# we1pingyu/CALD

Measured on AMD Instinct MI355X. Metric: unlabeled images scored/sec (CALD consistency sweep), higher is better.
Workload: dtype f32

## Files before the change

### cald_amd/_ffi.py

```python
import ctypes as C
import os

_HERE = os.path.dirname(os.path.abspath(__file__))
LIB_PATH = os.path.join(_HERE, "lib", "libcaldhip.so")
_lib = None

c_f = C.POINTER(C.c_float)
c_i = C.POINTER(C.c_int)
c_i64 = C.POINTER(C.c_int64)
c_d = C.POINTER(C.c_double)
c_u8 = C.POINTER(C.c_uint8)
c_i8 = C.POINTER(C.c_int8)


class ModelCfg(C.Structure):
    _fields_ = [("arch", C.c_int), ("depth", C.c_int), ("num_classes", C.c_int), ("min_size", C.c_int),
                ("max_size", C.c_int), ("box_score_thresh", C.c_float), ("box_nms_thresh", C.c_float),
                ("detections_per_img", C.c_int), ("rpn_pre_nms_top_n", C.c_int), ("rpn_post_nms_top_n", C.c_int),
                ("rpn_nms_thresh", C.c_float), ("precision", C.c_int)]


PRECISION = {"fp32": 0, "f16x3": 1}


# ... 51 lines not shown
PROBE_MAX_RECTS = 8


class ConvProbe(C.Structure):
    _fields_ = [("V", C.c_int), ("in_hw", (C.c_int * 2) * PROBE_MAX_VIEWS), ("up_hw", (C.c_int * 2) * PROBE_MAX_VIEWS),
                ("dyn_rows", C.c_int * PROBE_MAX_VIEWS), ("has_dyn", C.c_int), ("gather", C.c_int), ("nrect", C.c_int * PROBE_MAX_VIEWS),
                ("rect", ((C.c_int * 4) * PROBE_MAX_RECTS) * PROBE_MAX_VIEWS),
                ("Cin", C.c_int), ("Cout", C.c_int), ("KH", C.c_int), ("KW", C.c_int), ("stride", C.c_int), ("pad", C.c_int),
                ("relu", C.c_int), ("in_relu", C.c_int), ("out_ld", C.c_int), ("cin_true", C.c_int),
                ("weight", c_f), ("bias", c_f), ("bn_scale", c_f), ("bn_shift", c_f), ("in_", c_f), ("in16", C.POINTER(C.c_uint32)),
                ("residual", c_f), ("up", c_f), ("ex16", C.c_int), ("mask", c_f), ("row_map", c_i),
                ("out", c_f), ("out_n", C.c_int64), ("out16", C.POINTER(C.c_uint32)), ("out16_n", C.c_int64),
                ("energy4", c_f), ("energy4_n", C.c_int64),
                ("head_w", c_f), ("head_b", c_f), ("head_out", c_f), ("head_out_n", C.c_int64), ("head_ld", C.c_int),
                ("row_packing", C.c_int)]


PRUNE_PROBE_MAX_VIEWS = 8


class RpnPruneProbe(C.Structure):
    _fields_ = [("V", C.c_int), ("guard", C.c_int), ("hw", ((C.c_int * 2) * PRUNE_PROBE_MAX_VIEWS) * 2),
                ("pre_n", C.c_int), ("head_ld", C.c_int), ("c1", C.c_float * 3), ("c0", C.c_float * 3),
                ("energy", c_f * 2), ("exact", c_f * 2), ("head", c_f * 2), ("pnorm", c_f * 2),
                ("tau_key", C.POINTER(C.c_uint32)), ("row_map", (c_i * 2) * 2), ("nsel", c_i * 2),
                ("check", C.c_float * 2), ("stat", C.c_uint64 * 4)]


class WgradPlan(C.Structure):
    _fields_ = [("variant", C.c_int), ("reduce", C.c_int), ("MT", C.c_int), ("JT", C.c_int), ("S", C.c_longlong), ("chunk", C.c_longlong),
                ("csplit", C.c_longlong), ("rows_per_block", C.c_longlong), ("scratch_bytes", C.c_longlong),
                ("kernel", C.c_char * 48), ("reduce_kernel", C.c_char * 32)]


PICK_FN = C.CFUNCTYPE(C.c_int, C.c_void_p, C.c_int, C.c_int, c_i, c_i, c_i)
SSM_RETINA_TAKE = 500

SIGNATURES = {
    "cald_last_error": (C.c_char_p, []),
    "cald_version": (C.c_int, []),
    "cald_ctx_create": (C.c_int, [C.c_int, C.c_void_p, C.POINTER(C.c_void_p)]),
    "cald_ctx_destroy": (C.c_int, [C.c_void_p]),
    "cald_ctx_sync": (C.c_int, [C.c_void_p]),
    "cald_model_create": (C.c_int, [C.c_void_p, C.POINTER(ModelCfg), C.POINTER(C.c_void_p)]),
    "cald_model_load_tensor": (C.c_int, [C.c_void_p, C.c_char_p, c_f, c_i64, C.c_int]),
    "cald_model_finalize": (C.c_int, [C.c_void_p]),
    "cald_model_set_rpn_prune": (C.c_int, [C.c_void_p, C.c_int, c_i]),
    "cald_model_set_rpn_prune_capture": (C.c_int, [C.c_void_p, C.c_int]),
    "cald_model_rpn_prune_bound": (C.c_int, [C.c_void_p, c_f, c_f]),
    "cald_model_set_rpn_prune_bound": (C.c_int, [C.c_void_p, c_f, c_f]),
    "cald_profile_prune_fallbacks": (C.c_int, [C.c_void_p, C.POINTER(C.c_int64)]),
    "cald_model_destroy": (C.c_int, [C.c_void_p]),
    "cald_forward": (C.c_int, [C.c_void_p, C.c_int, C.POINTER(View), C.POINTER(Dets)]),
    "cald_sweep": (C.c_int, [C.c_void_p, C.c_int, C.POINTER(C.c_void_p), c_i, c_i, c_i64, C.POINTER(SweepCfg), c_d, c_d]),
    "cald_sweep_audit": (C.c_int, [C.c_void_p, C.c_int, C.POINTER(C.c_void_p), c_i, c_i, c_i64, C.POINTER(SweepCfg), c_d, c_d, c_f]),
    "cald_sweep_ltc": (C.c_int, [C.c_void_p, C.c_int, C.POINTER(C.c_void_p), c_i, c_i, C.c_int, c_d]),
    "cald_sweep_ssm": (C.c_int, [C.c_void_p, C.c_int, C.POINTER(C.c_void_p), c_i, c_i, C.c_int, C.c_int64, c_i, c_i, c_f, c_f, c_i8, c_i64]),
    "cald_ssm_pick_mt19937": (C.c_int, [C.c_void_p, C.c_int, C.c_int, c_i, c_i, c_i]),
    "cald_sweep_ssm_retina": (C.c_int, [C.c_void_p, C.c_int, C.POINTER(C.c_void_p), c_i, c_i, C.c_int, C.c_void_p, C.c_void_p, C.c_int64, c_i, c_i, c_f, c_f,
                                        c_i8, c_i64]),
    "cald_sweep_lsc": (C.c_int, [C.c_void_p, C.c_int, C.POINTER(C.c_void_p), c_i, c_i, c_i64, C.c_uint64, C.c_int, c_d]),
    "cald_lossnet_create": (C.c_int, [C.c_void_p, C.POINTER(C.c_void_p)]),
    "cald_lossnet_load_tensor": (C.c_int, [C.c_void_p, C.c_char_p, c_f, c_i64, C.c_int]),
    "cald_lossnet_finalize": (C.c_int, [C.c_void_p]),
    "cald_lossnet_destroy": (C.c_int, [C.c_void_p]),
    "cald_sweep_ll": (C.c_int, [C.c_void_p, C.c_void_p, C.c_int, C.POINTER(C.c_void_p), c_i, c_i, c_i, C.POINTER(LLCfg), c_d, c_f]),
    "cald_vaal_create": (C.c_int, [C.c_void_p, C.POINTER(C.c_void_p)]),
    "cald_vaal_load_tensor": (C.c_int, [C.c_void_p, C.c_char_p, c_f, c_i64, C.c_int]),
    "cald_vaal_finalize": (C.c_int, [C.c_void_p]),
    "cald_vaal_destroy": (C.c_int, [C.c_void_p]),
    "cald_sweep_vaal": (C.c_int, [C.c_void_p, C.c_void_p, C.c_int, C.POINTER(C.c_void_p), c_i, c_i, C.POINTER(VaalCfg), c_f, c_f]),
    "cald_op_vaal_resize": (C.c_int, [C.c_void_p, c_u8, C.c_int, C.c_int, c_f]),
    "cald_op_vaal_bn_relu": (C.c_int, [C.c_void_p, c_f, C.c_longlong, C.c_int, C.c_int, C.c_int, c_f, c_f, c_f]),
    "cald_op_vaal_fc_mu": (C.c_int, [C.c_void_p, C.c_int, c_f, c_f]),
    "cald_op_vaal_head": (C.c_int, [C.c_void_p, C.c_int, c_f, c_f]),
    "cald_train_gap": (C.c_int, [C.c_void_p, C.c_int, C.POINTER(C.c_void_p), c_i, C.c_void_p]),
    "cald_lossnet_train_fwd": (C.c_int, [C.c_void_p, C.c_int, C.c_int, C.POINTER(LossNetTensors), C.c_void_p, C.c_void_p, C.c_void_p]),
    "cald_lossnet_train_bwd": (C.c_int, [C.c_void_p, C.c_int, C.c_int, C.POINTER(LossNetTensors), C.c_void_p, C.c_void_p, C.c_void_p, C.c_void_p,
                                         C.POINTER(LossNetTensors), C.c_int, C.c_void_p]),
    "cald_loss_pred_loss": (C.c_int, [C.c_void_p, C.c_int, C.c_void_p, C.c_void_p, C.c_float, C.c_int, C.c_void_p, C.c_void_p, C.c_void_p, C.c_void_p]),
    "cald_op_gap": (C.c_int, [C.c_void_p, c_f, C.c_int, C.c_int, C.c_int, c_f]),
    "cald_op_lossnet": (C.c_int, [C.c_void_p, C.c_int, c_f, c_f]),
    "cald_op_consistency": (C.c_int, [C.c_void_p, C.c_int, c_f, c_f, c_f, C.c_int, c_f, c_f, c_f, C.c_int, C.c_float, c_f]),
    "cald_op_cls_corr": (C.c_int, [C.c_void_p, C.c_int, c_f, c_i64, C.c_int, c_f]),
    "cald_op_pil_resize": (C.c_int, [C.c_void_p, C.c_void_p, C.c_int, C.c_int, C.c_void_p, C.c_int, C.c_int]),
    "cald_op_cutout_rects": (C.c_int, [C.c_uint64, C.c_int, C.c_int, C.c_int, c_f, C.c_int, c_i, c_i]),
    "cald_op_cutout_geometry": (C.c_int, [C.c_int, C.c_int, C.c_int, C.c_int, C.c_int, c_i, C.c_int, c_i, c_i]),
    "cald_op_augment": (C.c_int, [C.c_void_p, C.c_int, C.c_double, C.c_uint64, C.c_void_p, C.c_int, C.c_int, C.c_int, c_f,
                                  C.c_void_p, c_f, c_i]),
    "cald_op_noise_stream": (C.c_int, [C.c_void_p, C.c_uint64, C.c_void_p, C.c_int, C.c_int, C.c_int, c_i, c_d, C.POINTER(C.c_void_p)]),
    "cald_op_frcnn_postprocess": (C.c_int, [C.c_void_p, C.c_int, C.c_int, c_f, c_f, c_f, C.c_int, C.c_int, C.c_int, C.c_int, C.c_float, C.c_float,
                                            C.c_int, c_f, c_f, c_i64, c_f, c_f, c_f, c_i]),
    "cald_op_frcnn_postprocess_min": (C.c_int, [C.c_void_p, C.c_int, C.c_int, c_f, c_f, c_f, C.c_int, C.c_int, C.c_int, C.c_int, C.c_float, C.c_float,
                                                C.c_int, C.c_float, c_f, c_f, c_i64, c_f, c_f, c_f, c_i]),
    "cald_op_ssm_postprocess": (C.c_int, [C.c_void_p, C.c_int, C.c_int, c_f, c_f, c_f, C.c_int, C.c_int, C.c_int, C.c_int, C.c_float, C.c_int,
                                          c_i, c_i, c_f, c_f, c_i8]),
    "cald_op_retina_postprocess": (C.c_int, [C.c_void_p, C.POINTER(c_f), C.POINTER(c_f), c_i, C.c_int, C.c_int, c_f] + [C.c_int] * 6
                                   + [C.c_float, C.c_float, C.c_int, c_f, c_f, c_i64, c_f, c_f, c_i]),
    "cald_op_retina_ssm_postprocess": (C.c_int, [C.c_void_p, C.POINTER(c_f), C.POINTER(c_f), c_i, C.c_int, C.c_int, c_f] + [C.c_int] * 6
                                       + [C.c_float, C.c_float, C.c_int, C.c_void_p, C.c_void_p, c_i, c_i, c_i, c_f, c_f, c_i8]),
    "cald_op_rpn_prune": (C.c_int, [C.c_void_p, C.POINTER(RpnPruneProbe)]),
    "cald_op_roi_align": (C.c_int, [C.c_void_p, C.POINTER(c_f), c_i, C.c_int, C.c_int, c_f, c_f]),
    "cald_op_conv2d": (C.c_int, [C.c_void_p, c_f, C.c_int, C.c_int, C.c_int, c_f, C.c_int, C.c_int, C.c_int, C.c_int,
                                 C.c_int, c_f, c_f, c_f, c_f, C.c_int, c_f]),
    "cald_op_conv_probe": (C.c_int, [C.c_void_p, C.c_int, C.POINTER(ConvProbe), C.c_int, C.c_int, C.c_int, C.c_char_p, C.c_int]),
    "cald_op_mfma_f16": (C.c_int, [C.c_void_p, C.POINTER(C.c_uint16), C.POINTER(C.c_uint16), C.POINTER(C.c_uint32), C.POINTER(C.c_uint32), C.c_int64]),
    "cald_op_conv2d_f16x3": (C.c_int, [C.c_void_p, c_f, C.c_int, C.c_int, C.c_int, c_f, C.c_int, C.c_int, C.c_int, C.c_int,
                                       C.c_int, c_f, c_f, c_f, c_f, C.c_int, c_f]),
    "cald_op_conv_bench": (C.c_int, [C.c_void_p] + [C.c_int] * 12 + [c_d, c_d]),
    "cald_op_row_pack_lookup": (C.c_int, [C.c_int, c_i, c_i, C.c_int, C.c_int, C.c_int64, c_i64, c_i, c_i64, c_i64]),
    "cald_op_transform_size": (C.c_int, [C.c_int, C.c_int, C.c_int, C.c_int, c_i, c_i, c_i, c_i]),
    "cald_debug_tensor": (C.c_int, [C.c_void_p, C.c_char_p, C.c_int, c_f, C.c_int64, c_i64]),
    "cald_jpeg_info": (C.c_int, [C.c_void_p, C.c_size_t, c_i, c_i, c_i]),
    "cald_jpeg_decode_batch": (C.c_int, [C.c_void_p, C.c_int, C.POINTER(C.c_void_p), C.POINTER(C.c_size_t), C.POINTER(C.c_void_p)]),
    "cald_jpeg_probe": (C.c_int, [C.c_void_p, C.c_size_t, c_i, c_i, c_i, c_i]),
    "cald_jpeg_decode_batch_any": (C.c_int, [C.c_void_p, C.c_int, C.POINTER(C.c_void_p), C.POINTER(C.c_size_t), C.POINTER(C.c_void_p)]),
    "cald_jpeg_decode_host": (C.c_int, [C.c_void_p, C.c_size_t, C.c_void_p]),
    "cald_profile_enable": (C.c_int, [C.c_void_p, C.c_int]),
    "cald_profile_read": (C.c_int, [C.c_void_p, c_d, c_d, c_i64, c_d]),
    "cald_profile_prune": (C.c_int, [C.c_void_p, c_d, c_d, c_d, c_d, c_d]),
    "cald_profile_roi_rows": (C.c_int, [C.c_void_p, c_d, c_i64]),
    "cald_profile_cutout": (C.c_int, [C.c_void_p, c_d, c_d, c_i64, c_i64]),
    "cald_model_set_cutout_reuse": (C.c_int, [C.c_void_p, C.c_int, c_i]),
    "cald_model_set_look_fuse": (C.c_int, [C.c_void_p, C.c_int, c_i]),
    "cald_model_set_row_packing": (C.c_int, [C.c_void_p, C.c_int, c_i]),
    "cald_model_set_box_min_size": (C.c_int, [C.c_void_p, C.c_float, c_f]),
    "cald_profile_dump": (C.c_int, [C.c_void_p, C.c_char_p]),
    "cald_train_packed_floats": (C.c_int, [C.c_int] * 6 + [c_i64]),
    "cald_train_pack_conv": (C.c_int, [C.c_void_p] * 5 + [C.c_int] * 6 + [C.c_void_p]),
    "cald_train_pack_plan_scratch_floats": (C.c_int, [C.c_int, C.POINTER(PackJob), c_i64]),
    "cald_train_pack_plan_create": (C.c_int, [C.c_void_p, C.c_int, C.POINTER(PackJob), C.c_void_p, C.c_int64, C.POINTER(C.c_void_p)]),
    "cald_train_pack_plan_run": (C.c_int, [C.c_void_p, C.c_void_p]),
    "cald_train_pack_plan_destroy": (C.c_int, [C.c_void_p]),
    "cald_train_conv": (C.c_int, [C.c_void_p, C.c_int, C.c_int, C.c_int, C.c_void_p, C.c_int, C.c_void_p] + [C.c_int] * 8
                        + [C.c_void_p, C.c_void_p, C.c_int, C.c_int, C.c_void_p, C.c_void_p, C.c_int]),
    "cald_train_conv_group": (C.c_int, [C.c_void_p, C.c_int, C.c_int, c_i, C.POINTER(C.c_void_p), C.c_int, C.POINTER(C.c_void_p)] + [C.c_int] * 8
                              + [C.POINTER(C.c_void_p), C.POINTER(C.c_void_p), C.c_int]),
    "cald_train_conv_wgrad": (C.c_int, [C.c_void_p, C.c_int, C.c_int, C.c_int, C.c_void_p, C.c_int, C.c_int, C.c_void_p, C.c_int,
                                        C.c_int, C.c_int, C.c_int, C.c_int, C.c_int, C.c_void_p, C.c_void_p, C.c_void_p, C.c_int]),
    "cald_train_linear_wgrad": (C.c_int, [C.c_void_p, C.c_int, C.c_void_p, C.c_int, C.c_void_p, C.c_int, C.c_int, C.c_int,
                                          C.c_void_p, C.c_void_p, C.c_int]),
    "cald_train_wgrad_plan": (C.c_int, [C.c_longlong] + [C.c_int] * 12 + [C.POINTER(WgradPlan)]),
    "cald_train_relu_bwd": (C.c_int, [C.c_void_p, C.c_longlong, C.c_int, C.c_void_p, C.c_void_p, C.c_void_p]),
    "cald_train_add": (C.c_int, [C.c_void_p, C.c_longlong, C.c_void_p, C.c_void_p, C.c_void_p]),
    "cald_train_dilate": (C.c_int, [C.c_void_p] + [C.c_int] * 7 + [C.c_void_p, C.c_void_p]),
    "cald_train_upsample_bwd": (C.c_int, [C.c_void_p] + [C.c_int] * 6 + [C.c_void_p, C.c_void_p]),
    "cald_train_rpn_proposals": (C.c_int, [C.c_void_p, C.c_int, C.c_int, C.c_int, c_i, C.POINTER(C.c_void_p), c_i, C.c_int, C.c_int, C.c_int,
                                           C.c_float, C.c_float, C.c_void_p, C.c_void_p]),
    "cald_train_roi_sample_host": (C.c_int, [C.c_int, c_i, c_i, c_i, C.c_void_p, C.c_void_p, C.c_void_p, C.c_int, C.c_double, C.c_int, C.c_int,
                                             C.c_void_p, C.c_void_p, C.c_void_p, C.c_void_p, C.c_void_p, C.c_void_p, c_i, c_i, c_i]),
    "cald_train_roi_gather": (C.c_int, [C.c_void_p, C.c_void_p, C.c_void_p, C.c_void_p, C.c_int, C.c_int, C.c_int] + [C.c_float] * 4 + [C.c_void_p, C.c_void_p]),
    "cald_train_anchors": (C.c_int, [C.c_void_p, C.c_int, C.c_int, C.c_int, c_i, C.c_void_p]),
    "cald_train_match": (C.c_int, [C.c_void_p, C.c_int, C.c_void_p, C.c_int, C.c_void_p, C.c_float, C.c_float, C.c_int, C.c_void_p, C.c_void_p]),
    "cald_train_box_encode": (C.c_int, [C.c_void_p, C.c_int, C.c_void_p, C.c_void_p, C.c_float, C.c_float, C.c_float, C.c_float, C.c_void_p]),
    "cald_train_roi_align": (C.c_int, [C.c_void_p, C.POINTER(C.c_void_p), c_i, C.c_int, C.c_int, C.c_void_p, C.c_void_p]),
    "cald_train_roi_align_bwd": (C.c_int, [C.c_void_p, C.c_int, C.POINTER(C.c_void_p), c_i, C.c_int, C.c_int, C.c_void_p, C.c_void_p]),
    "cald_train_softmax_ce": (C.c_int, [C.c_void_p, C.c_int, C.c_int, C.c_int, C.c_void_p, C.c_void_p, C.c_float, C.c_void_p, C.c_void_p]),
    "cald_train_smooth_l1": (C.c_int, [C.c_void_p, C.c_int, C.c_void_p, C.c_void_p, C.c_void_p, C.c_float, C.c_float, C.c_void_p, C.c_float,
                                       C.c_void_p, C.c_void_p]),
    "cald_train_focal_loss": (C.c_int, [C.c_void_p, C.c_int, c_i, C.c_int, C.c_int, C.c_int, C.c_void_p, C.c_void_p, C.c_void_p, C.c_void_p,
                                        C.c_void_p, C.c_float, C.c_float, C.c_void_p, C.c_void_p]),
    "cald_train_bce_logits": (C.c_int, [C.c_void_p, C.c_int, C.c_void_p, C.c_void_p, C.c_void_p, C.c_float, C.c_void_p, C.c_void_p]),
    "cald_train_softmax_ce_seg": (C.c_int, [C.c_void_p, C.c_int, c_i, C.c_int, C.c_int, C.c_void_p, C.c_void_p, C.c_void_p, C.c_void_p, C.c_void_p]),
    "cald_train_smooth_l1_seg": (C.c_int, [C.c_void_p, C.c_int, c_i, C.c_void_p, C.c_void_p, C.c_void_p, C.c_float, c_f, C.c_void_p, C.c_void_p,
                                           C.c_void_p]),
    "cald_train_bce_logits_seg": (C.c_int, [C.c_void_p, C.c_int, c_i, C.c_void_p, C.c_void_p, C.c_void_p, C.c_void_p, C.c_void_p, C.c_void_p]),
    "cald_train_focal_loss_seg": (C.c_int, [C.c_void_p, C.c_int, c_i, C.c_int, C.c_int, C.c_int, C.c_void_p, C.c_void_p, C.c_void_p, C.c_void_p,
                                            c_f, C.c_float, C.c_void_p, C.c_void_p, C.c_void_p, C.c_void_p]),
    "cald_train_seg_mean": (C.c_int, [C.c_void_p, C.c_int, C.c_void_p, C.c_void_p]),
    "cald_train_add_bcast": (C.c_int, [C.c_void_p, C.c_int, C.c_longlong, C.c_int, C.c_void_p, C.c_void_p, C.c_void_p, C.c_void_p, C.c_longlong]),
    "cald_train_preprocess": (C.c_int, [C.c_void_p, C.c_int, C.POINTER(C.c_void_p), C.POINTER(C.c_void_p), c_i, C.c_int, C.c_int, C.c_void_p]),
    "cald_train_maxpool": (C.c_int, [C.c_void_p, C.c_int, C.c_int, C.c_int, C.c_int, C.c_void_p, C.c_void_p]),
    "cald_train_subsample2": (C.c_int, [C.c_void_p, C.c_int, C.c_int, C.c_int, C.c_int, C.c_void_p, C.c_void_p]),
    "cald_train_sgd": (C.c_int, [C.c_void_p, C.c_longlong, C.c_void_p, C.c_void_p, C.c_void_p, C.c_float, C.c_float, C.c_float, C.c_int]),
    "cald_train_seg_cache_size": (C.c_int, []),
    "cald_comm_unique_id": (C.c_int, [C.c_void_p]),
# ... 37 lines not shown
```

### cald_amd/csrc/conv_p4.hip

```cpp
#include "h16.h"

typedef float f32x16 __attribute__((ext_vector_type(16)));
typedef int i32x4 __attribute__((ext_vector_type(4)));
typedef float f32x4 __attribute__((ext_vector_type(4)));

template <int EPI, bool MASK, int TM, int TN, bool GATHER = false>
__device__ __forceinline__ void p4_epilogue(const ConvArgs& a, const f32x16 (&acc)[TM][TN], float* smem, const int v, const LevelSeg& so,
                                            const int m0, const int Mv, const int n0, const bool straddle = false) {
    constexpr int BM = 128, WN = 2;
    const int tid = threadIdx.x, lane = tid & 63, wave = tid >> 6;
    const int wm = wave / WN, wn = wave % WN;
    const int kh_lane = lane >> 5, l31 = lane & 31;
    const int Ho = so.H, Wo = so.W;
    const int out_ld = a.out_ld;
    float* __restrict__ out_v = a.out + so.pix_off * (long long)out_ld;
    const float* __restrict__ ex_v = nullptr;
    int upH = 1, upW = 1;
    float uph_s = 0.f, upw_s = 0.f;
    long long up_off = 0;
    if (EPI == 1) ex_v = a.residual + so.pix_off * (long long)out_ld;
    if (EPI == 2) {
        const LevelSeg su = a.seg_up[v];
        up_off = su.pix_off;
        ex_v = a.up + su.pix_off * (long long)out_ld;
        upH = su.H; upW = su.W;
        uph_s = (float)upH / (float)Ho; upw_s = (float)upW / (float)Wo;
    }
    const bool relu = a.relu != 0, has_bias = a.bias != nullptr, has_bn = a.scale != nullptr;
    constexpr bool has_mask = MASK;
    const float* __restrict__ mask_v = has_mask ? a.mask + so.pix_off * (long long)out_ld : out_v;
    const int row_b = out_ld * 4;
    const unsigned long long vb64 = (unsigned long long)(GATHER ? Ho * Wo : Mv) * (unsigned)row_b;
    const unsigned valid_b = vb64 < 0x7FFE0000ull ? (unsigned)vb64 : 0x7FFE0000u;
    const __amdgpu_buffer_rsrc_t rsO = __builtin_amdgcn_make_buffer_rsrc((void*)out_v, 0, valid_b, 0x00020000);
    const __amdgpu_buffer_rsrc_t rsX = __builtin_amdgcn_make_buffer_rsrc((void*)(EPI != 0 ? ex_v : out_v), 0, EPI == 1 ? valid_b : 0x7FFE0000, 0x00020000);
    const __amdgpu_buffer_rsrc_t rsM = __builtin_amdgcn_make_buffer_rsrc((void*)mask_v, 0, valid_b, 0x00020000);
    static_assert(!(GATHER && EPI == 2), "gathered rows take no top-down term");
    const int Mlast = Mv - 1;
    int* const s_src = reinterpret_cast<int*>(smem);
    if (EPI == 2 || GATHER) {
        if (tid < BM) {
            int m = m0 + tid;
            if (GATHER) {
                s_src[tid] = m < Mv ? gather_pixel(a.gather[v], m, Wo) * row_b : 0x7FFF0000;
            } else if (EPI == 2 && straddle) {
                int src = 0;
                if (m < Mv) {
                    const long long r = so.pix_off + m;
                    int vr = v;
                    while (vr + 1 < a.V && a.seg_out[vr + 1].pix_off <= r) vr++;
                    const LevelSeg sor = a.seg_out[vr], sur = a.seg_up[vr];
                    const int ml = (int)(r - sor.pix_off), oy = ml / sor.W, ox = ml - oy * sor.W;
                    const float hs = (float)sur.H / (float)sor.H, ws = (float)sur.W / (float)sor.W;
                    int sy = (int)floorf((float)oy * hs); sy = sy > sur.H - 1 ? sur.H - 1 : sy;
                    int sx = (int)floorf((float)ox * ws); sx = sx > sur.W - 1 ? sur.W - 1 : sx;
                    src = ((int)(sur.pix_off - up_off) + sy * sur.W + sx) * out_ld * 4;
                }
                s_src[tid] = src;
            } else {
                m = m < Mlast ? m : Mlast;
                const int oy = m / Wo, ox = m - oy * Wo;
                int sy = (int)floorf((float)oy * uph_s); sy = sy > upH - 1 ? upH - 1 : sy;
                int sx = (int)floorf((float)ox * upw_s); sx = sx > upW - 1 ? upW - 1 : sx;
                s_src[tid] = (sy * upW + sx) * out_ld * 4;
            }
        }
        __syncthreads();
    }
    auto gather_offs = [&](const int i, const int n, const bool nok, int (&go)[16]) {
        const int rl = wm * TM * 32 + i * 32 + 4 * kh_lane;
#pragma unroll
        for (int q = 0; q < 4; q++) {
            const i32x4 so4 = *reinterpret_cast<const i32x4*>(s_src + rl + 8 * q);
#pragma unroll
            for (int jj = 0; jj < 4; jj++) go[4 * q + jj] = nok ? so4[jj] + n * 4 : 0x7FFF0000;
        }
    };
    constexpr bool EXTRA = EPI == 0 && !MASK && !GATHER;
    const bool want16 = EXTRA && a.out16 != nullptr, wantE = EXTRA && TN == 2 && a.energy4 != nullptr;
    unsigned char* const out16_v = want16 ? reinterpret_cast<unsigned char*>(a.out16) + so.pix_off * (long long)out_ld * 4 : nullptr;
    const __amdgpu_buffer_rsrc_t rsS = __builtin_amdgcn_make_buffer_rsrc((void*)(want16 ? (void*)out16_v : (void*)out_v), 0, valid_b, 0x00020000);
    const bool odd = (lane & 1) != 0;
    float sq[TM][16];
    if (EXTRA) {
#pragma unroll
        for (int i = 0; i < TM; i++)
#pragma unroll
            for (int r = 0; r < 16; r++) sq[i][r] = 0.0f;
    }
    float bs_[TN], sc_[TN], sh_[TN];
#pragma unroll
    for (int j = 0; j < TN; j++) {
        const int n = n0 + wn * TN * 32 + j * 32 + l31;
        const int nc = n < a.Cout ? n : 0;
        bs_[j] = has_bias ? a.bias[nc] : 0.0f;
        sc_[j] = has_bn ? a.scale[nc] : 1.0f;
        sh_[j] = has_bn ? a.shift[nc] : 0.0f;
    }
    constexpr int NTILE = TM * TN, PRE = GATHER ? 1 : NTILE;
    float extra_[EPI != 0 ? NTILE : 1][16];
    auto load_extra = [&](const int t, float (&extra)[16]) {
        const int j = t / TM, i = t - j * TM;
        const int n = n0 + wn * TN * 32 + j * 32 + l31;
        const bool nok = n < a.Cout;
        const int nc = nok ? n : 0;
        const int mbase = m0 + wm * TM * 32 + i * 32 + 4 * kh_lane;
        if (EPI == 1 && GATHER) {
            int go[16];
            gather_offs(i, n, nok, go);
#pragma unroll
            for (int r = 0; r < 16; r++) extra[r] = __builtin_bit_cast(float, __builtin_amdgcn_raw_buffer_load_b32(rsX, go[r], 0, 0));
        } else if (EPI == 1) {
            const int vo = nok ? (mbase * out_ld + n) * 4 : 0x7FFF0000;
#pragma unroll
            for (int r = 0; r < 16; r++)
                extra[r] = __builtin_bit_cast(float, __builtin_amdgcn_raw_buffer_load_b32(rsX, vo, ((r & 3) + 8 * (r >> 2)) * row_b, 0));
        } else if (EPI == 2) {
            const int rl = wm * TM * 32 + i * 32 + 4 * kh_lane;
#pragma unroll
            for (int q = 0; q < 4; q++) {
                const i32x4 so4 = *reinterpret_cast<const i32x4*>(s_src + rl + 8 * q);
#pragma unroll
                for (int jj = 0; jj < 4; jj++)
                    extra[4 * q + jj] = __builtin_bit_cast(float, __builtin_amdgcn_raw_buffer_load_b32(rsX, so4[jj] + nc * 4, 0, 0));
            }
        }
    };
    if (EPI != 0) {
#pragma unroll
        for (int t = 0; t < PRE; t++) load_extra(t, extra_[EPI != 0 ? t : 0]);
    }
#pragma unroll
    for (int j = 0; j < TN; j++) {
        const int n = n0 + wn * TN * 32 + j * 32 + l31;
        const bool nok = n < a.Cout;
        const int nc = nok ? n : 0;
        const float bs = bs_[j], sc = sc_[j], sh = sh_[j];
#pragma unroll
        for (int i = 0; i < TM; i++) {
            const int mbase = m0 + wm * TM * 32 + i * 32 + 4 * kh_lane;
            const float (&extra)[16] = extra_[EPI != 0 ? j * TM + i : 0];
            float val[16];
#pragma unroll
            for (int r = 0; r < 16; r++) val[r] = acc[i][j][r];
            if (has_bias) {
#pragma unroll
                for (int r = 0; r < 16; r++) val[r] = val[r] + bs;
            }
            if (has_bn) {
#pragma unroll
                for (int r = 0; r < 16; r++) { val[r] = val[r] * sc; val[r] = val[r] + sh; }
            }
            if (EPI != 0) {
#pragma unroll
                for (int r = 0; r < 16; r++) val[r] = val[r] + extra[r];
            }
            if (relu) {
#pragma unroll
                for (int r = 0; r < 16; r++) val[r] = val[r] > 0.0f ? val[r] : 0.0f;
            }
            if (EPI != 0 && j * TM + i + PRE < NTILE) load_extra(j * TM + i + PRE, extra_[EPI != 0 ? j * TM + i + PRE : 0]);
            const int vo = nok ? (mbase * out_ld + n) * 4 : 0x7FFF0000;
            if (has_mask) {
                float mk[16];
#pragma unroll
                for (int r = 0; r < 16; r++)
                    mk[r] = __builtin_bit_cast(float, __builtin_amdgcn_raw_buffer_load_b32(rsM, vo, ((r & 3) + 8 * (r >> 2)) * row_b, 0));
#pragma unroll
                for (int r = 0; r < 16; r++) val[r] = mk[r] > 0.0f ? val[r] : 0.0f;
            }
            if (GATHER) {
                int go[16];
                gather_offs(i, n, nok, go);
#pragma unroll
                for (int r = 0; r < 16; r++) __builtin_amdgcn_raw_buffer_store_b32(__builtin_bit_cast(unsigned, val[r]), rsO, go[r], 0, 0);
            } else {
#pragma unroll
                for (int r = 0; r < 16; r++)
                    __builtin_amdgcn_raw_buffer_store_b32(__builtin_bit_cast(unsigned, val[r]), rsO, vo, ((r & 3) + 8 * (r >> 2)) * row_b, 0);
            }
            if (EXTRA) {
                if (wantE) {
#pragma unroll
                    for (int r = 0; r < 16; r++) sq[i][r] = sq[i][r] + (nok ? val[r] * val[r] : 0.0f);
                }
                if (want16) {
                    const int poff = h16_pair_off(nc);
#pragma unroll
                    for (int r = 0; r < 16; r++) {
                        const unsigned w = h16_split(val[r]);
                        const unsigned pw = h16_pair_word(w, h16_partner(w), odd);
                        __builtin_amdgcn_raw_buffer_store_b32(pw, rsS, nok ? mbase * row_b + poff : 0x7FFF0000, ((r & 3) + 8 * (r >> 2)) * row_b, 0);
                    }
                }
            }
        }
    }
    if (EXTRA) {
        if (wantE) {
            __syncthreads();
            float* const red = smem + wave * (64 * 33);
#pragma unroll
            for (int i = 0; i < TM; i++)
#pragma unroll
                for (int r = 0; r < 16; r++) red[(i * 32 + 4 * kh_lane + (r & 3) + 8 * (r >> 2)) * 33 + l31] = sq[i][r];
            asm volatile("s_waitcnt lgkmcnt(0)" ::: "memory");
            float e = 0.0f;
#pragma unroll
            for (int q = 0; q < 32; q++) e = e + red[lane * 33 + q];
            const int m = m0 + wm * TM * 32 + lane;
            if (m < Mv) a.energy4[(so.pix_off + m) * 4 + (n0 / (64 * TN)) * 2 + wn] = e;
        }
    }
}

template <int EPIX, bool C4, int TN, int TAPS>
__device__ __forceinline__ void conv_p4_body(const ConvArgs& a, const int blk, const ConvArgs* a3 = nullptr) {
    constexpr int EPI = EPIX & 3;
    constexpr bool MASK = (EPIX & 4) != 0;
    constexpr bool FUSE = (EPIX & 8) != 0;
    constexpr bool GATHER = (EPIX & 16) != 0;
    static_assert(!(GATHER && (FUSE || MASK || C4)), "gathered rows: plain EPI 0 / 1 kernels only");
    constexpr int BM = 128, BN = 64 * TN, BK = 16, TM = 2, WN = 2;
    constexpr int TILE_A = 2 * BM * 8, TILE_F = TILE_A + 2 * BN * 8;
    constexpr int FUSE_T = 4 * TILE_A;
    __shared__ __attribute__((aligned(16))) float smem[FUSE ? FUSE_T + 4096 : 3 * TILE_F];

    const int tid = threadIdx.x, lane = tid & 63, wave = tid >> 6;
    const int wm = wave / WN, wn = wave % WN;
    const int NT = a.CoutPad / BN;
    unsigned long long* const trace = (a.trace && blockIdx.x < (1u << 17)) ? a.trace + (size_t)blockIdx.x * 8 : nullptr;
    if (trace && tid == 0) {
        trace[0] = __builtin_amdgcn_s_memtime();
        trace[5] = (unsigned)__builtin_amdgcn_s_getreg((31 << 11) | 4);
        trace[6] = (unsigned)__builtin_amdgcn_s_getreg((31 << 11) | 20);
        trace[7] = blockIdx.x;
    }
    int mt, nt;
    if (a.KH * a.KW > 1) {
        const int MT = a.total_mtiles, CH = (MT + 7) >> 3;
        const int xcd = blk & 7, idx = blk >> 3;
        mt = xcd * CH + idx / NT; nt = idx % NT;
        if (idx / NT >= CH || mt >= MT) return;
    } else {
        const int b = blk, MT = a.total_mtiles, MT8 = MT & ~7;
        if (b < MT8 * NT) { const int xcd = b & 7, idx = b >> 3; mt = (idx / NT) * 8 + xcd; nt = idx % NT; }
        else { const int r = b - MT8 * NT; mt = MT8 + r / NT; nt = r % NT; }
    }
    const int n0 = nt * BN;
    constexpr bool CAN_PACK = !C4 && !MASK && !FUSE && !GATHER;
    const bool packed = CAN_PACK && a.packed_rows != 0;
    const int v = packed ? seg_find_row(a.seg_out, a.V, (long long)mt * BM) : seg_find_view(a.seg_out, a.V, mt);
    const LevelSeg so = a.seg_out[v];
    const LevelSeg si = a.seg_in[v];
    const int Ho = so.H, Wo = so.W, Hi = si.H, Wi = si.W;
    int Mv = Ho * Wo;
    if (a.dyn_rows) { const int d = a.dyn_rows[v]; Mv = d < Mv ? d : Mv; }
    if (GATHER) Mv = a.gather[v].cum[a.gather[v].nr];
    int m0 = (mt - so.tile_start) * BM;
    bool straddle = false;
    if (CAN_PACK && packed) {
        const int row0 = mt * BM, left = a.packed_rows - row0;
        m0 = row0 - (int)so.pix_off;
        const int end = m0 + (left < BM ? left : BM);
        straddle = end > Mv;
        Mv = end;
    }
    if (m0 >= Mv) return;
    const float* __restrict__ in_v = a.in + si.pix_off * (long long)a.Cin;
    const int Cin = a.Cin, KW = a.KW, KH = a.KH, CoutPad = a.CoutPad;
    const bool in_relu = a.in_relu != 0;

    const int g = tid & 3, arow = tid >> 2;
    unsigned rowmask[2];
// ... 328 lines not shown
            __syncthreads();
            if (n0c + 64 < CoutPad3) fetch_w(n0c + 64);
            const int n3 = n0c + wn * 32 + l31;
            int vo3[2];
            float ex[2][16];
#pragma unroll
            for (int i = 0; i < 2; i++) vo3[i] = ((m0 + wm * 64 + i * 32 + 4 * kh_lane) * ld3 + n3) * 4;
#pragma unroll
            for (int i = 0; i < 2; i++)
#pragma unroll
                for (int r = 0; r < 16; r++)
                    ex[i][r] = __builtin_bit_cast(float, __builtin_amdgcn_raw_buffer_load_b32(rsX3, vo3[i], ((r & 3) + 8 * (r >> 2)) * ld3 * 4, 0));
            __builtin_amdgcn_sched_barrier(0);
            f32x16 acc2[2][1];
#pragma unroll
            for (int i = 0; i < 2; i++)
#pragma unroll
                for (int r = 0; r < 16; r++) acc2[i][0][r] = 0.0f;
#pragma unroll
            for (int kt = 0; kt < 4; kt++) {
                f32x4 ga0[2], ga1[2];
#pragma unroll
                for (int t = 0; t < 2; t++) {
                    ga0[t] = *reinterpret_cast<const f32x4*>(Tl + kt * TILE_A + foa2[t]);
                    ga1[t] = *reinterpret_cast<const f32x4*>(Tl + kt * TILE_A + foa2[t] + BM * 8);
                }
                const f32x4 gb0 = *reinterpret_cast<const f32x4*>(Wl + kt * 1024 + fob2);
                const f32x4 gb1 = *reinterpret_cast<const f32x4*>(Wl + kt * 1024 + fob2 + 64 * 8);
#pragma unroll
                for (int q = 0; q < 4; q++)
#pragma unroll
                    for (int i = 0; i < 2; i++) acc2[i][0] = __builtin_amdgcn_mfma_f32_32x32x2f32(ga0[i][q], gb0[q], acc2[i][0], 0, 0, 0);
#pragma unroll
                for (int q = 0; q < 4; q++)
#pragma unroll
                    for (int i = 0; i < 2; i++) acc2[i][0] = __builtin_amdgcn_mfma_f32_32x32x2f32(ga1[i][q], gb1[q], acc2[i][0], 0, 0, 0);
            }
            {
                const float sc3 = b.scale[n3], sh3 = b.shift[n3];
#pragma unroll
                for (int i = 0; i < 2; i++) {
#pragma unroll
                    for (int r = 0; r < 16; r++) {
                        float val = acc2[i][0][r] * sc3;
                        val = val + sh3;
                        val = val + ex[i][r];
                        if (relu3) val = val > 0.0f ? val : 0.0f;
                        __builtin_amdgcn_raw_buffer_store_b32(__builtin_bit_cast(unsigned, val), rsO3, vo3[i], ((r & 3) + 8 * (r >> 2)) * ld3 * 4, 0);
                    }
                }
            }
        }
    } else {
        p4_epilogue<EPI, MASK, TM, TN, GATHER>(a, acc, smem, v, so, m0, Mv, n0, CAN_PACK && straddle);
    }
    if (trace && tid == 0) {
        trace[3] = __builtin_amdgcn_s_memtime();
        asm volatile("s_waitcnt vmcnt(0)" ::: "memory");
        trace[4] = __builtin_amdgcn_s_memtime();
    }
}

template <int EPI, bool C4, int TN, int TAPS>
__global__ __launch_bounds__(256, 3) void conv_p4_kernel(const ConvArgs a) { conv_p4_body<EPI, C4, TN, TAPS>(a, blockIdx.x); }
template <int EPI, bool C4, int TN, int TAPS>
__global__ __launch_bounds__(256, 3) void conv_p4_group_kernel(const ConvGroup g) {
    int i = 0;
    while (i + 1 < g.n && g.blk0[i + 1] <= (int)blockIdx.x) i++;
    conv_p4_body<EPI, C4, TN, TAPS>(g.p[i], (int)blockIdx.x - g.blk0[i]);
}
__global__ __launch_bounds__(256, 3) void conv_p4_fused_kernel(const ConvGroup g) { conv_p4_body<8, false, 1, 9>(g.p[0], blockIdx.x, &g.p[1]); }

static inline int p4_taps(const ConvArgs& a) {
    if (a.Cin % 16 != 0) return 0;
    if (a.KH == 3 && a.KW == 3) return 9;
    if (a.KH == 1 && a.KW == 1) return 1;
    return 0;
}

static inline int p4_grid_mtiles(const ConvArgs& a) { return a.KH * a.KW > 1 ? 8 * ((a.total_mtiles + 7) / 8) : a.total_mtiles; }

static inline bool p4_refuses(const ConvArgs& a) {
    if (!a.w4 || !a.out || a.in16 || a.ex16 || a.CoutPad % 64 != 0 || (a.residual && a.up)) return true;
    const bool extra = a.out16 || a.energy4;
    if (extra && (a.residual || a.up || a.mask || a.gather)) return true;
    if (a.energy4 && a.CoutPad != 256) return true;
    if (a.row_map && (a.residual || a.up || a.mask || a.gather)) return true;
    return false;
}
static inline bool p4_tile_ok(const ConvArgs& a, const bool wide, const ConvForce f) {
    if (f.tile == TILE_NARROW && wide) return false;
    if (f.tile == TILE_WIDE && !wide) return false;
    return !(a.energy4 && !wide);
}

static inline ConvArgs p4_tiled(ConvArgs a) {
    if (a.packed_rows > 0 && a.Cin != 4 && !a.dyn_rows && !a.row_map && !a.gather && !a.mask) a.total_mtiles = (a.packed_rows + 127) / 128;
    else a.packed_rows = 0;
    return a;
}

#define P4_NAME(K, EPIV, C4V, TNV, TAPSV) K "<" #EPIV "," #C4V "," #TNV "," #TAPSV ">"
template <int EPI, bool C4, int TN, int TAPS>
static const char* p4_go(const dim3 grid, hipStream_t stream, const ConvArgs& a, const char* name) {
    hipLaunchKernelGGL((conv_p4_kernel<EPI, C4, TN, TAPS>), grid, dim3(256), 0, stream, a);
    return name;
}
template <int EPI, int TN, int TAPS>
static const char* p4_group_go(const dim3 grid, hipStream_t stream, const ConvGroup& g, const char* name) {
    hipLaunchKernelGGL((conv_p4_group_kernel<EPI, false, TN, TAPS>), grid, dim3(256), 0, stream, g);
    return name;
}

const char* launch_conv_p4_group(const ConvArgs* p, int n, hipStream_t stream, ConvForce f) {
    if (n < 1 || n > CALD_MAX_GROUP) return nullptr;
    const bool wide = f.tile == TILE_NARROW ? false : p[0].CoutPad % 128 == 0;
    ConvGroup g; g.n = n; int blk = 0;
    for (int i = 0; i < n; i++) {
        const ConvArgs a = p4_tiled(p[i]);
        if (p4_refuses(a) || !p4_tile_ok(a, wide, f) || (a.CoutPad % 128 == 0) != (p[0].CoutPad % 128 == 0)) return nullptr;
        if (a.Cin % 16 != 0 || a.KH * a.KW > 32 || a.residual || a.up || a.gather) return nullptr;
        if ((a.mask != nullptr) != (p[0].mask != nullptr)) return nullptr;
        if (a.mask && (a.out16 || a.energy4)) return nullptr;
        g.blk0[i] = blk; blk += p4_grid_mtiles(a) * (a.CoutPad / (wide ? 128 : 64)); g.p[i] = a;
    }
    g.blk0[n] = blk;
    const int taps = p4_taps(p[0]);
    for (int i = 1; i < n; i++) if (p4_taps(p[i]) != taps) return nullptr;
    const dim3 grid((unsigned)blk);
#define P4_GROUP(EV, TNV, TAPSV) p4_group_go<EV, TNV, TAPSV>(grid, stream, g, P4_NAME("conv_p4_group_kernel", EV, false, TNV, TAPSV))
#define P4_GROUP_T(EV) (wide ? (taps == 9 ? P4_GROUP(EV, 2, 9) : taps == 1 ? P4_GROUP(EV, 2, 1) : P4_GROUP(EV, 2, 0)) \
                             : (taps == 9 ? P4_GROUP(EV, 1, 9) : taps == 1 ? P4_GROUP(EV, 1, 1) : P4_GROUP(EV, 1, 0)))
    const char* name = p[0].mask ? P4_GROUP_T(4) : P4_GROUP_T(0);
#undef P4_GROUP_T
#undef P4_GROUP
    return name;
}

const char* launch_conv_p4_fused(const ConvArgs& c2, const ConvArgs& c3, hipStream_t stream) {
    if (!c2.w4 || !c3.w4 || c2.w16 || c3.w16) return nullptr;
    if (c2.KH != 3 || c2.KW != 3 || c2.stride != 1 || c2.pad != 1 || c2.Cin % 16 || c2.Cout != 64 || c2.CoutPad != 64 || c2.out_ld != 64) return nullptr;
    if (c2.residual || c2.up || c2.mask || c2.dyn_rows || c2.in_relu || c2.gather || c3.gather || p4_taps(c2) != 9) return nullptr;
    if (c3.KH != 1 || c3.KW != 1 || c3.stride != 1 || c3.pad != 0 || c3.Cin != 64 || c3.Kpad != 64 || c3.CoutPad % 64 || c3.Cout != c3.CoutPad) return nullptr;
    if (!c3.residual || !c3.scale || c3.bias || c3.out_ld != c3.Cout || c3.up || c3.mask || c3.dyn_rows || c3.in_relu || c3.in != c2.out || c3.total_mtiles != c2.total_mtiles || c3.V != c2.V) return nullptr;
    if (c2.row_map || c3.row_map || c2.in16 || c3.in16 || c2.out16 || c3.out16 || c2.energy4 || c3.energy4 || c2.ex16 || c3.ex16 || !c3.out) return nullptr;
    ConvGroup g; g.n = 2; g.blk0[0] = 0; g.p[0] = c2; g.p[1] = c3;
    const unsigned grid = (unsigned)p4_grid_mtiles(c2);
    hipLaunchKernelGGL(conv_p4_fused_kernel, dim3(grid), dim3(256), 0, stream, g);
    return "conv_p4_fused_kernel";
}

const char* launch_conv_p4(const ConvArgs& a_in, hipStream_t stream, ConvForce f) {
    const ConvArgs a = p4_tiled(a_in);
    if (p4_refuses(a)) return nullptr;
    bool wide = a.CoutPad % 128 == 0;
    if (wide) {
        const long long b2 = (long long)a.total_mtiles * (a.CoutPad / 128), b1 = 2 * b2;
        const double e2 = (double)b2 / (double)(((b2 + 767) / 768) * 768), e1 = 0.88 * (double)b1 / (double)(((b1 + 767) / 768) * 768);
        if (e1 > e2 && !a.dyn_rows && !a.energy4) wide = false;
    }
    if (f.tile == TILE_NARROW) wide = false;
    else if (f.tile == TILE_WIDE) wide = a.CoutPad % 128 == 0;
    if (!p4_tile_ok(a, wide, f)) return nullptr;
    const dim3 grid((unsigned)(p4_grid_mtiles(a) * (a.CoutPad / (wide ? 128 : 64))));
#define P4_ONE(EPIV, C4V, TNV, TAPSV) p4_go<EPIV, C4V, TNV, TAPSV>(grid, stream, a, P4_NAME("conv_p4_kernel", EPIV, C4V, TNV, TAPSV))
    if (a.gather) {
        const int taps = p4_taps(a);
        if (a.Cin == 4 || a.up || a.mask || a.in_relu || a.dyn_rows || a.row_map || (taps != 1 && taps != 9)) return nullptr;
        if (a.total_mtiles == 0) return "none (no gathered rows)";
#define P4_G(EPIV, TNV) (taps == 9 ? P4_ONE(EPIV, false, TNV, 9) : P4_ONE(EPIV, false, TNV, 1))
        return wide ? (a.residual ? P4_G(17, 2) : P4_G(16, 2)) : (a.residual ? P4_G(17, 1) : P4_G(16, 1));
#undef P4_G
    }
    if (a.Cin == 4) {
        if (a.residual || a.up || a.in_relu || a.mask) return nullptr;
        if (a.KH == 7 && a.KW == 7 && a.Kpad == 208)
            return wide ? P4_ONE(0, true, 2, 13) : P4_ONE(0, true, 1, 13);
        return wide ? P4_ONE(0, true, 2, 0) : P4_ONE(0, true, 1, 0);
    }
    if (a.Cin % 16 != 0 || a.KH * a.KW > 32) return nullptr;
    const int taps = p4_taps(a);
#define P4_TAPS(EPIV, TNV) (taps == 9 ? P4_ONE(EPIV, false, TNV, 9) : taps == 1 ? P4_ONE(EPIV, false, TNV, 1) : P4_ONE(EPIV, false, TNV, 0))
    const char* name;
    if (a.mask) {
        if (a.up) return nullptr;
        name = wide ? (a.residual ? P4_TAPS(5, 2) : P4_TAPS(4, 2)) : (a.residual ? P4_TAPS(5, 1) : P4_TAPS(4, 1));
    } else if (wide) {
        name = a.residual ? P4_TAPS(1, 2) : a.up ? P4_TAPS(2, 2) : P4_TAPS(0, 2);
    } else {
        name = a.residual ? P4_TAPS(1, 1) : a.up ? P4_TAPS(2, 1) : P4_TAPS(0, 1);
    }
#undef P4_TAPS
#undef P4_ONE
    return name;
}
#undef P4_NAME
```

### cald_amd/csrc/ctx.hip

```cpp
#include "host.h"

static thread_local char g_err[512] = "";
int cald_host::fail(int code, const char* fmt, ...) {
    va_list ap; va_start(ap, fmt); vsnprintf(g_err, sizeof(g_err), fmt, ap); va_end(ap);
    return code;
}

int cald_internal_fail(int code, const char* fmt, ...) {
    va_list ap; va_start(ap, fmt); vsnprintf(g_err, sizeof(g_err), fmt, ap); va_end(ap);
    return code;
}
void cald_internal_train_release(cald_ctx* c);

extern "C" const char* cald_last_error(void) { return g_err; }
extern "C" int cald_version(void) { return 100; }

hipStream_t cald_internal_stream(cald_ctx* c) { return c->stream; }
int cald_internal_device(cald_ctx* c) { return c->device; }
const float* cald_internal_zeros(cald_ctx* c) { return c->d_zeros; }
int cald_internal_scratch(cald_ctx* c, size_t bytes, void** out) {
    if (bytes > c->train_scratch_cap) {
        HIPCHK(hipStreamSynchronize(c->stream));
        if (c->train_scratch) HIPCHK(hipFree(c->train_scratch));
        c->train_scratch = nullptr; c->train_scratch_cap = 0;
// ... 97 lines not shown
    }
    if (gemm_ms) *gemm_ms = ms;
    unsigned long long rows = 0;
    HIPCHK(hipMemcpy(&rows, c->d_roi_rows, 8, hipMemcpyDeviceToHost));
    double fl = c->prof_flops - look_fl;
    if (c->prof_roi_rows_cap > 0.0) fl -= c->prof_roi_flops_cap * (1.0 - (double)rows / c->prof_roi_rows_cap);
    unsigned long long st[4] = {0, 0, 0, 0};
    HIPCHK(hipMemcpy(st, c->d_prune_stat, 32, hipMemcpyDeviceToHost));
    for (int l = 0; l < 2; l++) if (st[2 * l + 1]) fl -= c->prof_prune_flops_cap[l] * (1.0 - (double)st[2 * l] / (2.0 * (double)st[2 * l + 1]));
    if (gemm_flops) *gemm_flops = fl;
    if (launches) *launches = (int64_t)c->prof_launches.size() - look_n + c->prof_extra_launches;
    if (total_ms) *total_ms = c->tot_ms;
    return 0;
}

extern "C" int cald_profile_prune(cald_ctx* c, double* look_ms, double* look_flops, double* selected_frac2, double* worst_bound_ratio, double* pruned_flops) {
    if (!c) return fail(CALD_ERR_INVALID, "ctx is null");
    HIPCHK(hipStreamSynchronize(c->stream));
    double ms = 0.0, fl = 0.0;
    for (const ProfLaunch& L : c->prof_launches)
        if (L.tag) { float t = 0.f; HIPCHK(hipEventElapsedTime(&t, L.e0, L.e1)); ms += t; fl += L.flops; }
    unsigned long long st[4] = {0, 0, 0, 0};
    HIPCHK(hipMemcpy(st, c->d_prune_stat, 32, hipMemcpyDeviceToHost));
    if (look_ms) *look_ms = ms;
    if (look_flops) *look_flops = fl;
    if (selected_frac2) for (int l = 0; l < 2; l++) selected_frac2[l] = st[2 * l + 1] ? (double)st[2 * l] / (double)st[2 * l + 1] : 0.0;
    if (worst_bound_ratio) *worst_bound_ratio = (double)c->prune_worst;
    if (pruned_flops) {
        double fl2 = 0.0;
        for (int l = 0; l < 2; l++) if (st[2 * l + 1]) fl2 += c->prof_prune_flops_cap[l] / 2.0 * (1.0 - (double)st[2 * l] / (double)st[2 * l + 1]);
        *pruned_flops = fl2;
    }
    return 0;
}

extern "C" int cald_profile_roi_rows(cald_ctx* c, double* mean_rows_per_view, int64_t* views) {
    if (!c) return fail(CALD_ERR_INVALID, "ctx is null");
    HIPCHK(hipStreamSynchronize(c->stream));
    unsigned long long rows = 0;
    HIPCHK(hipMemcpy(&rows, c->d_roi_rows, 8, hipMemcpyDeviceToHost));
    if (views) *views = c->prof_roi_views;
    if (mean_rows_per_view) *mean_rows_per_view = c->prof_roi_views ? (double)rows / (double)c->prof_roi_views : 0.0;
    return 0;
}

extern "C" int cald_profile_cutout(cald_ctx* c, double* rows3, double* dense_rows3, int64_t* batches, int64_t* fallbacks) {
    if (!c) return fail(CALD_ERR_INVALID, "ctx is null");
    for (int i = 0; i < 3; i++) { if (rows3) rows3[i] = c->cut_rows[i]; if (dense_rows3) dense_rows3[i] = c->cut_dense[i]; }
    if (batches) *batches = c->cut_batches;
    if (fallbacks) *fallbacks = c->cut_fallbacks;
    return 0;
}

extern "C" int cald_profile_dump(cald_ctx* c, const char* path) {
    if (!c || !path) return fail(CALD_ERR_INVALID, "null argument");
    HIPCHK(hipStreamSynchronize(c->stream));
    FILE* f = fopen(path, "w");
    if (!f) return fail(CALD_ERR_INVALID, "cannot open %s", path);
    fprintf(f, "launch,desc,gflop,ms,tflops\n");
    std::vector<unsigned long long> lg((size_t)CALD_PRUNE_LOG * 4, 0ull);
    if (!c->prof_gather.empty()) HIPCHK(hipMemcpy(lg.data(), c->d_prune_log, lg.size() * 8, hipMemcpyDeviceToHost));
    for (size_t i = 0; i < c->prof_launches.size(); i++) {
        const ProfLaunch& L = c->prof_launches[i];
        float t = 0.f; hipEventElapsedTime(&t, L.e0, L.e1);
        double fl = L.flops;
        const char* extra = L.tag ? ",f16x3-lookahead" : "";
        auto g = c->prof_gather.find(i);
        if (g != c->prof_gather.end()) {
            for (int l = 0; l < 2; l++) {
                const unsigned long long sel = lg[(size_t)g->second.log * 4 + 2 * l], tot = lg[(size_t)g->second.log * 4 + 2 * l + 1];
                if (tot) fl -= g->second.cap[l] * (1.0 - (double)sel / (double)tot);
            }
            extra = ",gathered-rows";
        }
        fprintf(f, "%zu,\"%s%s\",%.3f,%.4f,%.2f\n", i, L.desc.c_str(), extra, fl / 1e9, t, fl / (t * 1e-3) / 1e12);
    }
    fclose(f);
    return 0;
}
extern "C" int cald_profile_prune_fallbacks(cald_ctx* c, int64_t* n) {
    if (!c || !n) return fail(CALD_ERR_INVALID, "null argument");
    *n = (int64_t)c->prune_fallbacks;
    return 0;
}

int cald_host::prof_begin(cald_ctx* c, ProfLaunch& t) {
    if (!c->prof) return 0;
    HIPCHK(hipEventCreate(&t.e0)); HIPCHK(hipEventCreate(&t.e1));
    HIPCHK(hipEventRecord(t.e0, c->stream));
    return 0;
}
int cald_host::prof_end(cald_ctx* c, ProfLaunch& t, double flops, int tag, const char* fmt, ...) {
    if (!c->prof) return 0;
    HIPCHK(hipEventRecord(t.e1, c->stream));
    char d[160];
    va_list ap; va_start(ap, fmt); vsnprintf(d, sizeof(d), fmt, ap); va_end(ap);
    t.flops = flops; t.tag = tag; t.desc = d;
    c->prof_launches.push_back(t); c->prof_flops += flops;
    return 0;
}

int cald_host::conv_refused(const ConvArgs& a) {
    return fail(CALD_ERR_UNSUPPORTED, "no conv kernel implements this launch (Cin=%d Cout=%d k=%dx%d residual=%d up=%d mask=%d gather=%d energy4=%d out16=%d)",
                a.Cin, a.Cout, a.KH, a.KW, a.residual != nullptr, a.up != nullptr, a.mask != nullptr, a.gather != nullptr, a.energy4 != nullptr,
                a.out16 != nullptr);
}
// ... 9 lines not shown
```

### cald_amd/csrc/forward.hip

```cpp
#include "host.h"

#define ROI_DENSE_VIEWS 32
void cald_host::build_plan(BatchPlan& P, int V, const ViewDesc* views, const int (*hp)[2], bool retina) {
    memset(&P, 0, sizeof(P));
    for (int l = 0; l < CALD_MAX_LEVELS; l++) {
        long long off = 0; int tile = 0;
        for (int v = 0; v <= V; v++) {
            LevelSeg& s = P.seg[l][v];
            s.pix_off = off; s.tile_start = tile;
            if (v == V) break;
            int H, W;
            if (l == 7 && retina) { int h6 = (hp[v][0] / 32 - 1) / 2 + 1, w6 = (hp[v][1] / 32 - 1) / 2 + 1; H = (h6 - 1) / 2 + 1; W = (w6 - 1) / 2 + 1; }
            else if (l == 7) { H = 1; W = CALD_ROI_CAP; }
            else if (l == 8) {
                const int first = v * ROI_DENSE_VIEWS, cnt = first < V ? (V - first < ROI_DENSE_VIEWS ? V - first : ROI_DENSE_VIEWS) : 0;
                H = cnt ? 1 : 0; W = cnt * CALD_ROI_CAP;
            }
            else if (l == 6) { H = (hp[v][0] / 32 - 1) / 2 + 1; W = (hp[v][1] / 32 - 1) / 2 + 1; }
            else { H = hp[v][0] >> l; W = hp[v][1] >> l; }
            s.H = H; s.W = W;
            off += (long long)H * W;
            tile += (H * W + 127) / 128;
        }
    }
// ... 248 lines not shown
static int conv_pair_on(cald_model* m, const ConvLayer& L2, const ConvLayer& L3, const float* in, float* mid, float* out, int lin, int lout,
                        int V, const float* residual) {
    cald_ctx* c = m->ctx;
    if (m->cfg.precision == CALD_PRECISION_FP32 && L2.stride == 1 && lin == lout) {
        ConvArgs a2, a3;
            const double f2 = fill_conv_args(m, a2, L2, in, mid, lin, lout, V, true);
        const double f3 = fill_conv_args(m, a3, L3, mid, out, lout, lout, V, true, residual);
        if (f2 < 0.0 || f3 < 0.0) return (int)(f2 < 0.0 ? f2 : f3);
        ProfLaunch t; int rc;
        if ((rc = prof_begin(c, t))) return rc;
        if (launch_conv_p4_fused(a2, a3, c->stream) != nullptr)
            return prof_end(c, t, f2 + f3, 0, "mt=%d,Cin=%d,Cout=%d,k=3x3+1x1,s=1,fused->%d", a2.total_mtiles, a2.Cin, a2.Cout, a3.Cout);
        if (c->prof) { hipEventDestroy(t.e0); hipEventDestroy(t.e1); }
    }
    int rc = conv_on(m, L2, in, mid, lin, lout, V, true);
    if (rc) return rc;
    return conv_on(m, L3, mid, out, lout, lout, V, true, residual);
}
static int conv_group_on(cald_model* m, const ConvSpec* sp, int n, int V) {
    ConvArgs a[CALD_MAX_GROUP];
    double flops = 0.0; int tiles = 0;
    for (int i = 0; i < n; i++) {
        const double f = fill_conv_args(m, a[i], *sp[i].L, sp[i].in, sp[i].out, sp[i].level, sp[i].level, V, sp[i].relu, nullptr, nullptr, 0, sp[i].dyn);
        if (f < 0.0) return (int)f;
        a[i].row_map = sp[i].row_map;
        if (sp[i].in16) a[i].in16 = sp[i].in16;
        if (sp[i].out16) a[i].out16 = sp[i].out16;
        a[i].energy4 = sp[i].energy4;
        offer_packing(m, a[i], sp[i].level, sp[i].level, 0, V);
        flops += f; tiles += a[i].total_mtiles;
    }
    cald_ctx* c = m->ctx;
    const char* names[CALD_MAX_GROUP];
    ProfLaunch t; int rc;
    if ((rc = prof_begin(c, t))) return rc;
    const int launches = launch_conv_group(a, n, c->stream, names);
    if (c->prof) c->prof_extra_launches += launches - 1;
    if ((rc = prof_end(c, t, flops, c->prof_tag_now, "mt=%d,Cin=%d,Cout=%d,k=%dx%d,s=%d,group=%d", tiles, a[0].Cin, a[0].Cout, a[0].KH, a[0].KW, a[0].stride, n))) return rc;
    for (int i = 0; i < n; i++) if (!names[i]) return conv_refused(a[i]);
    return 0;
}

static int gconv_on(cald_model* m, const ConvLayer& L, const float* in, float* out, int lin, int lout, int V, bool relu, const float* residual,
                    const FwdReuse& ru, int b, int kind) {
    if (!ru.tiles[b][kind]) return 0;
    ConvArgs a;
    const double f = fill_conv_args(m, a, L, in, out, lin, lout, V, relu, residual);
    if (f < 0.0) return (int)f;
    const char* base = ru.d_gp + (size_t)(2 * b + kind) * cut_plan_set_bytes(V);
    a.seg_out = reinterpret_cast<const LevelSeg*>(base);
    a.gather = reinterpret_cast<const GatherSet*>(base + (size_t)(V + 1) * sizeof(LevelSeg));
    a.total_mtiles = ru.tiles[b][kind];
    return run_conv(m->ctx, a, 2.0 * ru.rows[b][kind] * (double)L.Cout * (double)(L.KH * L.KW * L.CinTrue));
}

__global__ void accumulate_rows_kernel(const int* __restrict__ counts, int V, unsigned long long* acc) {
    unsigned long long s = 0;
    for (int v = threadIdx.x; v < V; v += 64) s += (unsigned long long)counts[v];
    for (int o = 32; o > 0; o >>= 1) s += __shfl_down(s, o);
    if (threadIdx.x == 0) atomicAdd(acc, s);
}

static const float RPN_MIN_SIZE = 1e-3f;
struct ForwardRun {
    cald_model* m; int V; ViewDesc* views; const DetBuffers& det; float* audit_out; bool prune_ok; const FwdReuse* ru; FwdFeatures* feat; FwdSsm* ssm; FwdRetinaSsm* rssm;
    cald_ctx* c = nullptr; hipStream_t st = nullptr; const BatchPlan* dp = nullptr;
    bool retina = false, prune = false;
    int hp[CALD_MAX_VIEWS][2], max_pix0 = 0, max_pix2 = 0, max_pix6 = 0;
    BodyBufs Fb; PyramidBufs Fp; RetinaBufs Fr; RpnBufs Fn; PruneBufs Fq; BoxBufs Fx; AuditBufs Fa;
    void layout(Bump& B) {
        const BatchPlan& P = m->plan; long long px[8];
        for (int l = 0; l < 8; l++) px[l] = level_pix(P, l, V);
        m->split.clear();
        static const bool split_on = !(getenv("CALD_H3_S16") && atoi(getenv("CALD_H3_S16")) == 0);
        SplitReg S{m, B, m->cfg.precision == CALD_PRECISION_F16X3 && split_on};
        Fb.layout(B, S, px);
        Fp.layout(B, S, px, retina);
        if (feat) return;
        if (retina) {
            int maxa = 0;
            for (int v = 0; v < V; v++) { int t = 0; for (int l = 3; l < 8; l++) t += P.seg[l][v].H * P.seg[l][v].W * 9; if (t > maxa) maxa = t; }
            Fr.layout(B, S, px, V, m->cls_out.Cout, m->cfg.num_classes, m->cfg.detections_per_img, maxa, rssm ? &rssm->out : nullptr);
            return;
        }
        Fn.layout(B, px, V, m->cfg.rpn_pre_nms_top_n);
        if (m->prune) Fq.layout(B, px, V, m->prune_capture);
        Fx.layout(B, S, V, m->pred.Cout, m->cfg.num_classes, m->key_cap);
        Fa.layout(B, V, m->det_cap());
        if (ssm) ssm->out.layout(B, V, m->cfg.num_classes, m->cfg.detections_per_img);
    }
    int prepare() {
        c = m->ctx;
        if (!m->finalized) return fail(CALD_ERR_STATE, "model not finalized (call cald_model_finalize)");
        if (V < 1 || V > CALD_MAX_VIEWS) return fail(CALD_ERR_INVALID, "n_views must be 1..%d", CALD_MAX_VIEWS);
        if (feat && (audit_out || prune_ok || ru)) return fail(CALD_ERR_INVALID, "a features-only forward takes no audit, pruning or cut_out reuse");
        if (ssm && (feat || audit_out || ru || m->cfg.arch != CALD_ARCH_FRCNN)) return fail(CALD_ERR_INVALID, "the SSM forward is a plain Faster R-CNN forward");
        if (rssm && (feat || audit_out || ru || ssm || !rssm->pick || m->cfg.arch != CALD_ARCH_RETINANET || m->cfg.num_classes < 2))
            return fail(CALD_ERR_INVALID, "the RetinaNet SSM forward is a plain RetinaNet forward with a pick callback and at least two classes");
        if (!feat && !ssm && !rssm && det.cap < m->det_cap()) return fail(CALD_ERR_INVALID, "detection capacity %d < required %d", det.cap, m->det_cap());
        HIPCHK(hipSetDevice(c->device));
        for (int v = 0; v < V; v++) {
            ViewDesc& d = views[v];
            if (!d.src || d.H <= 0 || d.W <= 0 || d.nrect < 0 || d.nrect > CALD_MAX_CUT) return fail(CALD_ERR_INVALID, "view %d is malformed", v);
            int Hp, Wp;
            transform_size(d.H, d.W, m->cfg.min_size, m->cfg.max_size, &d.Hr, &d.Wr, &Hp, &Wp);
            d.Ho = d.H; d.Wo = d.W;
// ... 20 lines not shown
        { Bump dry(nullptr, true); layout(dry); int rc = arena_reserve(c, dry.off); if (rc) return rc; }
        { Bump real(c->arena, false); layout(real); }
        const int si = c->stage_i; c->stage_i = (si + 1) % cald_ctx::NSTAGE;
        HIPCHK(hipEventSynchronize(c->stage_ev[si]));
        memcpy(c->h_stage[si], &m->plan, sizeof(BatchPlan));
        memcpy(c->h_stage[si] + sizeof(BatchPlan), views, sizeof(ViewDesc) * V);
        HIPCHK(hipMemcpyAsync(c->d_plan, c->h_stage[si], sizeof(BatchPlan), hipMemcpyHostToDevice, c->stream));
        HIPCHK(hipMemcpyAsync(c->d_views, c->h_stage[si] + sizeof(BatchPlan), sizeof(ViewDesc) * V, hipMemcpyHostToDevice, c->stream));
        HIPCHK(hipEventRecord(c->stage_ev[si], c->stream));
        dp = c->d_plan; st = c->stream;
        m->dbg.clear();
        return 0;
    }
    int dense_block(const Bottleneck& B, const float* cur, float* dst, int lvl, int lout) {
        int rc; const float* idn = cur;
        if (B.has_down) { if ((rc = conv_on(m, B.down, cur, Fb.D, lvl, lout, V, false))) return rc; idn = Fb.D; }
        if ((rc = conv_on(m, B.c1, cur, Fb.T1, lvl, lvl, V, true))) return rc;
        return conv_pair_on(m, B.c2, B.c3, Fb.T1, Fb.T2, dst, lvl, lout, V, idn);
    }
    int gathered_block(const Bottleneck& B, int b, const float* cur, float* dst, int lvl, int lout) {
        int rc; const float* idn = cur;
        if (B.has_down) { if ((rc = gconv_on(m, B.down, cur, Fb.D, lvl, lout, V, false, nullptr, *ru, b, 0))) return rc; idn = Fb.D; }
        if ((rc = gconv_on(m, B.c1, cur, Fb.T1, lvl, lvl, V, true, nullptr, *ru, b, 1))) return rc;
        if ((rc = gconv_on(m, B.c2, Fb.T1, Fb.T2, lvl, lout, V, true, nullptr, *ru, b, 0))) return rc;
        return gconv_on(m, B.c3, Fb.T2, dst, lout, lout, V, true, idn, *ru, b, 0);
    }
    int body() {
        int rc;
        launch_preprocess(c->d_views, dp->seg[0], Fb.in0, V, max_pix0, st);
        m->dbg["input"] = {Fb.in0, 0, 4, 0};
        if ((rc = conv_on(m, m->conv1, Fb.in0, Fb.c1, 0, 1, V, true))) return rc;
        m->dbg["conv1"] = {Fb.c1, 1, 64, 0};
        launch_maxpool(Fb.c1, Fb.p1, dp->seg[1], dp->seg[2], 64, V, max_pix2, st, m->split.count(Fb.p1) != 0);
        m->dbg["pool1"] = {Fb.p1, 2, 64, 0};
        const float* cur = Fb.p1; int lvl = 2, layer = 0, xi = 0;
        for (size_t b = 0; b < m->blocks.size(); b++) {
            const Bottleneck& B = m->blocks[b];
            const int lout = lvl + (B.c2.stride == 2 ? 1 : 0);
            const bool kept = ru && (int)b < ru->nblk;
            float* dst = kept ? ru->out[b] : (B.layer_end ? Fb.Cf[layer] : Fb.X[xi]);
            if ((rc = kept && ru->mode == 2 && ru->gather[layer] ? gathered_block(B, (int)b, cur, dst, lvl, lout) : dense_block(B, cur, dst, lvl, lout))) return rc;
            if (B.layer_end) Fb.Cf[layer] = dst;
            cur = dst; lvl = lout;
            if (B.layer_end) layer++; else xi ^= 1;
        }
        const char* cn[4] = {"C2", "C3", "C4", "C5"};
        for (int i = 0; i < 4; i++) m->dbg[cn[i]] = {Fb.Cf[i], 2 + i, CCH[i], 0};
        return 0;
    }
    void name_pyramid(int first, int n) { for (int i = 0; i < n; i++) m->dbg["P" + std::to_string(first + i)] = {Fp.Pf[i], first + i, 256, 0}; }
    int fpn() {
        const int first = retina ? 3 : 2, nl = retina ? 3 : 4, c0 = 4 - nl;
        int rc; ConvSpec sp[4];
        if ((rc = conv_on(m, m->fpn_inner[nl - 1], Fb.Cf[3], Fp.inner[nl - 1], 5, 5, V, false))) return rc;
        for (int i = nl - 2; i >= 0; i--)
            if ((rc = conv_on(m, m->fpn_inner[i], Fb.Cf[c0 + i], Fp.inner[i], first + i, first + i, V, false, nullptr, Fp.inner[i + 1], first + 1 + i))) return rc;
        for (int i = 0; i < nl; i++) sp[i] = {&m->fpn_layer[i], Fp.inner[i], Fp.Pf[i], first + i, false};
        if (prune)
            for (int i = 0; i < 2; i++) { sp[i].out16 = Fq.p16[i]; sp[i].energy4 = Fq.energy[i]; }
        if ((rc = conv_group_on(m, sp, nl, V))) return rc;
        if (!retina) return 0;
        if ((rc = conv_on(m, m->p6, Fp.Pf[2], Fp.Pf[3], 5, 6, V, false))) return rc;
        if (feat && !feat->p7) return 0;
        return conv_on(m, m->p7, Fp.Pf[3], Fp.Pf[4], 6, 7, V, false, nullptr, nullptr, 0, nullptr, true);
    }
    void hand_out(int first, int n) {
        name_pyramid(first, n);
        for (int i = 0; i < n; i++) {
            auto sp = m->split.find(Fp.Pf[i]);
            feat->P[i] = Fp.Pf[i]; feat->split_only[i] = sp != m->split.end() && sp->second.fp32_dead; feat->plan_level[i] = first + i;
        }
    }
    int retina_head_and_tail() {
        int rc;
        for (int t = 0; t < 4; t++) {
            ConvSpec sp[10];
            for (int hsel = 0; hsel < 2; hsel++)
                for (int i = 0; i < 5; i++)
                    sp[hsel * 5 + i] = {&(hsel == 0 ? m->cls_tower : m->reg_tower)[t], t == 0 ? Fp.Pf[i] : Fr.ret_t[hsel][(t - 1) & 1][i],
                                        Fr.ret_t[hsel][t & 1][i], 3 + i, true};
            if ((rc = conv_group_on(m, sp, 10, V))) return rc;
        }
        for (int hsel = 0; hsel < 2; hsel++) {
            ConvSpec sp[5];
            for (int i = 0; i < 5; i++) sp[i] = {hsel == 0 ? &m->cls_out : &m->reg_out, Fr.ret_t[hsel][1][i], hsel == 0 ? Fr.cls_h[i] : Fr.reg_h[i], 3 + i, false};
            if ((rc = conv_group_on(m, sp, 5, V))) return rc;
        }
        for (int i = 0; i < 5; i++) {
            m->dbg["cls" + std::to_string(i)] = {Fr.cls_h[i], 3 + i, m->cls_out.Cout, 0};
            m->dbg["reg" + std::to_string(i)] = {Fr.reg_h[i], 3 + i, 36, 0};
        }
        if (rssm) return retina_ssm_tail();
        launch_retina_postprocess(retina_args(Fr.tail, Fr.cls_h, Fr.reg_h, dp, c->d_views, m->d_anchors, 9, m->cfg.num_classes, V, m->cfg.box_score_thresh,
                                              m->cfg.box_nms_thresh, m->cfg.detections_per_img, det), Fr.tail.max_anchors, st);
        return 0;
    }
    int retina_ssm_tail() {
        const RetinaSsmArgs sa = retina_ssm_args(rssm->out, Fr.cls_h, Fr.reg_h, dp, c->d_views, m->d_anchors, 9, m->cfg.num_classes, V, m->cfg.box_score_thresh,
                                                 m->cfg.box_nms_thresh, m->cfg.detections_per_img);
        launch_retina_ssm_phase_a(sa, st);
        HIPCHK(hipGetLastError());
        if (int rc = retina_ssm_pick_stop(c, rssm->out, V, m->cfg.num_classes, rssm->pick, rssm->user, rssm->image0, nullptr)) return rc;
        launch_retina_ssm_phase_b(sa, st);
        return 0;
    }
    void p6_subsample() {
        auto tw = m->split.find(Fp.Pf[3]);
        const bool p6_split = m->split.count(Fp.Pf[4]) != 0 && tw != m->split.end();
        launch_subsample2(p6_split ? reinterpret_cast<const float*>(tw->second.s16) : Fp.Pf[3], Fp.Pf[4], dp->seg[5], dp->seg[6], 256, V, max_pix6, st);
        name_pyramid(2, 5);
    }
    void name_rpn(int first) { for (int i = first; i < 5; i++) m->dbg["rpn" + std::to_string(i)] = {Fn.rpn_h[i], 2 + i, 15, 0}; }
    int rpn_dense() {
// ... 208 lines not shown
```

### cald_amd/csrc/host.h

```cpp
#pragma once
#include "../../include/cald_hip.h"
#include "common.h"
#include "kernels.h"
#include "host_logic.h"

#include <climits>
#include <cmath>
#include <cstdarg>
#include <cstdio>
#include <cstring>
#include <algorithm>
#include <map>
#include <string>
#include <vector>

namespace cald_host {
int fail(int code, const char* fmt, ...);
#define HIPCHK(x) do { hipError_t e_ = (x); if (e_ != hipSuccess) return fail(CALD_ERR_HIP, "%s failed: %s (%s:%d)", #x, hipGetErrorString(e_), __FILE__, __LINE__); } while (0)

struct PilCoef { int ksize; int* d_bounds; int* d_kk; };
struct PilKey { int in, out, fid; bool operator<(const PilKey& o) const { return in != o.in ? in < o.in : (out != o.out ? out < o.out : fid < o.fid); } };
struct ProfLaunch {
    hipEvent_t e0 = nullptr, e1 = nullptr;
    double flops = 0.0;
    int tag = 0;
    std::string desc;
};
}
using namespace cald_host;

#define CALD_PRUNE_LOG 4096
struct cald_ctx {
    int device = 0;
    hipStream_t stream = nullptr;
    bool own_stream = false;
    char* arena = nullptr; size_t arena_cap = 0, arena_off = 0;
    BatchPlan* d_plan = nullptr;
    ViewDesc* d_views = nullptr;
    float* d_zeros = nullptr;
    static const int NSTAGE = 8;
    char* h_stage[NSTAGE] = {nullptr}; hipEvent_t stage_ev[NSTAGE] = {nullptr}; int stage_i = 0;
    bool prof = false;
    std::vector<ProfLaunch> prof_launches;
    double prof_flops = 0.0; int64_t prof_extra_launches = 0;
    int prof_tag_now = 0;
    double prof_prune_flops_cap[2] = {0.0, 0.0};
    hipEvent_t tot0 = nullptr, tot1 = nullptr; bool tot_open = false; double tot_ms = 0.0;
    float prune_worst = 0.0f;
    long long prune_fallbacks = 0;
    float* d_prune_check = nullptr;
    unsigned long long* d_prune_stat = nullptr;
    unsigned long long* d_prune_log = nullptr; int prune_log_n = 0;
    struct GatherNote { int log; double cap[2]; };
    std::map<size_t, GatherNote> prof_gather;
    unsigned long long* d_roi_rows = nullptr; double prof_roi_rows_cap = 0.0, prof_roi_flops_cap = 0.0; long long prof_roi_views = 0;
    std::map<PilKey, PilCoef> pil;
    char* train_scratch = nullptr; size_t train_scratch_cap = 0;
    double cut_rows[3] = {0.0, 0.0, 0.0}, cut_dense[3] = {0.0, 0.0, 0.0};
    long long cut_batches = 0, cut_fallbacks = 0;
};

namespace cald_host {
struct ScopedDev {
    std::vector<void*> ptrs;
    hipStream_t st;
    explicit ScopedDev(hipStream_t s) : st(s) {}
    ~ScopedDev() { if (!ptrs.empty()) { hipStreamSynchronize(st); for (void* p : ptrs) hipFree(p); } }
    void release() { ptrs.clear(); }
    template <typename T> int alloc(T** out, size_t bytes) {
        HIPCHK(hipMalloc((void**)out, bytes ? bytes : 1));
        ptrs.push_back((void*)*out);
        return 0;
    }
    template <typename T> int upload(T** out, const void* h, size_t bytes) {
        *out = nullptr;
        if (!h) return 0;
        if (int rc = alloc(out, bytes)) return rc;
        HIPCHK(hipMemcpy((void*)*out, h, bytes, hipMemcpyHostToDevice));
        return 0;
    }
};
struct Bump {
    char* base; size_t off = 0; bool dry;
    explicit Bump(char* b, bool d) : base(b), dry(d) {}
    template <typename T> T* get(size_t count) {
        size_t bytes = (count * sizeof(T) + 255) & ~(size_t)255;
        T* p = dry ? nullptr : reinterpret_cast<T*>(base + off);
        off += bytes;
        return p;
    }
};

struct HostTensor { std::vector<float> data; std::vector<int64_t> shape; };
struct ConvLayer {
    float *w = nullptr, *w4 = nullptr, *bias = nullptr, *scale = nullptr, *shift = nullptr;
    float* wstem = nullptr;
    uint16_t* w16 = nullptr; float w16_unscale = 1.0f;
    int Cin = 0, Cout = 0, CoutPad = 0, K = 0, Kpad = 0, KH = 1, KW = 1, stride = 1, pad = 0;
    int CinTrue = 0;
};
struct Bottleneck { ConvLayer c1, c2, c3, down; bool has_down = false; bool layer_end = false; };
struct DebugEntry { const float* ptr; int level; int C; int kind; };
}

struct cald_model {
    cald_ctx* ctx = nullptr;
    cald_model_cfg cfg;
    std::map<std::string, HostTensor> sd;
    bool finalized = false;
    ConvLayer conv1; std::vector<Bottleneck> blocks;
    ConvLayer fpn_inner[4], fpn_layer[4], rpn_conv, rpn_head, fc6, fc7, pred;
    ConvLayer rpn_conv16; bool prune = false; float prune_c1[3] = {0, 0, 0}, prune_c0[3] = {0, 0, 0};
    bool prune_allowed = false;
    int look_fuse = 1; float* look_head_w = nullptr; float look_head_b[3] = {0, 0, 0};
    int row_packing = -1;
    bool prune_bound_voided = false;
    bool prune_capture = false;
    ConvLayer p6, p7, cls_tower[4], reg_tower[4], cls_out, reg_out;
    int det_cap() const { return cfg.arch == CALD_ARCH_RETINANET ? cfg.num_classes * cfg.detections_per_img : cfg.detections_per_img; }
    float* d_anchors = nullptr;
    std::vector<void*> owned;
    std::map<std::string, DebugEntry> dbg;
    BatchPlan plan; int last_V = 0;
    struct SplitFmt { unsigned* s16; bool fp32_dead; };
    std::map<const float*, SplitFmt> split;
    std::vector<ViewDesc> last_views;
    DetBuffers sweep_det; int sweep_det_views = 0;
    DetBuffers sweep_det2; int sweep_det2_views = 0;
    struct SweepScratch {
        size_t dev_bytes = 0, pin_bytes = 0, aug_cap = 0;
        char* dev = nullptr; char* pin = nullptr; uint8_t* d_aug = nullptr;
        hipEvent_t ev_ref[2] = {nullptr, nullptr}, ev_score[2] = {nullptr, nullptr};
    } ss;
    float box_min_size = 0.0f;
    int key_cap = 32768;
    struct CutReuse {
        int mode = -1;
        char* slot[2] = {nullptr, nullptr}; size_t cap[2] = {0, 0};
        char* h_gp[2] = {nullptr, nullptr}; char* d_gp = nullptr;
    } cr;
};

namespace cald_host {
struct ConvPack {
    std::vector<float> w, w4, wstem;
    std::vector<uint16_t> w16; float w16_unscale = 1.0f;
    int Cout = 0, CoutPad = 0, K = 0, Kpad = 0;
};
struct ConvSpec { const ConvLayer* L; const float* in; float* out; int level; bool relu; const int* dyn = nullptr; const int* row_map = nullptr; const unsigned* in16 = nullptr;
                  unsigned* out16 = nullptr; float* energy4 = nullptr; };

#define CUT_MAX_BLOCKS 32
struct FwdReuse {
    int mode = 0;
    int nblk = 0;
    float* out[CUT_MAX_BLOCKS] = {};
    bool gather[3] = {false, false, false};
    const char* d_gp = nullptr;
    int tiles[CUT_MAX_BLOCKS][2] = {};
    double rows[CUT_MAX_BLOCKS][2] = {};
};
struct FwdFeatures {
    const int (*pad_to)[2] = nullptr;
    bool p7 = false;
    const float* P[5] = {}; bool split_only[5] = {}; int plan_level[5] = {};
};
struct ProposalBufs { float* proposals = nullptr; int* prop_count = nullptr; void layout(Bump& B, int V); };
struct RoiBufs { float* roi = nullptr; int* order = nullptr; void layout(Bump& B, int V, int C); };
struct PostBufs {
    float *prob = nullptr, *pmax = nullptr, *cbox = nullptr; unsigned long long* keys = nullptr; int* key_count = nullptr; int key_cap = 0;
    unsigned char* skip = nullptr;
    void layout(Bump& B, int V, int C, int key_cap);
};
struct SsmBufs {
    float *prob = nullptr, *kept_box = nullptr, *boxes = nullptr, *scores = nullptr; unsigned* vmax = nullptr; signed char* labels = nullptr;
    int *kept_prop = nullptr, *cls_count = nullptr, *row_off = nullptr, *al = nullptr, *count = nullptr, *total = nullptr;
    void layout(Bump& B, int V, int C, int cap);
};
struct FwdSsm { SsmBufs out; };
#define SSM_NMS_THR 0.3f
#define SSM_CONF_THR 0.5f
struct RetinaTailBufs {
    int *cand_count = nullptr, *kept_anchor = nullptr, *kept_count = nullptr, cand_cap = 0, max_anchors = 0; unsigned long long* cand_key = nullptr;
    float *cand_box = nullptr, *kept_box = nullptr; unsigned char* cand_skip = nullptr;
    void layout(Bump& B, int V, int K, int per_class, int max_anchors);
};
struct RetinaSsmBufs {
    int *cand_count = nullptr, *blk_off = nullptr, *list = nullptr, *al = nullptr, *picks = nullptr, *n_picks = nullptr, *kept_anchor = nullptr, *kept_count = nullptr,
        *row_off = nullptr, *count = nullptr, *total = nullptr, cand_cap = 0, nblk = 0;
    unsigned* vmax = nullptr; float *kept_box = nullptr, *boxes = nullptr, *scores = nullptr; signed char* labels = nullptr;
    void layout(Bump& B, int V, int K, int per_class, int max_anchors);
};
struct FwdRetinaSsm { cald_ssm_pick_fn pick = nullptr; void* user = nullptr; int image0 = 0; RetinaSsmBufs out; };
RetinaSsmArgs retina_ssm_args(const RetinaSsmBufs& S, const float* const* cls, const float* const* reg, const BatchPlan* plan, const ViewDesc* views,
                              const float* base_anchors, int A, int K, int V, float score_thr, float nms_thr, int per_class);
int retina_ssm_pick_stop(cald_ctx* c, const RetinaSsmBufs& S, int V, int K, cald_ssm_pick_fn pick, void* user, int image0, int* h_counts);
RoiArgs roi_args(const RoiBufs& S, const float* const* feat, const BatchPlan* plan, int C, int V, const ProposalBufs& P, bool out16);
PostArgs post_args(const PostBufs& S, const float* pred, int pred_ld, int C, int V, const ProposalBufs& P, const ViewDesc* views,
                   float score_thr, float nms_thr, const DetBuffers& det);
SsmArgs ssm_args(const SsmBufs& S, const float* pred, int pred_ld, int C, int V, const ProposalBufs& P, const ViewDesc* views, float score_thr, int cap);
RetinaArgs retina_args(const RetinaTailBufs& S, const float* const* cls, const float* const* reg, const BatchPlan* plan, const ViewDesc* views,
                       const float* base_anchors, int A, int K, int V, float score_thr, float nms_thr, int per_class, const DetBuffers& det);
inline size_t cut_plan_set_bytes(int V) { return (size_t)(V + 1) * sizeof(LevelSeg) + (size_t)V * sizeof(GatherSet); }
inline long long level_pix(const BatchPlan& P, int l, int V) { return P.seg[l][V].pix_off; }

int arena_reserve(cald_ctx* c, size_t bytes);
int prof_begin(cald_ctx* c, ProfLaunch& t);
int prof_end(cald_ctx* c, ProfLaunch& t, double flops, int tag, const char* fmt, ...);
int conv_refused(const ConvArgs& a);
int run_conv(cald_ctx* c, const ConvArgs& a, double flops);
int pil_resize(cald_ctx* c, const uint8_t* src, int H, int W, uint8_t* dst, int oh, int ow, uint8_t* tmp, int fid = 0);
std::vector<float> pack_w4(const std::vector<float>& w, int Kpad, int CoutPad);
void pack_conv(const std::vector<const float*>& ts, const std::vector<int>& couts, int cin, int cinp, int kh, int kw, int stride, int pad,
// ... 11 lines not shown
```

### cald_amd/csrc/host_logic.h

```cpp
#pragma once
#include <cmath>
#include <cstdint>
#include <cstdio>
#include <cstdlib>
#include <cstring>
#include <vector>

static inline void transform_size(int H, int W, int min_size, int max_size, int* Hr, int* Wr, int* Hp, int* Wp) {
    double mn = (double)(H < W ? H : W), mx = (double)(H > W ? H : W);
    double scale = (double)min_size / mn;
    if (mx * scale > (double)max_size) scale = (double)max_size / mx;
    *Hr = (int)std::floor((double)H * scale);
    *Wr = (int)std::floor((double)W * scale);
    *Hp = ((*Hr + 31) / 32) * 32;
    *Wp = ((*Wr + 31) / 32) * 32;
}

struct PyRandom {
    uint32_t mt[624]; int idx;
    void init_genrand(uint32_t s) {
        mt[0] = s;
        for (int i = 1; i < 624; i++) mt[i] = 1812433253u * (mt[i - 1] ^ (mt[i - 1] >> 30)) + (uint32_t)i;
        idx = 624;
    }
// ... 217 lines not shown
    if (h > n - 1) h = n - 1;
    *lo = l; *hi = h;
    return l <= h;
}
static inline CutSet cut_map(const CutSet& in, int k, int s, int p, int Ho, int Wo) {
    CutSet o; o.n = 0;
    for (int i = 0; i < in.n; i++) {
        CutRect r;
        if (cut_span(in.r[i].x0, in.r[i].x1, k, s, p, Wo, &r.x0, &r.x1) && cut_span(in.r[i].y0, in.r[i].y1, k, s, p, Ho, &r.y0, &r.y1)) o.r[o.n++] = r;
    }
    return o;
}
static inline CutSet cut_window(const CutSet& out, int s, int Hi, int Wi) {
    CutSet o; o.n = 0;
    for (int i = 0; i < out.n; i++) {
        CutRect r = {out.r[i].x0 * s - 1, out.r[i].y0 * s - 1, out.r[i].x1 * s + 1, out.r[i].y1 * s + 1};
        if (r.x0 < 0) r.x0 = 0; if (r.y0 < 0) r.y0 = 0;
        if (r.x1 > Wi - 1) r.x1 = Wi - 1; if (r.y1 > Hi - 1) r.y1 = Hi - 1;
        if (r.x0 <= r.x1 && r.y0 <= r.y1) o.r[o.n++] = r;
    }
    return o;
}
static inline bool cut_resize_span(int a, int b, int n_src, int nr, int* lo, int* hi) {
    const double sc = (double)n_src / (double)nr;
    int l = nr, h = -1;
    for (int y = 0; y < nr; y++) {
        double f = sc * ((double)y + 0.5) - 0.5; if (f < 0.0) f = 0.0;
        const int t0 = (int)f;
        if (t0 + 2 >= a && t0 - 1 <= b) { if (y < l) l = y; h = y; }
    }
    *lo = l; *hi = h;
    return l <= h;
}
static inline void cut_geometry(int H, int W, int Hr, int Wr, int Hp, int Wp, int nrect, const int* rects, int nblk, const int* stride,
                                CutSet* pool1, CutSet* out, CutSet* t1) {
    CutSet s; s.n = 0;
    for (int i = 0; i < nrect && i < CUT_SET_MAX; i++) {
        const int* q = rects + 4 * i;
        if (q[2] <= q[0] || q[3] <= q[1]) continue;
        CutRect r;
        if (cut_resize_span(q[0], q[2] - 1, W, Wr, &r.x0, &r.x1) && cut_resize_span(q[1], q[3] - 1, H, Hr, &r.y0, &r.y1)) s.r[s.n++] = r;
    }
    s = cut_map(s, 7, 2, 3, Hp >> 1, Wp >> 1);
    s = cut_map(s, 3, 2, 1, Hp >> 2, Wp >> 2);
    *pool1 = s;
    int l = 2;
    for (int b = 0; b < nblk; b++) {
        const int lo = l + (stride[b] == 2 ? 1 : 0);
        out[b] = cut_map(s, 3, stride[b], 1, Hp >> lo, Wp >> lo);
        t1[b] = cut_window(out[b], stride[b], Hp >> l, Wp >> l);
        s = out[b]; l = lo;
    }
}
static inline int cut_disjoint(const CutSet& s, CutRect* o, int cap) {
    int ys[2 * CUT_SET_MAX], ny = 0;
    for (int i = 0; i < s.n; i++) { ys[ny++] = s.r[i].y0; ys[ny++] = s.r[i].y1 + 1; }
    for (int i = 1; i < ny; i++) for (int j = i; j > 0 && ys[j] < ys[j - 1]; j--) { const int t = ys[j]; ys[j] = ys[j - 1]; ys[j - 1] = t; }
    int n = 0;
    for (int k = 0; k + 1 < ny; k++) {
        const int ya = ys[k], yb = ys[k + 1] - 1;
        if (ya > yb) continue;
        int x0[CUT_SET_MAX], x1[CUT_SET_MAX], nx = 0;
        for (int i = 0; i < s.n; i++)
            if (s.r[i].y0 <= ya && s.r[i].y1 >= yb) { x0[nx] = s.r[i].x0; x1[nx] = s.r[i].x1; nx++; }
        for (int i = 1; i < nx; i++) for (int j = i; j > 0 && x0[j] < x0[j - 1]; j--) {
            int t = x0[j]; x0[j] = x0[j - 1]; x0[j - 1] = t; t = x1[j]; x1[j] = x1[j - 1]; x1[j - 1] = t;
        }
        for (int i = 0; i < nx;) {
            const int a = x0[i];
            int b = x1[i++];
            while (i < nx && x0[i] <= b + 1) { if (x1[i] > b) b = x1[i]; i++; }
            bool ext = false;
            for (int q = 0; q < n && !ext; q++)
                if (o[q].x0 == a && o[q].x1 == b && o[q].y1 == ya - 1) { o[q].y1 = yb; ext = true; }
            if (ext) continue;
            if (n == cap) return -1;
            o[n++] = {a, ya, b, yb};
        }
    }
    return n;
}
```

### cald_amd/csrc/model.hip

```cpp
#include "host.h"

extern "C" int cald_model_create(cald_ctx* ctx, const cald_model_cfg* cfg, cald_model** out) {
    if (!ctx || !cfg || !out) return fail(CALD_ERR_INVALID, "null argument");
    if (cfg->arch != CALD_ARCH_FRCNN && cfg->arch != CALD_ARCH_RETINANET) return fail(CALD_ERR_INVALID, "unknown arch %d", cfg->arch);
    if (cfg->depth != 50 && cfg->depth != 101) return fail(CALD_ERR_INVALID, "depth must be 50 or 101");
    if (cfg->num_classes < 2 || cfg->num_classes > 256) return fail(CALD_ERR_INVALID, "num_classes out of range");
    if (cfg->rpn_pre_nms_top_n > 1024 || cfg->rpn_post_nms_top_n > CALD_ROI_CAP || cfg->rpn_pre_nms_top_n < 1 || cfg->rpn_post_nms_top_n < 1)
        return fail(CALD_ERR_INVALID, "rpn top-n out of range (pre <= 1024, post <= %d)", CALD_ROI_CAP);
    if (cfg->detections_per_img < 1 || cfg->detections_per_img > 1024) return fail(CALD_ERR_INVALID, "detections_per_img out of range");
    if (cfg->precision != CALD_PRECISION_FP32 && cfg->precision != CALD_PRECISION_F16X3) return fail(CALD_ERR_INVALID, "unknown precision %d", cfg->precision);
    cald_model* m = new cald_model();
    m->ctx = ctx; m->cfg = *cfg;
    {
        const float thr = cfg->box_score_thresh;
        long long per = cfg->num_classes - 1;
        if (thr > 0.0f && std::isfinite(thr)) { const long long lim = (long long)std::ceil(1.0 / (double)thr) - 1; if (lim < per) per = lim < 1 ? 1 : lim; }
        long long need = (long long)CALD_ROI_CAP * per;
        int kc = 1024; while (kc < need) kc <<= 1;
        m->key_cap = kc;
    }
    memset(&m->sweep_det, 0, sizeof(m->sweep_det)); memset(&m->sweep_det2, 0, sizeof(m->sweep_det2));
    *out = m;
    return 0;
}
// ... 244 lines not shown
        for (int i = 0; i < 3; i++) {
            char k[128];
            snprintf(k, sizeof(k), "backbone.fpn.inner_blocks.%d", i);
            if ((rc = make_conv(m, m->fpn_inner[i], {std::string(k) + ".weight"}, {std::string(k) + ".bias"}, "", 1, 0))) return rc;
            snprintf(k, sizeof(k), "backbone.fpn.layer_blocks.%d", i);
            if ((rc = make_conv(m, m->fpn_layer[i], {std::string(k) + ".weight"}, {std::string(k) + ".bias"}, "", 1, 1))) return rc;
        }
        if ((rc = make_conv(m, m->p6, {"backbone.fpn.extra_blocks.p6.weight"}, {"backbone.fpn.extra_blocks.p6.bias"}, "", 2, 1))) return rc;
        if ((rc = make_conv(m, m->p7, {"backbone.fpn.extra_blocks.p7.weight"}, {"backbone.fpn.extra_blocks.p7.bias"}, "", 2, 1))) return rc;
        for (int i = 0; i < 4; i++) {
            char k[128];
            snprintf(k, sizeof(k), "head.classification_head.conv.%d", 2 * i);
            if ((rc = make_conv(m, m->cls_tower[i], {std::string(k) + ".weight"}, {std::string(k) + ".bias"}, "", 1, 1))) return rc;
            snprintf(k, sizeof(k), "head.regression_head.conv.%d", 2 * i);
            if ((rc = make_conv(m, m->reg_tower[i], {std::string(k) + ".weight"}, {std::string(k) + ".bias"}, "", 1, 1))) return rc;
        }
        if ((rc = make_conv(m, m->cls_out, {"head.classification_head.cls_logits.weight"}, {"head.classification_head.cls_logits.bias"}, "", 1, 1))) return rc;
        if ((rc = make_conv(m, m->reg_out, {"head.regression_head.bbox_reg.weight"}, {"head.regression_head.bbox_reg.bias"}, "", 1, 1))) return rc;
        if (m->cls_out.Cout != 9 * m->cfg.num_classes || m->reg_out.Cout != 36)
            return fail(CALD_ERR_INVALID, "RetinaNet heads must have 9*num_classes / 36 outputs (got %d / %d)", m->cls_out.Cout, m->reg_out.Cout);
        std::vector<float> base(5 * 9 * 4);
        const float ratios[3] = {0.5f, 1.0f, 2.0f};
        for (int l = 0; l < 5; l++) {
            const int x = 32 << l;
            const float sizes[3] = {(float)x, (float)(int)((double)x * pow(2.0, 1.0 / 3)), (float)(int)((double)x * pow(2.0, 2.0 / 3))};
            for (int r = 0; r < 3; r++) {
                float hr = sqrtf(ratios[r]), wr = 1.0f / hr;
                for (int sidx = 0; sidx < 3; sidx++) {
                    float ws = wr * sizes[sidx], hs = hr * sizes[sidx];
                    float* b = &base[((l * 9) + r * 3 + sidx) * 4];
                    b[0] = rintf(-ws / 2.0f); b[1] = rintf(-hs / 2.0f); b[2] = rintf(ws / 2.0f); b[3] = rintf(hs / 2.0f);
                }
            }
        }
        if ((rc = upload(m, base, &m->d_anchors))) return rc;
    }
    m->sd.clear();
    m->finalized = true;
    return 0;
}
extern "C" int cald_model_set_rpn_prune(cald_model* m, int on, int* was) {
    if (!m) return fail(CALD_ERR_INVALID, "model is null");
    if (!m->finalized) return fail(CALD_ERR_STATE, "model not finalized");
    if (was) *was = m->prune ? 1 : 0;
    m->prune = on != 0 && m->prune_allowed;
    return 0;
}
extern "C" int cald_model_set_cutout_reuse(cald_model* m, int mode, int* was) {
    if (!m || mode < -1 || mode > 2) return fail(CALD_ERR_INVALID, "bad argument");
    if (was) *was = m->cr.mode;
    m->cr.mode = mode;
    return 0;
}
extern "C" int cald_model_set_row_packing(cald_model* m, int mode, int* was) {
    if (!m || mode < -1 || mode > 1) return fail(CALD_ERR_INVALID, "bad argument");
    if (was) *was = m->row_packing;
    m->row_packing = mode;
    return 0;
}
extern "C" int cald_model_set_look_fuse(cald_model* m, int mode, int* was) {
    if (!m || mode < 0 || mode > 2) return fail(CALD_ERR_INVALID, "bad argument");
    if (was) *was = m->look_fuse;
    m->look_fuse = mode;
    return 0;
}
extern "C" int cald_model_set_box_min_size(cald_model* m, float min_size, float* was) {
    if (!m || !(min_size >= 0.0f)) return fail(CALD_ERR_INVALID, "bad argument");
    if (m->cfg.arch != CALD_ARCH_FRCNN) return fail(CALD_ERR_INVALID, "box_min_size belongs to the Faster R-CNN tail (RetinaNet's always removes small boxes)");
    if (was) *was = m->box_min_size;
    m->box_min_size = min_size;
    return 0;
}
extern "C" int cald_model_set_rpn_prune_capture(cald_model* m, int on) {
    if (!m) return fail(CALD_ERR_INVALID, "model is null");
    if (on && !(m->prune && m->prune_allowed)) return fail(CALD_ERR_STATE, "certified RPN pruning is not active on this model");
    m->prune_capture = on != 0;
    return 0;
}
extern "C" int cald_model_rpn_prune_bound(cald_model* m, float* c1, float* c0) {
    if (!m || !c1 || !c0) return fail(CALD_ERR_INVALID, "null argument");
    if (!m->rpn_conv16.w16) return fail(CALD_ERR_STATE, "the model has no look-ahead layer (not an exact Faster R-CNN model)");
    for (int a = 0; a < 3; a++) { c1[a] = m->prune_c1[a]; c0[a] = m->prune_c0[a]; }
    return 0;
}
extern "C" int cald_model_set_rpn_prune_bound(cald_model* m, const float* c1, const float* c0) {
    if (!m || !c1 || !c0) return fail(CALD_ERR_INVALID, "null argument");
    if (!m->rpn_conv16.w16) return fail(CALD_ERR_STATE, "the model has no look-ahead layer (not an exact Faster R-CNN model)");
    for (int a = 0; a < 3; a++) { m->prune_c1[a] = c1[a]; m->prune_c0[a] = c0[a]; }
    m->prune_bound_voided = true;
    return 0;
}
extern "C" int cald_model_destroy(cald_model* m) {
    if (!m) return 0;
    hipSetDevice(m->ctx->device);
    hipStreamSynchronize(m->ctx->stream);
    for (void* p : m->owned) hipFree(p);
    if (m->sweep_det_views) free_det(m->sweep_det);
    if (m->sweep_det2_views) free_det(m->sweep_det2);
    if (m->ss.dev) hipFree(m->ss.dev);
    if (m->ss.pin) hipHostFree(m->ss.pin);
    if (m->ss.d_aug) hipFree(m->ss.d_aug);
    for (int i = 0; i < 2; i++) { if (m->cr.slot[i]) hipFree(m->cr.slot[i]); if (m->cr.h_gp[i]) hipHostFree(m->cr.h_gp[i]); }
    if (m->cr.d_gp) hipFree(m->cr.d_gp);
    for (int i = 0; i < 2; i++) { if (m->ss.ev_ref[i]) hipEventDestroy(m->ss.ev_ref[i]); if (m->ss.ev_score[i]) hipEventDestroy(m->ss.ev_score[i]); }
    delete m;
    return 0;
// ... 2 lines not shown
```

### cald_amd/csrc/ops.hip

```cpp
#include "host.h"

extern "C" int cald_op_transform_size(int H, int W, int min_size, int max_size, int* Hr, int* Wr, int* Hp, int* Wp) {
    if (H <= 0 || W <= 0 || min_size <= 0 || max_size <= 0) return fail(CALD_ERR_INVALID, "bad sizes");
    transform_size(H, W, min_size, max_size, Hr, Wr, Hp, Wp);
    return 0;
}

extern "C" int cald_op_cutout_rects(uint64_t seed, int H, int W, int N, const float* boxes, int cut_num, int* rects_out, int* n_out) {
    if (cut_num < 0 || cut_num > CALD_MAX_CUT) return fail(CALD_ERR_INVALID, "cut_num must be 0..%d", CALD_MAX_CUT);
    *n_out = cutout_rects(seed, H, W, N, boxes, cut_num, rects_out);
    return 0;
}

extern "C" int cald_op_cutout_geometry(int H, int W, int min_size, int max_size, int nrect, const int* rects, int nblk, const int* strides, int* out) {
    if (H < 1 || W < 1 || nrect < 0 || nrect > CALD_MAX_CUT || (nrect && !rects) || nblk < 0 || nblk > 64 || (nblk && !strides) || !out)
        return fail(CALD_ERR_INVALID, "bad argument");
    int Hr, Wr, Hp, Wp;
    transform_size(H, W, min_size, max_size, &Hr, &Wr, &Hp, &Wp);
    std::vector<CutSet> o(nblk + 1), t(nblk + 1);
    cut_geometry(H, W, Hr, Wr, Hp, Wp, nrect, rects, nblk, strides, &o[0], o.data() + 1, t.data() + 1);
    t[0].n = 0;
    for (int e = 0; e <= nblk; e++)
        for (int k = 0; k < 2; k++) {
            const CutSet& sset = k ? t[e] : o[e];
            int* q = out + (size_t)(2 * e + k) * (1 + 4 * CUT_SET_MAX);
            memset(q, 0, sizeof(int) * (1 + 4 * CUT_SET_MAX));
            q[0] = sset.n;
            for (int i = 0; i < sset.n; i++) { q[1 + 4 * i] = sset.r[i].x0; q[2 + 4 * i] = sset.r[i].y0; q[3 + 4 * i] = sset.r[i].x1; q[4 + 4 * i] = sset.r[i].y1; }
        }
    return 0;
}
static int get_pil(cald_ctx* c, int inSize, int outSize, int fid, PilCoef* out) {
    PilKey key{inSize, outSize, fid};
    auto it = c->pil.find(key);
    if (it == c->pil.end()) {
        std::vector<int> b, k;
        PilCoef pc; pc.ksize = pil_coeffs(inSize, outSize, fid, b, k);
        ScopedDev sd(c->stream); int rc;
        if ((rc = sd.upload(&pc.d_bounds, b.data(), b.size() * sizeof(int))) || (rc = sd.upload(&pc.d_kk, k.data(), k.size() * sizeof(int)))) return rc;
        sd.release();
        it = c->pil.insert(std::make_pair(key, pc)).first;
    }
    *out = it->second;
    return 0;
}
int cald_host::pil_resize(cald_ctx* c, const uint8_t* src, int H, int W, uint8_t* dst, int oh, int ow, uint8_t* tmp, int fid) {
    const uint8_t* cur = src;
    if (ow != W) {
        PilCoef pc; int rc = get_pil(c, W, ow, fid, &pc); if (rc) return rc;
        uint8_t* hdst = (oh != H) ? tmp : dst;
        launch_pil_horizontal(src, H, W, hdst, ow, pc.d_bounds, pc.d_kk, pc.ksize, c->stream);
        cur = hdst;
    }
    if (oh != H) {
        PilCoef pc; int rc = get_pil(c, H, oh, fid, &pc); if (rc) return rc;
        launch_pil_vertical(cur, H, ow, dst, oh, pc.d_bounds, pc.d_kk, pc.ksize, c->stream);
    } else if (ow == W) {
        HIPCHK(hipMemcpyAsync(dst, src, (size_t)H * W * 3, hipMemcpyDeviceToDevice, c->stream));
    }
    return 0;
}
extern "C" int cald_op_pil_resize(cald_ctx* c, const uint8_t* src_dev, int H, int W, uint8_t* dst_dev, int oh, int ow) {
    if (!c || !src_dev || !dst_dev || H <= 0 || W <= 0 || oh <= 0 || ow <= 0) return fail(CALD_ERR_INVALID, "bad arguments");
    ScopedDev sd(c->stream);
    uint8_t* tmp; int rc;
    if ((rc = sd.alloc(&tmp, (size_t)H * ow * 3))) return rc;
    return pil_resize(c, src_dev, H, W, dst_dev, oh, ow, tmp);
}

extern "C" int cald_op_noise_stream(cald_ctx* c, uint64_t seed, const uint8_t* src_dev, int H, int W, int nseg, const int* kinds,
                                    const double* params, void* const* dsts) {
    if (!c || !src_dev || H <= 0 || W <= 0 || !kinds || !params || !dsts) return fail(CALD_ERR_INVALID, "cald_op_noise_stream: bad arguments");
    if (nseg < 1 || nseg > CALD_MAX_NOISE_SEG) return fail(CALD_ERR_INVALID, "cald_op_noise_stream: 1..%d segments", CALD_MAX_NOISE_SEG);
    NoiseJob nj; memset(&nj, 0, sizeof(nj));
    nj.seed = seed; nj.src = src_dev; nj.H = H; nj.W = W; nj.nseg = nseg;
    for (int g = 0; g < nseg; g++) {
        NoiseSeg& sg = nj.seg[g];
        if (!dsts[g]) return fail(CALD_ERR_INVALID, "cald_op_noise_stream: segment %d has no destination", g);
        sg.dst = dsts[g];
        if (kinds[g] == CALD_AUG_GAUSS) {
            if (randn_unsupported(H, W))
                return fail(CALD_ERR_UNSUPPORTED, "GaussianNoise on a %dx%d image: torch.randn of fewer than 16 elements takes torch's scalar path, which is not implemented", H, W);
// ... 658 lines not shown
```

### cald_amd/csrc/sweep.hip

```cpp
#include "host.h"

void cald_host::free_det(DetBuffers& d) {
    hipFree(d.boxes); hipFree(d.scores); hipFree(d.labels); hipFree(d.props); hipFree(d.prob_max); hipFree(d.scores_cls); hipFree(d.count);
    memset(&d, 0, sizeof(d));
}
int cald_host::alloc_det(DetBuffers& d, int V, int cap, int C) {
    memset(&d, 0, sizeof(d));
    d.cap = cap; d.C = C;
    hipError_t e = hipMalloc((void**)&d.boxes, (size_t)V * cap * 16);
    if (e == hipSuccess) e = hipMalloc((void**)&d.scores, (size_t)V * cap * 4);
    if (e == hipSuccess) e = hipMalloc((void**)&d.labels, (size_t)V * cap * 8);
    if (e == hipSuccess) e = hipMalloc((void**)&d.props, (size_t)V * cap * 16);
    if (e == hipSuccess) e = hipMalloc((void**)&d.prob_max, (size_t)V * cap * 4);
    if (e == hipSuccess) e = hipMalloc((void**)&d.scores_cls, (size_t)V * cap * C * 4);
    if (e == hipSuccess) e = hipMalloc((void**)&d.count, (size_t)V * 4);
    if (e != hipSuccess) {
        free_det(d);
        return fail(CALD_ERR_HIP, "hipMalloc of detection buffers (%d views x %d rows x %d classes) failed: %s", V, cap, C, hipGetErrorString(e));
    }
    return 0;
}
static int ensure_det(cald_model* m, DetBuffers& set, int& views, int VT) {
    if (views >= VT) return 0;
    if (views) {
        HIPCHK(hipStreamSynchronize(m->ctx->stream));
        free_det(set);
        views = 0;
    }
    int rc = alloc_det(set, VT, m->det_cap(), m->cfg.num_classes);
    if (rc) return rc;
    views = VT;
    return 0;
}
static DetBuffers det_at(const DetBuffers& D, size_t o) {
    DetBuffers d2 = D;
    const int cap = D.cap, C = D.C;
    d2.boxes += o * cap * 4; d2.scores += o * cap; d2.labels += o * cap; d2.props += o * cap * 4;
    d2.prob_max += o * cap; d2.scores_cls += o * cap * C; d2.count += o;
    return d2;
}
static ViewDesc plain_view(const uint8_t* src, int H, int W) {
    ViewDesc d; memset(&d, 0, sizeof(d));
    d.src = src; d.H = H; d.W = W;
    return d;
}
static std::vector<ViewDesc> ref_views(const uint8_t* const* images_dev, const int* H, const int* W, int i0, int nb) {
    std::vector<ViewDesc> views(nb);
    for (int i = 0; i < nb; i++) views[i] = plain_view(images_dev[i0 + i], H[i0 + i], W[i0 + i]);
    return views;
}

static int sweep_fwd_views() {
    static const int env = getenv("CALD_FWD_VIEWS") ? atoi(getenv("CALD_FWD_VIEWS")) : 96;
    return env < 1 ? 1 : (env > CALD_MAX_VIEWS ? CALD_MAX_VIEWS : env);
}
static int fwd_count(int n) { return (n + sweep_fwd_views() - 1) / sweep_fwd_views(); }
static void fwd_span(int n, int f, int* a0, int* nv) {
    const int n_fw = fwd_count(n);
    *a0 = (int)(((long long)n * f) / n_fw); *nv = (int)(((long long)n * (f + 1)) / n_fw) - *a0;
}
static bool cut_reuse_env() {
    static const bool on = !(getenv("CALD_CUTOUT_REUSE") && atoi(getenv("CALD_CUTOUT_REUSE")) == 0);
    return on;
}
#define CUT_GATHER_MAX_COST 0.7

namespace {
struct PairLayout {
    int P_MAX, B, VT;
    struct Ptrs { int *ref_view, *aug_view, *aug_kind, *pair_img, *ref_sel, *ref_n, *view_img, *view_isref; };
    size_t n_ints() const { return (size_t)P_MAX * 4 + (size_t)B * 51 + (size_t)VT * 2; }
    Ptrs at(int* base) const {
        Ptrs p;
        p.ref_view = base; p.aug_view = p.ref_view + P_MAX; p.aug_kind = p.aug_view + P_MAX; p.pair_img = p.aug_kind + P_MAX;
        p.ref_sel = p.pair_img + P_MAX; p.ref_n = p.ref_sel + (size_t)B * 50; p.view_img = p.ref_n + B; p.view_isref = p.view_img + VT;
        return p;
    }
    ScoreArgs score_args(int* d_base, const DetBuffers& D, const float* d_par, int P, float bp, float* cons) const {
        const Ptrs p = at(d_base);
        ScoreArgs sa; sa.det = D;
        sa.ref_view = p.ref_view; sa.aug_view = p.aug_view; sa.aug_kind = p.aug_kind; sa.pair_img = p.pair_img;
        sa.ref_sel = p.ref_sel; sa.ref_n = p.ref_n; sa.aug_param = d_par; sa.P = P; sa.bp = bp; sa.cons = cons;
        return sa;
    }
};

struct SweepBatch {
    int i0 = 0, nb = 0, P = 0, VV = 0; bool live = false;
    int* h_count; float* h_boxes; int* h_ints; float* h_par; NoiseJob* h_jobs; float* h_cons; float* h_clsc; float* h_vm; float* h_pm;
    std::vector<int> ref_n, pair_img, view_img, pair_aug, view_aug;
    std::vector<char> view_inert;
    std::vector<float> cut_margin;
    bool kept = false;
    std::vector<int> ref_sel, pair_kind, view_isref;
    std::vector<float> pair_par;
    std::vector<ViewDesc> aviews;
};

struct SweepRun {
    cald_model* m; int n_images; const uint8_t* const* images_dev; const int* H; const int* W; const int64_t* pool_pos;
    const cald_sweep_cfg* cfg; double* consistency_out; double* cls_corr_out; float* margins_out; bool force_dense;
    cald_ctx* c = nullptr;
    bool audit = false, prune_ok = false, retina = false, reuse = false;
    int C = 0, cap = 0, A = 0, B = 0, VT = 0, NB = 0, P_MAX = 0, cut_a = -1;
    PairLayout lay{0, 0, 0}; size_t n_ints = 0;
    DetBuffers* DS[2] = {nullptr, nullptr};
    int* d_ints = nullptr; float *d_par = nullptr, *d_cons = nullptr, *d_clsc = nullptr; NoiseJob* d_jobs = nullptr; unsigned long long* d_lsum = nullptr;
    float *d_vm[2] = {nullptr, nullptr}, *d_pm = nullptr;
    SweepBatch bt[2];
    int nblk = 0, blk_lin[CUT_MAX_BLOCKS], blk_lout[CUT_MAX_BLOCKS], blk_stage[CUT_MAX_BLOCKS], blk_stride[CUT_MAX_BLOCKS];
    std::vector<BatchPlan> rplan;

    static size_t al(size_t b) { return (b + 255) & ~(size_t)255; }

    int setup() {
        if (!m || !images_dev || !H || !W || !pool_pos || !cfg || !consistency_out || !cls_corr_out) return fail(CALD_ERR_INVALID, "null argument");
        audit = margins_out != nullptr;
        prune_ok = !audit && !force_dense;
        if (!m->finalized) return fail(CALD_ERR_STATE, "model not finalized");
        c = m->ctx;
        HIPCHK(hipSetDevice(c->device));
        C = m->cfg.num_classes; cap = m->det_cap();
        A = cfg->n_augs;
        if (A < 0 || A > CALD_MAX_AUGS) return fail(CALD_ERR_INVALID, "n_augs %d outside [0, %d]", A, CALD_MAX_AUGS);
        int n_noise = 0; bool any_gauss = false;
        for (int a = 0; a < A; a++) {
            const int k = cfg->augs[a].kind;
            if (k < CALD_AUG_FLIP || k > CALD_AUG_ROTATE) return fail(CALD_ERR_INVALID, "augmentation %d: unknown kind %d", a, k);
            if (k == CALD_AUG_CUTOUT && (cfg->augs[a].param < 1.0 || cfg->augs[a].param > (double)CALD_MAX_CUT))
                return fail(CALD_ERR_INVALID, "cutout: cut_num must be in [1, %d]", CALD_MAX_CUT);
            if (k == CALD_AUG_RESIZE && !(cfg->augs[a].param > 0.0)) return fail(CALD_ERR_INVALID, "resize: ratio must be positive");
            n_noise += (k == CALD_AUG_GAUSS || k == CALD_AUG_SALT_PEPPER);
            any_gauss |= k == CALD_AUG_GAUSS;
        }
        if (n_noise > CALD_MAX_NOISE_SEG) return fail(CALD_ERR_INVALID, "at most %d GaussianNoise / SaltPepperNoise views per image", CALD_MAX_NOISE_SEG);
        if (any_gauss)
            for (int i = 0; i < n_images; i++)
                if (randn_unsupported(H[i], W[i]))
                    return fail(CALD_ERR_UNSUPPORTED, "GaussianNoise on image %d (%dx%d): torch.randn of fewer than 16 elements takes torch's scalar path, which is not implemented", i, H[i], W[i]);
        B = cfg->batch_images > 0 ? cfg->batch_images : 64;
        if (B > CALD_MAX_VIEWS) B = CALD_MAX_VIEWS;
        VT = B * (1 + A);
        NB = (n_images + B - 1) / B;
        const bool two_sets = NB > 1;
        { int rc0 = ensure_det(m, m->sweep_det, m->sweep_det_views, VT); if (rc0) return rc0; }
        if (two_sets) { int rc0 = ensure_det(m, m->sweep_det2, m->sweep_det2_views, VT); if (rc0) return rc0; }
        DS[0] = &m->sweep_det; DS[1] = two_sets ? &m->sweep_det2 : &m->sweep_det;
        P_MAX = B * (A > 0 ? A : 1);
        lay = PairLayout{P_MAX, B, VT}; n_ints = lay.n_ints();
        cald_model::SweepScratch& S = m->ss;
        const size_t dev_need = al(n_ints * 4) + al((size_t)P_MAX * 12 * 4) + al((size_t)P_MAX * 4) + al((size_t)VT * (C - 1) * 4) + al(sizeof(NoiseJob) * B) +
                                al(sizeof(unsigned long long) * P_MAX) + 2 * al((size_t)VT * CALD_VM * 4) + al((size_t)P_MAX * 2 * 4);
        const size_t pin_set = al((size_t)VT * 4) + al((size_t)B * cap * 16) + al(n_ints * 4) + al((size_t)P_MAX * 12 * 4) + al(sizeof(NoiseJob) * B) +
                               al((size_t)P_MAX * 4) + al((size_t)VT * (C - 1) * 4) + al((size_t)VT * CALD_VM * 4) + al((size_t)P_MAX * 2 * 4);
        if (dev_need > S.dev_bytes || 2 * pin_set > S.pin_bytes) {
            HIPCHK(hipStreamSynchronize(c->stream));
            if (S.dev) { hipFree(S.dev); S.dev = nullptr; S.dev_bytes = 0; }
            if (S.pin) { hipHostFree(S.pin); S.pin = nullptr; S.pin_bytes = 0; }
            HIPCHK(hipMalloc((void**)&S.dev, dev_need)); S.dev_bytes = dev_need;
            HIPCHK(hipHostMalloc((void**)&S.pin, 2 * pin_set)); S.pin_bytes = 2 * pin_set;
        }
        for (int i = 0; i < 2; i++) {
            if (!S.ev_ref[i]) HIPCHK(hipEventCreateWithFlags(&S.ev_ref[i], hipEventDisableTiming));
            if (!S.ev_score[i]) HIPCHK(hipEventCreateWithFlags(&S.ev_score[i], hipEventDisableTiming));
        }
        { Bump b(S.dev, false); d_ints = b.get<int>(n_ints); d_par = b.get<float>((size_t)P_MAX * 12); d_cons = b.get<float>(P_MAX);
          d_clsc = b.get<float>((size_t)VT * (C - 1)); d_jobs = b.get<NoiseJob>(B); d_lsum = b.get<unsigned long long>(P_MAX);
          d_vm[0] = b.get<float>((size_t)VT * CALD_VM); d_vm[1] = b.get<float>((size_t)VT * CALD_VM); d_pm = b.get<float>((size_t)P_MAX * 2); }
        for (int q = 0; q < 2; q++) {
            Bump b(S.pin + (size_t)q * pin_set, false);
            bt[q].h_count = b.get<int>(VT); bt[q].h_boxes = b.get<float>((size_t)B * cap * 4); bt[q].h_ints = b.get<int>(n_ints);
            bt[q].h_par = b.get<float>((size_t)P_MAX * 12); bt[q].h_jobs = b.get<NoiseJob>(B); bt[q].h_cons = b.get<float>(P_MAX);
            bt[q].h_clsc = b.get<float>((size_t)VT * (C - 1));
            bt[q].h_vm = b.get<float>((size_t)VT * CALD_VM); bt[q].h_pm = b.get<float>((size_t)P_MAX * 2);
        }
        if (m->prune && prune_ok) HIPCHK(hipMemsetAsync(c->d_prune_check, 0, 8, c->stream));
        retina = m->cfg.arch == CALD_ARCH_RETINANET;
        for (int a = 0; a < A && cut_a < 0; a++) if (cfg->augs[a].kind == CALD_AUG_CUTOUT) cut_a = a;
        for (int b = 0, layer = 0, l = 2; b < (int)m->blocks.size() && layer < 3 && nblk < CUT_MAX_BLOCKS; b++) {
            const Bottleneck& Bk = m->blocks[b];
            blk_stride[nblk] = Bk.c2.stride; blk_lin[nblk] = l; l += Bk.c2.stride == 2 ? 1 : 0; blk_lout[nblk] = l; blk_stage[nblk] = layer;
            nblk++;
            if (Bk.layer_end) layer++;
        }
        reuse = (m->cr.mode < 0 ? cut_reuse_env() : m->cr.mode != 0) && cut_a >= 0 && !audit && m->cfg.precision == CALD_PRECISION_FP32 && nblk < CUT_MAX_BLOCKS;
        rplan.resize(reuse ? 1 : 0);
        return 0;
    }

    void plan_of(int nv, const ViewDesc* vs, BatchPlan& P) const {
        int hp[CALD_MAX_VIEWS][2];
        for (int v = 0; v < nv; v++) { int Hr, Wr; transform_size(vs[v].H, vs[v].W, m->cfg.min_size, m->cfg.max_size, &Hr, &Wr, &hp[v][0], &hp[v][1]); }
        build_plan(P, nv, vs, hp, retina);
    }
    size_t retain_layout(const BatchPlan& P, int nv, char* base, float** out) const {
        size_t off = 0;
        for (int b = 0; b < nblk; b++) {
            if (out) out[b] = reinterpret_cast<float*>(base + off);
            off += al((size_t)level_pix(P, blk_lout[b], nv) * (size_t)m->blocks[b].c3.Cout * 4);
        }
        return off;
    }

    int enqueue_ref(int k) {
        SweepBatch& b = bt[k & 1];
        b.i0 = k * B; b.nb = (n_images - b.i0 < B) ? n_images - b.i0 : B; b.live = true; b.P = 0; b.VV = b.nb;
        std::vector<ViewDesc> views = ref_views(images_dev, H, W, b.i0, b.nb);
        const DetBuffers& D = *DS[k & 1];
        FwdReuse ru; b.kept = false;
        if (reuse) {
            plan_of(b.nb, views.data(), rplan[0]);
            const size_t need = retain_layout(rplan[0], b.nb, nullptr, nullptr);
            cald_model::CutReuse& R = m->cr;
            const int q = k & 1;
            if (need > R.cap[q]) {
                HIPCHK(hipStreamSynchronize(c->stream));
                if (R.slot[q]) hipFree(R.slot[q]);
                R.slot[q] = nullptr; R.cap[q] = 0;
                if (hipMalloc((void**)&R.slot[q], need + (need >> 3)) != hipSuccess) { (void)hipGetLastError(); R.slot[q] = nullptr; }
                else R.cap[q] = need + (need >> 3);
            }
            if (R.slot[q]) { ru.mode = 1; ru.nblk = nblk; retain_layout(rplan[0], b.nb, R.slot[q], ru.out); b.kept = true; }
            else c->cut_fallbacks++;
        }
        int r = forward_model(m, b.nb, views.data(), D, audit ? d_vm[k & 1] : nullptr, prune_ok, b.kept ? &ru : nullptr);
        if (r) return r;
        if (hipMemcpyAsync(b.h_count, D.count, (size_t)b.nb * 4, hipMemcpyDeviceToHost, c->stream) != hipSuccess ||
            hipMemcpyAsync(b.h_boxes, D.boxes, (size_t)b.nb * cap * 16, hipMemcpyDeviceToHost, c->stream) != hipSuccess ||
            hipEventRecord(m->ss.ev_ref[k & 1], c->stream) != hipSuccess) return fail(CALD_ERR_HIP, "D2H of reference detections failed");
        return 0;
    }

    int build_aug_views(int k) {
        SweepBatch& b = bt[k & 1];
        cald_model::SweepScratch& S = m->ss;
        const int nb = b.nb, i0 = b.i0;
        if (hipEventSynchronize(S.ev_ref[k & 1]) != hipSuccess) return fail(CALD_ERR_HIP, "reference forward failed: %s", hipGetErrorString(hipGetLastError()));
        const int* h_count = b.h_count; const float* h_boxes = b.h_boxes;
        b.ref_sel.assign((size_t)B * 50, 0); b.pair_aug.clear(); b.pair_kind.clear(); b.view_isref.assign(VT, 0);
        b.ref_n.assign(B, 0); b.pair_img.clear(); b.view_img.assign(VT, 0); b.cut_margin.assign(B, INFINITY);
        b.view_aug.assign(VT, 0); b.view_inert.assign(VT, 0);
        b.pair_par.clear(); b.aviews.clear();
        int njobs = 0;
        size_t need = 0;
        for (int i = 0; i < nb; i++) {
            if (h_count[i] == 0) continue;
            const int Hi = H[i0 + i], Wi = W[i0 + i];
            for (int a = 0; a < A; a++) {
                const int kd = cfg->augs[a].kind; const double prm = cfg->augs[a].param;
                if (kd == CALD_AUG_SALT_PEPPER) need += al((size_t)Hi * Wi * 3);
                else if (kd == CALD_AUG_GAUSS) need += al((size_t)Hi * Wi * 3 * sizeof(float));
                else if (kd == CALD_AUG_COLOR_ADJUST) need += 2 * al((size_t)Hi * Wi * 3);
                else if (kd == CALD_AUG_RESIZE) {
                    const int ow = (int)((double)Wi * prm), oh = (int)((double)Hi * prm);
                    if (ow < 1 || oh < 1) return fail(CALD_ERR_INVALID, "resize ratio %g empties a %dx%d image", prm, Hi, Wi);
                    need += al((size_t)oh * ow * 3) + al((size_t)Hi * ow * 3);
                } else if (kd == CALD_AUG_ROTATE) {
                    int fx[6], nh, nw; pil_rotate_setup(Hi, Wi, prm, fx, &nh, &nw);
                    need += al((size_t)nh * nw * 3) + al((size_t)nh * Wi * 3) + al((size_t)Hi * Wi * 3);
                }
            }
        }
        if (need > S.aug_cap) {
            HIPCHK(hipStreamSynchronize(c->stream));
            if (S.d_aug) hipFree(S.d_aug);
            S.d_aug = nullptr; S.aug_cap = 0;
            if (hipMalloc((void**)&S.d_aug, need + (need >> 2)) != hipSuccess) return fail(CALD_ERR_HIP, "hipMalloc of the augmentation arena failed");
            S.aug_cap = need + (need >> 2);
        }
        size_t aug_off = 0;
        auto take = [&](size_t bytes) { uint8_t* p = S.d_aug + aug_off; aug_off += al(bytes); return p; };
        int r = 0;
        for (int i = 0; i < nb; i++) {
            b.view_img[i] = i; b.view_isref[i] = 1;
            const int n = h_count[i];
            b.ref_n[i] = subsample_indices(n, &b.ref_sel[(size_t)i * 50]);
            if (n == 0) continue;
            const int Hi = H[i0 + i], Wi = W[i0 + i];
            const uint64_t seed = (uint64_t)cfg->base_seed * 1000003ull + (uint64_t)pool_pos[i0 + i];
            float sub[50 * 4];
            for (int q = 0; q < b.ref_n[i]; q++) memcpy(sub + 4 * q, &h_boxes[((size_t)i * cap + b.ref_sel[(size_t)i * 50 + q]) * 4], 16);
            int cur_a = 0;
// ... 8 lines not shown
            NoiseJob nj; memset(&nj, 0, sizeof(nj)); nj.seed = seed; nj.src = images_dev[i0 + i]; nj.H = Hi; nj.W = Wi;
            for (int a = 0; a < A && !r; a++) {
                const int kd = cfg->augs[a].kind; const double prm = cfg->augs[a].param;
                float par[12] = {0};
                cur_a = a;
                if (kd == CALD_AUG_FLIP) { ViewDesc v = base; v.flip = 1; par[0] = (float)Wi; add_view(v, 1, par); }
                else if (kd == CALD_AUG_GAUSS) {
                    NoiseSeg& sg = nj.seg[nj.nseg++]; sg.kind = 0; sg.p0 = (float)prm; sg.p1 = 0.0f;
                    sg.dst = take((size_t)Hi * Wi * 3 * sizeof(float));
                    ViewDesc v = base; v.noise = reinterpret_cast<const float*>(sg.dst); add_view(v, 0, nullptr);
                } else if (kd == CALD_AUG_SALT_PEPPER) {
                    NoiseSeg& sg = nj.seg[nj.nseg++]; sg.kind = 1; sg.p0 = (float)(prm / 2.0); sg.p1 = (float)(1.0 - prm / 2.0);
                    sg.dst = take((size_t)Hi * Wi * 3);
                    ViewDesc v = base; v.src = reinterpret_cast<const uint8_t*>(sg.dst); add_view(v, 0, nullptr);
                } else if (kd == CALD_AUG_COLOR_ADJUST) {
                    uint8_t* tmp = take((size_t)Hi * Wi * 3); uint8_t* dst = take((size_t)Hi * Wi * 3);
                    launch_color_adjust(images_dev[i0 + i], Hi, Wi, (float)prm, tmp, d_lsum + b.pair_img.size(), dst, c->stream);
                    ViewDesc v = base; v.src = dst; add_view(v, 0, nullptr);
                } else if (kd == CALD_AUG_COLOR_SWAP) {
                    ViewDesc v = base; v.swap = pyrng.randbelow(6); add_view(v, 0, nullptr);
                } else if (kd == CALD_AUG_CUTOUT) {
                    ViewDesc v = base;
                    float cm = INFINITY;
                    v.nrect = cutout_rects(pyrng, Hi, Wi, b.ref_n[i], sub, (int)prm, v.rects, &cm);
                    if (cm < b.cut_margin[i]) b.cut_margin[i] = cm;
                    add_view(v, 0, nullptr);
                } else if (kd == CALD_AUG_RESIZE) {
                    const int ow = (int)((double)Wi * prm), oh = (int)((double)Hi * prm);
                    uint8_t* dst = take((size_t)oh * ow * 3); uint8_t* tmp = take((size_t)Hi * ow * 3);
                    if ((r = pil_resize(c, images_dev[i0 + i], Hi, Wi, dst, oh, ow, tmp, 0))) break;
                    par[0] = (float)prm; add_view(plain_view(dst, oh, ow), 2, par);
                } else if (kd == CALD_AUG_ROTATE) {
                    int fx[6], nh, nw; pil_rotate_setup(Hi, Wi, prm, fx, &nh, &nw);
                    uint8_t* rot = take((size_t)nh * nw * 3); uint8_t* tmp = take((size_t)nh * Wi * 3); uint8_t* dst = take((size_t)Hi * Wi * 3);
                    launch_affine_nearest(images_dev[i0 + i], Hi, Wi, rot, nh, nw, fx, c->stream);
                    if ((r = pil_resize(c, rot, nh, nw, dst, Hi, Wi, tmp, 1))) break;
                    ViewDesc v = base; v.src = dst;
                    rotate_box_params(Hi, Wi, prm, nw, nh, par);
                    add_view(v, 3, par);
                }
            }
            if (r) return r;
            if (nj.nseg) b.h_jobs[njobs++] = nj;
        }
        if (njobs) {
            if (hipMemcpyAsync(d_jobs, b.h_jobs, sizeof(NoiseJob) * njobs, hipMemcpyHostToDevice, c->stream) != hipSuccess) return fail(CALD_ERR_HIP, "H2D of noise jobs failed");
            launch_noise_stream(d_jobs, njobs, c->stream);
        }
        return 0;
    }

    int cut_plan(int k, int V, const ViewDesc* vs, FwdReuse& ru) {
        cald_model::CutReuse& R = m->cr;
        const size_t per = cut_plan_set_bytes(V), total = per * 2 * (size_t)nblk;
        if (!R.d_gp) {
            const size_t cap = cut_plan_set_bytes(CALD_MAX_VIEWS) * 2 * CUT_MAX_BLOCKS;
            HIPCHK(hipMalloc((void**)&R.d_gp, cap));
            HIPCHK(hipHostMalloc((void**)&R.h_gp[0], cap)); HIPCHK(hipHostMalloc((void**)&R.h_gp[1], cap));
        }
        plan_of(V, vs, rplan[0]);
        const BatchPlan& P = rplan[0];
        char* const h = R.h_gp[k & 1];
        std::vector<CutSet> g_out((size_t)V * nblk), g_t1((size_t)V * nblk);
        for (int v = 0; v < V; v++) {
            int Hr, Wr, Hp, Wp; CutSet pool1;
            transform_size(vs[v].H, vs[v].W, m->cfg.min_size, m->cfg.max_size, &Hr, &Wr, &Hp, &Wp);
            cut_geometry(vs[v].H, vs[v].W, Hr, Wr, Hp, Wp, vs[v].nrect, vs[v].rects, nblk, blk_stride, &pool1, &g_out[(size_t)v * nblk], &g_t1[(size_t)v * nblk]);
        }
        auto kf = [](const ConvLayer& L) { return (double)L.Cout * (double)(L.KH * L.KW * L.CinTrue); };
        double cost_g[3] = {0, 0, 0}, cost_d[3] = {0, 0, 0}, rows_g[3] = {0, 0, 0}, rows_d[3] = {0, 0, 0};
        for (int b = 0; b < nblk; b++)
            for (int kind = 0; kind < 2; kind++) {
                const int lvl = kind ? blk_lin[b] : blk_lout[b];
                LevelSeg* sg = reinterpret_cast<LevelSeg*>(h + (size_t)(2 * b + kind) * per);
                GatherSet* gs = reinterpret_cast<GatherSet*>(reinterpret_cast<char*>(sg) + (size_t)(V + 1) * sizeof(LevelSeg));
                int tiles = 0; double rows = 0.0;
                for (int v = 0; v < V; v++) {
                    LevelSeg L = P.seg[lvl][v]; L.tile_start = tiles; sg[v] = L;
                    CutRect rr[CALD_GATHER_RECTS];
                    int n = cut_disjoint(kind ? g_t1[(size_t)v * nblk + b] : g_out[(size_t)v * nblk + b], rr, CALD_GATHER_RECTS);
                    if (n < 0) { n = 1; rr[0] = {0, 0, L.W - 1, L.H - 1}; }
                    GatherSet& G = gs[v]; memset(&G, 0, sizeof(G));
                    G.nr = n;
                    for (int q = 0; q < n; q++) {
                        G.x0[q] = rr[q].x0; G.y0[q] = rr[q].y0; G.w[q] = rr[q].x1 - rr[q].x0 + 1;
                        G.cum[q + 1] = G.cum[q] + G.w[q] * (rr[q].y1 - rr[q].y0 + 1);
                    }
                    tiles += (G.cum[n] + 127) / 128; rows += (double)G.cum[n];
                }
                sg[V] = P.seg[lvl][V]; sg[V].tile_start = tiles;
                ru.tiles[b][kind] = tiles; ru.rows[b][kind] = rows;
                const Bottleneck& Bk = m->blocks[b];
                const double w = kind ? kf(Bk.c1) : kf(Bk.c2) + kf(Bk.c3) + (Bk.has_down ? kf(Bk.down) : 0.0);
                const double nconv = kind ? 1.0 : (Bk.has_down ? 3.0 : 2.0), dense = (double)level_pix(P, lvl, V);
                const int st = blk_stage[b];
                cost_g[st] += 128.0 * tiles * w; cost_d[st] += dense * w;
                rows_g[st] += rows * nconv; rows_d[st] += dense * nconv;
            }
        for (int st = 0; st < 3; st++) {
            ru.gather[st] = m->cr.mode != 2 && cost_g[st] <= CUT_GATHER_MAX_COST * cost_d[st];
            c->cut_rows[st] += ru.gather[st] ? rows_g[st] : rows_d[st]; c->cut_dense[st] += rows_d[st];
        }
        if (hipMemcpyAsync(R.d_gp, h, total, hipMemcpyHostToDevice, c->stream) != hipSuccess) return fail(CALD_ERR_HIP, "H2D of the cut_out gather plan failed");
        ru.mode = 2; ru.nblk = nblk; ru.d_gp = R.d_gp;
        retain_layout(P, V, m->cr.slot[k & 1], ru.out);
        c->cut_batches++;
        return 0;
    }

    int enqueue_aug_forwards(int k) {
        SweepBatch& b = bt[k & 1];
        const DetBuffers& D = *DS[k & 1];
        const int nb = b.nb, na = (int)b.aviews.size();
        int r, n_rest = na, rest_slot = nb;
        ViewDesc* rest_views = b.aviews.data();
        std::vector<ViewDesc> rest;
        int n_cut = 0;
        for (int j = 0; j < na; j++) n_cut += b.view_aug[nb + j] == cut_a;
        b.VV = nb + na;
        if (b.kept && n_cut > 0 && 2 * nb + (na - n_cut) <= VT) {
            std::vector<ViewDesc> cutv(nb);
            std::vector<int> slot(na), nimg(VT, 0), naug(VT, 0);
            std::vector<char> has(nb, 0), ninert(VT, 0);
            for (int i = 0; i < nb; i++) nimg[i] = i;
            int nr2 = 0;
            for (int j = 0; j < na; j++) {
                const int img = b.view_img[nb + j];
                if (b.view_aug[nb + j] == cut_a) { slot[j] = nb + img; cutv[img] = b.aviews[j]; has[img] = 1; }
                else { slot[j] = 2 * nb + nr2++; rest.push_back(b.aviews[j]); }
                nimg[slot[j]] = img; naug[slot[j]] = b.view_aug[nb + j];
            }
            for (int i = 0; i < nb; i++)
                if (!has[i]) {
                    cutv[i] = plain_view(images_dev[b.i0 + i], H[b.i0 + i], W[b.i0 + i]);
                    nimg[nb + i] = i; naug[nb + i] = cut_a; ninert[nb + i] = 1;
                }
            for (size_t p = 0; p < b.pair_aug.size(); p++) b.pair_aug[p] = slot[b.pair_aug[p] - nb];
            b.view_img = nimg; b.view_aug = naug; b.view_inert = ninert;
            FwdReuse ru;
            if ((r = cut_plan(k, nb, cutv.data(), ru))) return r;
            if ((r = forward_model(m, nb, cutv.data(), det_at(D, (size_t)nb), nullptr, prune_ok, &ru))) return r;
            b.VV = 2 * nb + nr2; n_rest = nr2; rest_slot = 2 * nb; rest_views = rest.data();
        } else if (b.kept) {
            c->cut_fallbacks++;
        }
        for (int f = 0; f < fwd_count(n_rest); f++) {
            int a0, nv; fwd_span(n_rest, f, &a0, &nv);
            const size_t o = (size_t)(rest_slot + a0);
            if ((r = forward_model(m, nv, rest_views + a0, det_at(D, o), audit ? d_vm[k & 1] + o * CALD_VM : nullptr, prune_ok))) return r;
        }
        return 0;
    }

    int enqueue_scoring(int k) {
        SweepBatch& b = bt[k & 1];
        const DetBuffers& D = *DS[k & 1];
        const int P = (int)b.pair_img.size(), VV = b.VV;
        b.P = P;
// ... 30 lines not shown
        for (int i = 0; i < nb; i++)
            std::stable_sort(img_views[i].begin(), img_views[i].end(), [&](int x, int y) { return b.view_aug[x] < b.view_aug[y]; });
        for (int i = 0; i < nb; i++) {
            double* cc = cls_corr_out + (size_t)(b.i0 + i) * (C - 1);
            const int nvw = 1 + (int)img_views[i].size();
            for (int k2 = 0; k2 < C - 1; k2++) {
                double sm = (double)b.h_clsc[(size_t)i * (C - 1) + k2];
                for (int v : img_views[i]) sm += (double)b.h_clsc[(size_t)v * (C - 1) + k2];
                cc[k2] = sm / (double)nvw;
            }
            if (b.h_count[i] == 0 || img_pairs[i].empty()) { consistency_out[b.i0 + i] = 0.0; continue; }
            std::vector<double> cs;
            for (int p : img_pairs[i]) cs.push_back((double)b.h_cons[p]);
            consistency_out[b.i0 + i] = np_sum(cs.data(), (int)cs.size()) / (double)cs.size();
        }
        if (audit) {
            for (int i = 0; i < nb; i++) {
                float* mg = margins_out + (size_t)(b.i0 + i) * CALD_N_MARGINS;
                for (int q = 0; q < CALD_N_MARGINS; q++) mg[q] = INFINITY;
                auto take_view = [&](int v) { for (int q = 0; q <= VM_POST_CAP; q++) { const float t = b.h_vm[(size_t)v * CALD_VM + q]; if (t < mg[q]) mg[q] = t; } };
                take_view(i);
                for (int v : img_views[i]) take_view(v);
                mg[CALD_MARGIN_REF_SUBSAMPLE] = b.h_vm[(size_t)i * CALD_VM + VM_POST_SUBORDER];
                for (int p : img_pairs[i]) {
                    if (b.h_pm[2 * p] < mg[CALD_MARGIN_ARGMAX]) mg[CALD_MARGIN_ARGMAX] = b.h_pm[2 * p];
                    if (b.h_pm[2 * p + 1] != 0.0f) {
                        const float t = b.h_vm[(size_t)b.pair_aug[p] * CALD_VM + VM_POST_TOP2];
                        if (t < mg[CALD_MARGIN_ZERO_ROW]) mg[CALD_MARGIN_ZERO_ROW] = t;
                    }
                }
                mg[CALD_MARGIN_CUTOUT] = b.cut_margin[i];
            }
        }
        b.live = false;
        return 0;
    }

    int run() {
        int rc = setup();
        if (rc) return rc;
        if (NB > 0) rc = enqueue_ref(0);
        for (int k = 0; k < NB && !rc; k++) {
            if (k + 1 < NB) {
                if ((rc = finish(k - 1))) break;
                if ((rc = enqueue_ref(k + 1))) break;
            }
            if ((rc = build_aug_views(k)) || (rc = enqueue_aug_forwards(k)) || (rc = enqueue_scoring(k))) break;
        }
        for (int k = (NB >= 2 ? NB - 2 : 0); k < NB && !rc; k++) rc = finish(k);
        if (rc) hipStreamSynchronize(c->stream);
        return rc;
    }
};
}

static int sweep_checked(cald_model* m, int n_images, const uint8_t* const* images_dev, const int* H, const int* W,
                         const int64_t* pool_pos, const cald_sweep_cfg* cfg, double* consistency_out, double* cls_corr_out, float* margins_out) {
    SweepRun first{m, n_images, images_dev, H, W, pool_pos, cfg, consistency_out, cls_corr_out, margins_out, false};
    int rc = first.run();
    if (rc || !(m->prune && first.prune_ok && first.NB > 0)) return rc;
    cald_ctx* c = m->ctx;
    float chk[2] = {0.0f, 0.0f};
    HIPCHK(hipMemcpy(chk, c->d_prune_check, 8, hipMemcpyDeviceToHost));
    const bool range = chk[1] != 0.0f;
    if (chk[0] == chk[0] && !range && !m->prune_bound_voided) c->prune_worst = chk[0] > c->prune_worst ? chk[0] : c->prune_worst;
    if (!(chk[0] <= 1.0f) || range) {
        c->prune_fallbacks++;
        SweepRun dense{m, n_images, images_dev, H, W, pool_pos, cfg, consistency_out, cls_corr_out, margins_out, true};
        rc = dense.run();
    }
    return rc;
}
extern "C" int cald_sweep(cald_model* m, int n_images, const uint8_t* const* images_dev, const int* H, const int* W,
                          const int64_t* pool_pos, const cald_sweep_cfg* cfg, double* consistency_out, double* cls_corr_out) {
    return sweep_checked(m, n_images, images_dev, H, W, pool_pos, cfg, consistency_out, cls_corr_out, nullptr);
}
extern "C" int cald_sweep_audit(cald_model* m, int n_images, const uint8_t* const* images_dev, const int* H, const int* W,
                                const int64_t* pool_pos, const cald_sweep_cfg* cfg, double* consistency_out, double* cls_corr_out,
                                float* margins_out) {
    if (!margins_out) return fail(CALD_ERR_INVALID, "null argument");
    return sweep_checked(m, n_images, images_dev, H, W, pool_pos, cfg, consistency_out, cls_corr_out, margins_out);
}


extern "C" int cald_sweep_ltc(cald_model* m, int n_images, const uint8_t* const* images_dev, const int* H, const int* W,
                              int batch_images, double* uncertainty_out) {
    if (!m || !images_dev || !H || !W || !uncertainty_out) return fail(CALD_ERR_INVALID, "null argument");
    if (!m->finalized) return fail(CALD_ERR_STATE, "model not finalized");
    if (m->cfg.arch != CALD_ARCH_FRCNN) return fail(CALD_ERR_INVALID, "lt_c needs the Faster R-CNN outputs (props)");
    cald_ctx* c = m->ctx;
    HIPCHK(hipSetDevice(c->device));
    int B = batch_images > 0 ? batch_images : 64; if (B > CALD_MAX_VIEWS) B = CALD_MAX_VIEWS;
    { int rc0 = ensure_det(m, m->sweep_det, m->sweep_det_views, B); if (rc0) return rc0; }
    float* d_out = nullptr; HIPCHK(hipMalloc((void**)&d_out, (size_t)B * 4));
    std::vector<float> h(B);
    int rc = 0;
    for (int i0 = 0; i0 < n_images && !rc; i0 += B) {
        const int nb = (n_images - i0 < B) ? n_images - i0 : B;
        std::vector<ViewDesc> views = ref_views(images_dev, H, W, i0, nb);
        if ((rc = forward_model(m, nb, views.data(), m->sweep_det))) break;
        launch_lt_uncertainty(m->sweep_det, nb, d_out, c->stream);
        if (hipMemcpyAsync(h.data(), d_out, (size_t)nb * 4, hipMemcpyDeviceToHost, c->stream) != hipSuccess ||
            hipStreamSynchronize(c->stream) != hipSuccess) { rc = fail(CALD_ERR_HIP, "lt_c scoring failed: %s", hipGetErrorString(hipGetLastError())); break; }
        for (int i = 0; i < nb; i++) uncertainty_out[i0 + i] = (double)h[i];
    }
    hipStreamSynchronize(c->stream); hipFree(d_out);
// ... 198 lines not shown
```

### cald_amd/detector.py

```python
import ctypes as C

import numpy as np
import torch

from . import _ffi

_CTX = {}


def get_ctx(device_index=None):
    if not torch.cuda.is_available():
        raise RuntimeError("cald_amd needs a visible MI355X (torch.cuda.is_available() is False); there is no CPU fallback")
    if device_index is None:
        device_index = torch.cuda.current_device()
    if device_index not in _CTX:
        h = C.c_void_p()
        stream = torch.cuda.current_stream(device_index).cuda_stream
        _ffi.check(_ffi.lib().cald_ctx_create(device_index, C.c_void_p(stream), C.byref(h)))
        _CTX[device_index] = h
    return _CTX[device_index]


_SIDE_CTX = {}

# ... 82 lines not shown
            raise RuntimeError("cald_amd detectors live on the MI355X only")
        self._device = dev.index if dev.index is not None else (torch.cuda.current_device() if torch.cuda.is_available() else 0)
        return self

    def cuda(self, device=None):
        return self.to("cuda" if device is None else "cuda:%d" % device)

    def state_dict(self):
        from collections import OrderedDict
        if self._trainer is not None and self.training:
            return OrderedDict((k, v.detach().cpu()) for k, v in self._trainer.state_dict().items())
        return OrderedDict((k, torch.from_numpy(np.array(v, dtype=np.float32))) for k, v in (self._state or {}).items())

    def load_state_dict(self, sd, strict=True):
        self._state = {k: (v.detach().cpu().float().numpy() if hasattr(v, "detach") else np.asarray(v, np.float32))
                       for k, v in sd.items() if not k.endswith("num_batches_tracked")}
        self._destroy()
        self._trainer = self._train_fn = None
        if self.training:
            self._ensure_trainer()
        return self

    def _destroy(self):
        if self._handle is not None:
            _ffi.lib().cald_model_destroy(self._handle)
            self._handle = None

    def __del__(self):
        try:
            self._destroy()
        except Exception:
            pass

    def handle(self):
        if self._handle is None:
            if self._state is None:
                raise RuntimeError("no weights: call load_state_dict() first (cald_train.py:356)")
            L = _ffi.lib()
            ctx = self._ctx if getattr(self, "_ctx", None) is not None else get_ctx(self._device)
            h = C.c_void_p()
            _ffi.check(L.cald_model_create(ctx, C.byref(self.cfg), C.byref(h)))
            for k, v in self._state.items():
                a = np.ascontiguousarray(v, dtype=np.float32)
                if a.ndim == 0:
                    continue
                shape = (C.c_int64 * a.ndim)(*a.shape)
                _ffi.check(L.cald_model_load_tensor(h, k.encode(), _ffi.ptr(a), shape, a.ndim))
            _ffi.check(L.cald_model_finalize(h))
            if self.box_min_size > 0.0:
                _ffi.check(L.cald_model_set_box_min_size(h, self.box_min_size, None))
            self._handle = h
        return self._handle

    def forward_views(self, views):
        L = _ffi.lib()
        h = self.handle()
        n = len(views)
        dev = views[0][0].device
        Cn = self.num_classes
        cap = self.cfg.detections_per_img * (Cn if self.arch == 1 else 1)
        out = dict(boxes=torch.empty((n, cap, 4), device=dev), scores=torch.empty((n, cap), device=dev),
                   labels=torch.empty((n, cap), dtype=torch.int64, device=dev), props=torch.empty((n, cap, 4), device=dev),
                   prob_max=torch.empty((n, cap), device=dev), scores_cls=torch.empty((n, cap, Cn), device=dev),
                   count=torch.zeros((n,), dtype=torch.int32, device=dev))
        arr = (_ffi.View * n)()
        for i, view in enumerate(views):
            img, flip, rects = view[:3]
            noise = view[3] if len(view) > 3 else None
            assert img.dtype == torch.uint8 and img.is_cuda and img.is_contiguous() and img.shape[2] == 3
            arr[i].image_dev = img.data_ptr(); arr[i].H = img.shape[0]; arr[i].W = img.shape[1]
            if noise is not None:
                assert noise.dtype == torch.float32 and noise.is_cuda and noise.is_contiguous() and tuple(noise.shape) == (3, img.shape[0], img.shape[1])
                arr[i].noise_dev = noise.data_ptr()
            arr[i].flip = int(bool(flip)); arr[i].nrect = 0 if rects is None else len(rects)
            if rects is not None:
                for j, r in enumerate(np.asarray(rects, np.int32).reshape(-1)):
                    arr[i].rects[j] = int(r)
        d = _ffi.Dets(out["boxes"].data_ptr(), out["scores"].data_ptr(), out["labels"].data_ptr(), out["props"].data_ptr(),
                      out["prob_max"].data_ptr(), out["scores_cls"].data_ptr(), out["count"].data_ptr(), cap)
        _ffi.check(L.cald_forward(h, n, arr, C.byref(d)))
        counts = out["count"].cpu().tolist()
        res = []
        for i, k in enumerate(counts):
            keys = ("boxes", "labels", "scores", "props", "prob_max", "scores_cls") if self.arch == 0 else \
                   ("boxes", "scores", "labels", "scores_cls", "prob_max")
            res.append({key: out[key][i, :k] for key in keys})
        return res

    def __call__(self, images, targets=None):
        if self.training:
            if targets is None:
                raise ValueError("In training mode, targets should be passed")
            return self._train_fn(images, targets)
        views = []
        for img in images:
            if img.dtype == torch.uint8:
                u8 = img if img.shape[-1] == 3 else img.permute(1, 2, 0)
                views.append((u8.contiguous().cuda(), False, None))
                continue
            x = img.detach().to(torch.float32).cuda().contiguous()
            if not bool(torch.isfinite(x).all()):
                raise ValueError("non-finite pixel values in the input image")
            g = (x * 255.0).round().clamp(0, 255).to(torch.uint8)
            base = _u8_over_255(x.device)[g.long()]
            rem = x - base
            if not bool(torch.equal(base + rem, x)):
                raise RuntimeError("float input is not representable as uint8 grid + float32 remainder")
            noise = rem.contiguous() if bool((rem != 0).any()) else None
            views.append((g.permute(1, 2, 0).contiguous(), False, None, noise))
        return self.forward_views(views)

    def set_rpn_prune(self, on):
        was = C.c_int(0)
        _ffi.check(_ffi.lib().cald_model_set_rpn_prune(self.handle(), int(bool(on)), C.byref(was)))
        return bool(was.value)

    def set_look_fuse(self, mode):
        was = C.c_int(0)
        _ffi.check(_ffi.lib().cald_model_set_look_fuse(self.handle(), int(mode), C.byref(was)))
        return was.value

    def set_rpn_prune_capture(self, on):
        _ffi.check(_ffi.lib().cald_model_set_rpn_prune_capture(self.handle(), int(bool(on))))

    def rpn_prune_bound(self):
        import numpy as np
        c1 = np.zeros(3, np.float32); c0 = np.zeros(3, np.float32)
        _ffi.check(_ffi.lib().cald_model_rpn_prune_bound(self.handle(), _ffi.ptr(c1), _ffi.ptr(c0)))
        return c1, c0

    def set_rpn_prune_bound(self, c1, c0):
        import numpy as np
        c1 = np.ascontiguousarray(c1, np.float32); c0 = np.ascontiguousarray(c0, np.float32)
        assert c1.shape == (3,) and c0.shape == (3,)
        _ffi.check(_ffi.lib().cald_model_set_rpn_prune_bound(self.handle(), _ffi.ptr(c1), _ffi.ptr(c0)))

    def debug_tensor(self, name, view=0):
        shape = (C.c_int64 * 3)()
        cap = 1 << 26
        buf = np.empty(cap, np.float32)
        _ffi.check(_ffi.lib().cald_debug_tensor(self.handle(), name.encode(), view, _ffi.ptr(buf), cap, shape))
        n = shape[0] * shape[1] * shape[2]
        return buf[:n].reshape(shape[0], shape[1], shape[2]).copy()


def fasterrcnn_resnet50_fpn_feature(pretrained=False, progress=True, num_classes=91, pretrained_backbone=True, **kwargs):
    return HipDetector(num_classes, depth=50, **kwargs)


def fasterrcnn_resnet101_fpn_feature(pretrained=False, progress=True, num_classes=91, pretrained_backbone=True, **kwargs):
    return HipDetector(num_classes, depth=101, **kwargs)


def retinanet_resnet50_fpn_cal(pretrained=False, progress=True, num_classes=91, pretrained_backbone=True,
                               score_thresh=0.05, nms_thresh=0.5, detections_per_img=300, **kwargs):
    return HipDetector(num_classes, depth=50, box_score_thresh=score_thresh, box_nms_thresh=nms_thresh,
                       box_detections_per_img=detections_per_img, arch=1, **kwargs)


def from_torch_module(task_model):
    sd = task_model.state_dict()
    tr = getattr(task_model, "transform", None)
    min_size = getattr(tr, "min_size", 800)
# ... 22 lines not shown
```

### include/cald_hip.h

```cpp
#ifndef CALD_HIP_H
#define CALD_HIP_H
#include <stddef.h>
#include <stdint.h>
#ifdef __cplusplus
extern "C" {
#endif

typedef struct cald_ctx cald_ctx;
typedef struct cald_model cald_model;

#define CALD_OK 0
#define CALD_ERR_INVALID (-1)
#define CALD_ERR_HIP (-2)
#define CALD_ERR_STATE (-3)
#define CALD_ERR_MISSING_WEIGHT (-4)
#define CALD_ERR_UNSUPPORTED (-5)

#define CALD_PRECISION_FP32 0
#define CALD_PRECISION_F16X3 1

#define CALD_ARCH_FRCNN 0
#define CALD_ARCH_RETINANET 1

const char* cald_last_error(void);
// ... 109 lines not shown
typedef struct cald_lossnet cald_lossnet;
int cald_lossnet_create(cald_ctx* ctx, cald_lossnet** out);
int cald_lossnet_load_tensor(cald_lossnet* ln, const char* key, const float* data, const int64_t* shape, int ndim);
int cald_lossnet_finalize(cald_lossnet* ln);
int cald_lossnet_destroy(cald_lossnet* ln);
typedef struct cald_ll_cfg {
    int batch_views;
    int levels[4];
} cald_ll_cfg;
int cald_sweep_ll(cald_model* m, cald_lossnet* ln, int n_images, const uint8_t* const* images_dev, const int* H, const int* W,
                  const int* group, const cald_ll_cfg* cfg, double* uncertainty_out, float* pooled_out);

int cald_train_gap(cald_ctx* ctx, int N, const float* const* maps, const int* level_hw, float* pooled);
typedef struct cald_lossnet_tensors {
    float* fc_w[4];
    float* fc_b[4];
    float* lin_w;
    float* lin_b;
} cald_lossnet_tensors;
int cald_lossnet_train_fwd(cald_ctx* ctx, int B, int D, const cald_lossnet_tensors* params, const float* pooled, float* hidden, float* pred);
int cald_lossnet_train_bwd(cald_ctx* ctx, int B, int D, const cald_lossnet_tensors* params, const float* pooled, const float* hidden,
                           const float* g_pred, float* gh_scratch, const cald_lossnet_tensors* grads, int accumulate, float* g_pooled);
int cald_loss_pred_loss(cald_ctx* ctx, int B, const float* input, const float* target, float margin, int per_pair, const float* g_up_dev,
                        float* loss_out, float* terms_out, float* grad_out);

typedef struct cald_vaal cald_vaal;
int cald_vaal_create(cald_ctx* ctx, cald_vaal** out);
int cald_vaal_load_tensor(cald_vaal* v, const char* key, const float* data, const int64_t* shape, int ndim);
int cald_vaal_finalize(cald_vaal* v);
int cald_vaal_destroy(cald_vaal* v);
#define CALD_VAAL_BN_BATCH 0
#define CALD_VAAL_BN_RUNNING 1
typedef struct cald_vaal_cfg {
    int bn_mode;
    int batch_images;
} cald_vaal_cfg;
int cald_sweep_vaal(cald_ctx* ctx, cald_vaal* v, int n_images, const uint8_t* const* images_dev, const int* H, const int* W,
                    const cald_vaal_cfg* cfg, float* preds_out, float* mu_out);

int cald_op_vaal_resize(cald_ctx* ctx, const uint8_t* image, int H, int W, float* out);
int cald_op_vaal_bn_relu(cald_ctx* ctx, const float* x, long long x_floats, int n, int HW, int C, const float* gamma, const float* beta,
                         float* out);
int cald_op_vaal_fc_mu(cald_vaal* v, int n, const float* act, float* mu_out);
int cald_op_vaal_head(cald_vaal* v, int n, const float* mu, float* preds_out);
int cald_op_gap(cald_ctx* ctx, const float* x, int H, int W, int C, float* mean_out);
int cald_op_lossnet(cald_lossnet* ln, int n, const float* pooled, float* out);
int cald_op_consistency(cald_ctx* ctx, int N, const float* aug_box, const float* ref_scores_cls, const float* ref_pm,
                        int M, const float* boxes, const float* scores_cls, const float* pm, int C, float bp,
                        float* consistency_out);
int cald_op_cls_corr(cald_ctx* ctx, int n, const float* scores, const int64_t* labels, int C, float* out);
int cald_op_pil_resize(cald_ctx* ctx, const uint8_t* src_dev, int H, int W, uint8_t* dst_dev, int oh, int ow);
int cald_op_cutout_rects(uint64_t seed, int H, int W, int N, const float* boxes, int cut_num, int* rects_out, int* n_out);
int cald_op_cutout_geometry(int H, int W, int min_size, int max_size, int nrect, const int* rects, int nblk, const int* strides, int* out);
int cald_op_augment(cald_ctx* ctx, int kind, double param, uint64_t seed, const uint8_t* src_dev, int H, int W,
                    int n_boxes, const float* boxes, void* dst_dev, float* boxes_out, int* aux_out);
int cald_op_noise_stream(cald_ctx* ctx, uint64_t seed, const uint8_t* src_dev, int H, int W, int nseg, const int* kinds,
                         const double* params, void* const* dsts);
int cald_op_frcnn_postprocess(cald_ctx* ctx, int R, int C, const float* logits, const float* deltas, const float* proposals,
                              int Hr, int Wr, int Ho, int Wo, float score_thr, float nms_thr, int det_max,
                              float* boxes_out, float* scores_out, int64_t* labels_out, float* props_out, float* prob_max_out,
                              float* scores_cls_out, int* n_out);
int cald_op_frcnn_postprocess_min(cald_ctx* ctx, int R, int C, const float* logits, const float* deltas, const float* proposals,
                                  int Hr, int Wr, int Ho, int Wo, float score_thr, float nms_thr, int det_max, float box_min_size,
                                  float* boxes_out, float* scores_out, int64_t* labels_out, float* props_out, float* prob_max_out,
                                  float* scores_cls_out, int* n_out);
int cald_op_ssm_postprocess(cald_ctx* ctx, int R, int C, const float* logits, const float* deltas, const float* proposals,
                            int Hr, int Wr, int Ho, int Wo, float score_thr, int det_max,
                            int* al_out, int* n_out, float* boxes_out, float* scores_out, int8_t* labels_out);
int cald_op_retina_postprocess(cald_ctx* ctx, const float* const* cls, const float* const* reg, const int* level_hw, int A, int K,
                               const float* base_anchors, int Hp, int Wp, int Hr, int Wr, int Ho, int Wo,
                               float score_thr, float nms_thr, int per_class,
                               float* boxes_out, float* scores_out, int64_t* labels_out, float* prob_max_out,
                               float* scores_cls_out, int* n_out);
int cald_op_retina_ssm_postprocess(cald_ctx* ctx, const float* const* cls, const float* const* reg, const int* level_hw, int A, int K,
                                   const float* base_anchors, int Hp, int Wp, int Hr, int Wr, int Ho, int Wo,
                                   float score_thr, float nms_thr, int per_class, cald_ssm_pick_fn pick, void* user,
                                   int* al_out, int* n_out, int* counts_out, float* boxes_out, float* scores_out, int8_t* labels_out);
#define CALD_PRUNE_PROBE_MAX_VIEWS 8
typedef struct {
    int V, guard;
    int hw[2][CALD_PRUNE_PROBE_MAX_VIEWS][2];
    int pre_n, head_ld;
    float c1[3], c0[3];
    const float* energy[2];
    const float* exact[2];
    float* head[2];
    float* pnorm[2];
    uint32_t* tau_key;
    int* row_map[2][2];
    int* nsel[2];
    float check[2];
    uint64_t stat[4];
} cald_rpn_prune_probe;
int cald_op_rpn_prune(cald_ctx* ctx, cald_rpn_prune_probe* p);
int cald_op_roi_align(cald_ctx* ctx, const float* const* feats, const int* level_hw, int C, int R, const float* rois, float* out);
int cald_op_conv2d(cald_ctx* ctx, const float* in, int H, int W, int Cin, const float* weight, int Cout, int KH, int KW,
                   int stride, int pad, const float* bias, const float* bn_scale, const float* bn_shift,
                   const float* residual, int relu, float* out);
int cald_op_conv2d_f16x3(cald_ctx* ctx, const float* in, int H, int W, int Cin, const float* weight, int Cout, int KH, int KW,
                         int stride, int pad, const float* bias, const float* bn_scale, const float* bn_shift,
                         const float* residual, int relu, float* out);
#define CALD_PROBE_MAX_VIEWS 8
#define CALD_PROBE_MAX_RECTS 8
typedef struct cald_conv_probe {
    int V;
    int in_hw[CALD_PROBE_MAX_VIEWS][2];
// ... 4 lines not shown
    int nrect[CALD_PROBE_MAX_VIEWS];
    int rect[CALD_PROBE_MAX_VIEWS][CALD_PROBE_MAX_RECTS][4];
    int Cin, Cout, KH, KW, stride, pad, relu, in_relu, out_ld;
    int cin_true;
    const float* weight;
    const float* bias;
    const float* bn_scale;
    const float* bn_shift;
    const float* in;
    const uint32_t* in16;
    const float* residual;
    const float* up;
    int ex16;
    const float* mask;
    const int* row_map;
    float* out; int64_t out_n;
    uint32_t* out16; int64_t out16_n;
    float* energy4; int64_t energy4_n;
    const float* head_w; const float* head_b;
    float* head_out; int64_t head_out_n; int head_ld;
    int row_packing;
} cald_conv_probe;
#define CALD_PROBE_PACK_AUTO 0
#define CALD_PROBE_PACK_OFF 1
#define CALD_PROBE_PACK_ON 2
int cald_op_conv_probe(cald_ctx* ctx, int precision, cald_conv_probe* probs, int n, int path, int tile, char* kernel, int kernel_cap);
int cald_op_row_pack_lookup(int V, const int* in_hw, const int* out_hw, int Cin, int out_ld, int64_t n, const int64_t* rows,
                            int* view_out, int64_t* local_out, int64_t* packed_rows_out);
int cald_op_mfma_f16(cald_ctx* ctx, const uint16_t* A, const uint16_t* B, const uint32_t* C, uint32_t* D, int64_t n);
int cald_op_conv_bench(cald_ctx* ctx, int n_views, int H, int W, int Cin, int Cout, int KH, int stride, int pad, int residual,
                       int relu, int iters, int group, double* ms_out, double* tflops_out);
int cald_op_transform_size(int H, int W, int min_size, int max_size, int* Hr, int* Wr, int* Hp, int* Wp);
int cald_debug_tensor(cald_model* m, const char* name, int view, float* host_out, int64_t capacity, int64_t* shape3);

#define CALD_JPEG_BASELINE 0
#define CALD_JPEG_GPU_EXTENDED 1
#define CALD_JPEG_HOST_ONLY 2
int cald_jpeg_info(const uint8_t* data, size_t size, int* H, int* W, int* ncomp);
int cald_jpeg_decode_batch(cald_ctx* ctx, int n, const uint8_t* const* data, const size_t* sizes, uint8_t* const* out_dev);
int cald_jpeg_probe(const uint8_t* data, size_t size, int* H, int* W, int* ncomp, int* kind);
int cald_jpeg_decode_batch_any(cald_ctx* ctx, int n, const uint8_t* const* data, const size_t* sizes, uint8_t* const* out_dev);
int cald_jpeg_decode_host(const uint8_t* data, size_t size, uint8_t* out_host);

int cald_profile_enable(cald_ctx* ctx, int on);
int cald_profile_read(cald_ctx* ctx, double* gemm_ms, double* gemm_flops, int64_t* gemm_launches, double* total_ms);
int cald_profile_prune(cald_ctx* ctx, double* lookahead_ms, double* lookahead_flops, double* selected_fraction_p2_p3, double* worst_bound_ratio,
                       double* pruned_flops);
int cald_profile_prune_fallbacks(cald_ctx* ctx, int64_t* n);
int cald_model_set_cutout_reuse(cald_model* m, int mode, int* was);
int cald_model_set_look_fuse(cald_model* m, int mode, int* was);
int cald_model_set_row_packing(cald_model* m, int mode, int* was);
int cald_model_set_box_min_size(cald_model* m, float min_size, float* was);
int cald_profile_cutout(cald_ctx* ctx, double* rows3, double* dense_rows3, int64_t* batches, int64_t* fallbacks);
int cald_profile_roi_rows(cald_ctx* ctx, double* mean_rows_per_view, int64_t* views);
int cald_profile_dump(cald_ctx* ctx, const char* path);

int cald_train_packed_floats(int Cout, int Cin, int KH, int KW, int CinK, int mode, int64_t* floats_out);
int cald_train_pack_conv(cald_ctx* ctx, const float* weight, const float* bias, const float* bn_scale, const float* bn_shift,
                         int Cout, int Cin, int KH, int KW, int CinK, int mode, float* packed);
typedef struct cald_pack_job {
    const float *weight, *bias, *bn_scale, *bn_shift;
    int Cout, Cin, KH, KW, CinK, mode;
    float* packed;
} cald_pack_job;
typedef struct cald_pack_plan cald_pack_plan;
int cald_train_pack_plan_scratch_floats(int n, const cald_pack_job* jobs, int64_t* floats_out);
int cald_train_pack_plan_create(cald_ctx* ctx, int n, const cald_pack_job* jobs, float* scratch, int64_t scratch_floats, cald_pack_plan** plan_out);
int cald_train_pack_plan_run(cald_ctx* ctx, const cald_pack_plan* plan);
int cald_train_pack_plan_destroy(cald_pack_plan* plan);
int cald_train_conv(cald_ctx* ctx, int N, int H, int W, const float* in, int CinK, const float* packed, int Cout, int Cin,
                    int KH, int KW, int stride, int pad, int mode, int flags, const float* residual, const float* up,
                    int Hup, int Wup, const float* mask, float* out, int out_ld);
int cald_train_conv_group(cald_ctx* ctx, int n, int N, const int* hw, const float* const* ins, int CinK, const float* const* packed,
                          int Cout, int Cin, int KH, int KW, int stride, int pad, int mode, int flags, const float* const* masks,
                          float* const* outs, int out_ld);
int cald_train_conv_wgrad(cald_ctx* ctx, int N, int H, int W, const float* x, int Cin, int ldx, const float* g, int Cout, int ldg,
                          int KH, int KW, int stride, int pad, const float* row_scale, float* dw, float* db, int accumulate);
int cald_train_linear_wgrad(cald_ctx* ctx, int R, const float* x, int K, const float* g, int Cout, int ldg, int taps,
                            float* dw, float* db, int accumulate);
enum { CALD_WGRAD_POINTWISE = 0, CALD_WGRAD_TABLE = 1, CALD_WGRAD_GENERAL = 2, CALD_WGRAD_GENERAL32 = 3, CALD_WGRAD_WIDE = 4 };
enum { CALD_WGRAD_REDUCE_FLAT = 0, CALD_WGRAD_REDUCE_TAPS = 1 };
typedef struct cald_wgrad_plan {
    int variant, reduce;
    int MT, JT;
    long long S, chunk;
    long long csplit, rows_per_block;
    long long scratch_bytes;
    char kernel[48], reduce_kernel[32];
} cald_wgrad_plan;
int cald_train_wgrad_plan(long long Q, int N, int H, int W, int Cin, int ldx, int Cout, int ldg, int KH, int KW, int stride, int pad,
                          int red_taps, cald_wgrad_plan* out);
int cald_train_relu_bwd(cald_ctx* ctx, long long rows, int C, float* g, const float* act, const float* scale);
int cald_train_add(cald_ctx* ctx, long long n, float* dst, const float* a, const float* b);
int cald_train_dilate(cald_ctx* ctx, int N, int Ho, int Wo, int C, int s, int Hd, int Wd, const float* g, float* out);
int cald_train_upsample_bwd(cald_ctx* ctx, int N, int Hf, int Wf, int Hc, int Wc, int C, const float* fine, float* coarse);
int cald_train_rpn_proposals(cald_ctx* ctx, int N, int Hp, int Wp, const int* image_sizes, const float* const* heads,
                             const int* level_hw, int head_ld, int pre_n, int post_n, float nms_thr, float min_size,
                             float* proposals_out, int* counts_out);
int cald_train_roi_sample_host(int N, const int* slots, const int* n_gt, const int* counts, const int32_t* matched,
                               const int64_t* gt_labels, const double* keys, int batch, double pos_fraction, int pred_ld, int num_classes,
                               int64_t* keep_rows, int64_t* gt_sel, int64_t* labels_out, float* img_col, int64_t* pos_rows,
                               int64_t* pred_idx, int* R_out, int* n_pos_out, int* per_image_out);
int cald_train_roi_gather(cald_ctx* ctx, const float* table, const float* gts, const int64_t* idx, int cap, int R, int n_pos,
                          float wx, float wy, float ww, float wh, float* rois_out, float* box_tgt_out);
int cald_train_anchors(cald_ctx* ctx, int kind, int Hp, int Wp, const int* level_hw, float* anchors_out);
int cald_train_match(cald_ctx* ctx, int n_boxes, const float* boxes, int n_gt, const float* gt, float hi, float lo,
// ... 48 lines not shown
```

Baseline: 174.7.

## Extend cutout reuse to FPN outputs with gathered-row FPN group convs

Cutout reuse now also keeps the reference view's FPN outputs, with their fp16 pair and energy extras. For cutout views it recomputes only the FPN output rows whose receptive field touches the cut rectangles, using a new grouped gathered-row conv kernel variant that can also write the pruning extras. The aim is to skip dense FPN 3x3 convs on unchanged regions. In exchange it needs more retained memory (with a retention cap), gather-plan geometry on the host, and a cost heuristic that chooses between gathered and dense paths.

```diff
diff --git a/cald_amd/_ffi.py b/cald_amd/_ffi.py
--- a/cald_amd/_ffi.py
+++ b/cald_amd/_ffi.py
@@ -127,6 +127,7 @@
     "cald_profile_prune_fallbacks": (C.c_int, [C.c_void_p, C.POINTER(C.c_int64)]),
     "cald_model_destroy": (C.c_int, [C.c_void_p]),
     "cald_forward": (C.c_int, [C.c_void_p, C.c_int, C.POINTER(View), C.POINTER(Dets)]),
+    "cald_debug_cutout_forward": (C.c_int, [C.c_void_p, C.c_int, C.POINTER(View), C.POINTER(Dets), C.c_int]),
     "cald_sweep": (C.c_int, [C.c_void_p, C.c_int, C.POINTER(C.c_void_p), c_i, c_i, c_i64, C.POINTER(SweepCfg), c_d, c_d]),
     "cald_sweep_audit": (C.c_int, [C.c_void_p, C.c_int, C.POINTER(C.c_void_p), c_i, c_i, c_i64, C.POINTER(SweepCfg), c_d, c_d, c_f]),
     "cald_sweep_ltc": (C.c_int, [C.c_void_p, C.c_int, C.POINTER(C.c_void_p), c_i, c_i, C.c_int, c_d]),
@@ -197,6 +198,9 @@
     "cald_profile_roi_rows": (C.c_int, [C.c_void_p, c_d, c_i64]),
     "cald_profile_cutout": (C.c_int, [C.c_void_p, c_d, c_d, c_i64, c_i64]),
     "cald_model_set_cutout_reuse": (C.c_int, [C.c_void_p, C.c_int, c_i]),
+    "cald_profile_cutout_stages": (C.c_int, [C.c_void_p, c_d, c_d, c_d, c_d, c_i64]),
+    "cald_model_set_cutout_retention_cap": (C.c_int, [C.c_void_p, C.c_int64, c_i64]),
+    "cald_op_cutout_fpn_geometry": (C.c_int, [C.c_int, C.c_int, C.c_int, C.c_int, C.c_int, c_i, C.c_int, c_i, c_i]),
     "cald_model_set_look_fuse": (C.c_int, [C.c_void_p, C.c_int, c_i]),
     "cald_model_set_row_packing": (C.c_int, [C.c_void_p, C.c_int, c_i]),
     "cald_model_set_box_min_size": (C.c_int, [C.c_void_p, C.c_float, c_f]),
diff --git a/cald_amd/csrc/conv_p4.hip b/cald_amd/csrc/conv_p4.hip
--- a/cald_amd/csrc/conv_p4.hip
+++ b/cald_amd/csrc/conv_p4.hip
@@ -4,7 +4,7 @@
 typedef int i32x4 __attribute__((ext_vector_type(4)));
 typedef float f32x4 __attribute__((ext_vector_type(4)));
 
-template <int EPI, bool MASK, int TM, int TN, bool GATHER = false>
+template <int EPI, bool MASK, int TM, int TN, bool GATHER = false, bool GEXTRA = false>
 __device__ __forceinline__ void p4_epilogue(const ConvArgs& a, const f32x16 (&acc)[TM][TN], float* smem, const int v, const LevelSeg& so,
                                             const int m0, const int Mv, const int n0, const bool straddle = false) {
     constexpr int BM = 128, WN = 2;
@@ -76,7 +76,8 @@
             for (int jj = 0; jj < 4; jj++) go[4 * q + jj] = nok ? so4[jj] + n * 4 : 0x7FFF0000;
         }
     };
-    constexpr bool EXTRA = EPI == 0 && !MASK && !GATHER;
+    static_assert(!GEXTRA || (GATHER && EPI == 0 && !MASK), "the pruning's extras on gathered rows: EPI 0 only");
+    constexpr bool EXTRA = EPI == 0 && !MASK && (!GATHER || GEXTRA);
     const bool want16 = EXTRA && a.out16 != nullptr, wantE = EXTRA && TN == 2 && a.energy4 != nullptr;
     unsigned char* const out16_v = want16 ? reinterpret_cast<unsigned char*>(a.out16) + so.pix_off * (long long)out_ld * 4 : nullptr;
     const __amdgpu_buffer_rsrc_t rsS = __builtin_amdgcn_make_buffer_rsrc((void*)(want16 ? (void*)out16_v : (void*)out_v), 0, valid_b, 0x00020000);
@@ -174,6 +175,15 @@
                 gather_offs(i, n, nok, go);
 #pragma unroll
                 for (int r = 0; r < 16; r++) __builtin_amdgcn_raw_buffer_store_b32(__builtin_bit_cast(unsigned, val[r]), rsO, go[r], 0, 0);
+                if (GEXTRA && want16) {
+                    const int dn = h16_pair_off(nc) - n * 4;
+#pragma unroll
+                    for (int r = 0; r < 16; r++) {
+                        const unsigned w = h16_split(val[r]);
+                        const unsigned pw = h16_pair_word(w, h16_partner(w), odd);
+                        __builtin_amdgcn_raw_buffer_store_b32(pw, rsS, nok ? go[r] + dn : 0x7FFF0000, 0, 0);
+                    }
+                }
             } else {
 #pragma unroll
                 for (int r = 0; r < 16; r++)
@@ -184,7 +194,7 @@
 #pragma unroll
                     for (int r = 0; r < 16; r++) sq[i][r] = sq[i][r] + (nok ? val[r] * val[r] : 0.0f);
                 }
-                if (want16) {
+                if (want16 && !GATHER) {
                     const int poff = h16_pair_off(nc);
 #pragma unroll
                     for (int r = 0; r < 16; r++) {
@@ -198,6 +208,7 @@
     }
     if (EXTRA) {
         if (wantE) {
+            const int pix_b = GATHER ? s_src[wm * TM * 32 + lane] : 0;
             __syncthreads();
             float* const red = smem + wave * (64 * 33);
 #pragma unroll
@@ -209,7 +220,7 @@
 #pragma unroll
             for (int q = 0; q < 32; q++) e = e + red[lane * 33 + q];
             const int m = m0 + wm * TM * 32 + lane;
-            if (m < Mv) a.energy4[(so.pix_off + m) * 4 + (n0 / (64 * TN)) * 2 + wn] = e;
+            if (m < Mv) a.energy4[(so.pix_off + (GATHER ? pix_b / row_b : m)) * 4 + (n0 / (64 * TN)) * 2 + wn] = e;
         }
     }
 }
@@ -220,6 +231,8 @@
     constexpr bool MASK = (EPIX & 4) != 0;
     constexpr bool FUSE = (EPIX & 8) != 0;
     constexpr bool GATHER = (EPIX & 16) != 0;
+    constexpr bool GEXTRA = (EPIX & 32) != 0;
+    static_assert(!GEXTRA || GATHER, "the extras bit rides on the gathered-rows bit");
     static_assert(!(GATHER && (FUSE || MASK || C4)), "gathered rows: plain EPI 0 / 1 kernels only");
     constexpr int BM = 128, BN = 64 * TN, BK = 16, TM = 2, WN = 2;
     constexpr int TILE_A = 2 * BM * 8, TILE_F = TILE_A + 2 * BN * 8;
@@ -654,7 +667,7 @@
             }
         }
     } else {
-        p4_epilogue<EPI, MASK, TM, TN, GATHER>(a, acc, smem, v, so, m0, Mv, n0, CAN_PACK && straddle);
+        p4_epilogue<EPI, MASK, TM, TN, GATHER, GEXTRA>(a, acc, smem, v, so, m0, Mv, n0, CAN_PACK && straddle);
     }
     if (trace && tid == 0) {
         trace[3] = __builtin_amdgcn_s_memtime();
@@ -685,7 +698,7 @@
 static inline bool p4_refuses(const ConvArgs& a) {
     if (!a.w4 || !a.out || a.in16 || a.ex16 || a.CoutPad % 64 != 0 || (a.residual && a.up)) return true;
     const bool extra = a.out16 || a.energy4;
-    if (extra && (a.residual || a.up || a.mask || a.gather)) return true;
+    if (extra && (a.residual || a.up || a.mask)) return true;
     if (a.energy4 && a.CoutPad != 256) return true;
     if (a.row_map && (a.residual || a.up || a.mask || a.gather)) return true;
     return false;
@@ -721,8 +734,9 @@
     for (int i = 0; i < n; i++) {
         const ConvArgs a = p4_tiled(p[i]);
         if (p4_refuses(a) || !p4_tile_ok(a, wide, f) || (a.CoutPad % 128 == 0) != (p[0].CoutPad % 128 == 0)) return nullptr;
-        if (a.Cin % 16 != 0 || a.KH * a.KW > 32 || a.residual || a.up || a.gather) return nullptr;
-        if ((a.mask != nullptr) != (p[0].mask != nullptr)) return nullptr;
+        if (a.Cin % 16 != 0 || a.KH * a.KW > 32 || a.residual || a.up) return nullptr;
+        if ((a.mask != nullptr) != (p[0].mask != nullptr) || (a.gather != nullptr) != (p[0].gather != nullptr)) return nullptr;
+        if (a.gather && (!wide || p4_taps(a) != 9 || a.mask || a.in_relu || a.dyn_rows || a.row_map)) return nullptr;
         if (a.mask && (a.out16 || a.energy4)) return nullptr;
         g.blk0[i] = blk; blk += p4_grid_mtiles(a) * (a.CoutPad / (wide ? 128 : 64)); g.p[i] = a;
     }
@@ -733,7 +747,8 @@
 #define P4_GROUP(EV, TNV, TAPSV) p4_group_go<EV, TNV, TAPSV>(grid, stream, g, P4_NAME("conv_p4_group_kernel", EV, false, TNV, TAPSV))
 #define P4_GROUP_T(EV) (wide ? (taps == 9 ? P4_GROUP(EV, 2, 9) : taps == 1 ? P4_GROUP(EV, 2, 1) : P4_GROUP(EV, 2, 0)) \
                              : (taps == 9 ? P4_GROUP(EV, 1, 9) : taps == 1 ? P4_GROUP(EV, 1, 1) : P4_GROUP(EV, 1, 0)))
-    const char* name = p[0].mask ? P4_GROUP_T(4) : P4_GROUP_T(0);
+    if (blk == 0) return "none (no gathered rows)";
+    const char* name = p[0].gather ? P4_GROUP(48, 2, 9) : p[0].mask ? P4_GROUP_T(4) : P4_GROUP_T(0);
 #undef P4_GROUP_T
 #undef P4_GROUP
     return name;
@@ -768,6 +783,7 @@
 #define P4_ONE(EPIV, C4V, TNV, TAPSV) p4_go<EPIV, C4V, TNV, TAPSV>(grid, stream, a, P4_NAME("conv_p4_kernel", EPIV, C4V, TNV, TAPSV))
     if (a.gather) {
         const int taps = p4_taps(a);
+        if (a.out16 || a.energy4) return nullptr;
         if (a.Cin == 4 || a.up || a.mask || a.in_relu || a.dyn_rows || a.row_map || (taps != 1 && taps != 9)) return nullptr;
         if (a.total_mtiles == 0) return "none (no gathered rows)";
 #define P4_G(EPIV, TNV) (taps == 9 ? P4_ONE(EPIV, false, TNV, 9) : P4_ONE(EPIV, false, TNV, 1))
diff --git a/cald_amd/csrc/ctx.hip b/cald_amd/csrc/ctx.hip
--- a/cald_amd/csrc/ctx.hip
+++ b/cald_amd/csrc/ctx.hip
@@ -173,6 +173,18 @@
     return 0;
 }
 
+extern "C" int cald_profile_cutout_stages(cald_ctx* c, double* rows6, double* dense_rows6, double* tiles6, double* dense_tiles6, int64_t* kept3) {
+    if (!c) return fail(CALD_ERR_INVALID, "ctx is null");
+    for (int i = 0; i < 6; i++) {
+        if (rows6) rows6[i] = c->cut_st_rows[i];
+        if (dense_rows6) dense_rows6[i] = c->cut_st_dense[i];
+        if (tiles6) tiles6[i] = c->cut_st_tiles[i];
+        if (dense_tiles6) dense_tiles6[i] = c->cut_st_dense_tiles[i];
+    }
+    if (kept3) for (int i = 0; i < 3; i++) kept3[i] = c->cut_kept[i];
+    return 0;
+}
+
 extern "C" int cald_profile_dump(cald_ctx* c, const char* path) {
     if (!c || !path) return fail(CALD_ERR_INVALID, "null argument");
     HIPCHK(hipStreamSynchronize(c->stream));
diff --git a/cald_amd/csrc/forward.hip b/cald_amd/csrc/forward.hip
--- a/cald_amd/csrc/forward.hip
+++ b/cald_amd/csrc/forward.hip
@@ -324,6 +324,28 @@
     a.gather = reinterpret_cast<const GatherSet*>(base + (size_t)(V + 1) * sizeof(LevelSeg));
     a.total_mtiles = ru.tiles[b][kind];
     return run_conv(m->ctx, a, 2.0 * ru.rows[b][kind] * (double)L.Cout * (double)(L.KH * L.KW * L.CinTrue));
+}
+
+static int gconv_group_on(cald_model* m, const ConvSpec* sp, int n, int V, const FwdReuse& ru) {
+    ConvArgs a[CALD_MAX_GROUP];
+    double flops = 0.0; int tiles = 0;
+    for (int i = 0; i < n; i++) {
+        const double f = fill_conv_args(m, a[i], *sp[i].L, sp[i].in, sp[i].out, sp[i].level, sp[i].level, V, sp[i].relu);
+        if (f < 0.0) return (int)f;
+        const char* base = ru.d_gp + (size_t)(2 * ru.nblk + i) * cut_plan_set_bytes(V);
+        a[i].seg_out = reinterpret_cast<const LevelSeg*>(base);
+        a[i].gather = reinterpret_cast<const GatherSet*>(base + (size_t)(V + 1) * sizeof(LevelSeg));
+        a[i].total_mtiles = ru.fpn_tiles[i];
+        a[i].out16 = sp[i].out16; a[i].energy4 = sp[i].energy4;
+        flops += 2.0 * ru.fpn_rows[i] * (double)sp[i].L->Cout * (double)(sp[i].L->KH * sp[i].L->KW * sp[i].L->CinTrue); tiles += ru.fpn_tiles[i];
+    }
+    if (!tiles) return 0;
+    cald_ctx* c = m->ctx;
+    ProfLaunch t; int rc;
+    if ((rc = prof_begin(c, t))) return rc;
+    const char* k = launch_conv_p4_group(a, n, c->stream);
+    if ((rc = prof_end(c, t, flops, c->prof_tag_now, "mt=%d,Cin=%d,Cout=%d,k=%dx%d,s=%d,group=%d,gathered-rows", tiles, a[0].Cin, a[0].Cout, a[0].KH, a[0].KW, a[0].stride, n))) return rc;
+    return k ? 0 : conv_refused(a[0]);
 }
 
 __global__ void accumulate_rows_kernel(const int* __restrict__ counts, int V, unsigned long long* acc) {
@@ -450,13 +472,19 @@
     int fpn() {
         const int first = retina ? 3 : 2, nl = retina ? 3 : 4, c0 = 4 - nl;
         int rc; ConvSpec sp[4];
+        const bool kept = ru && ru->fpn && !retina;
+        if (kept) {
+            for (int i = 0; i < 4; i++) Fp.Pf[i] = ru->pf[i];
+            if (prune) for (int i = 0; i < 2; i++) { Fq.p16[i] = ru->p16[i]; Fq.energy[i] = ru->energy[i]; }
+        }
         if ((rc = conv_on(m, m->fpn_inner[nl - 1], Fb.Cf[3], Fp.inner[nl - 1], 5, 5, V, false))) return rc;
         for (int i = nl - 2; i >= 0; i--)
             if ((rc = conv_on(m, m->fpn_inner[i], Fb.Cf[c0 + i], Fp.inner[i], first + i, first + i, V, false, nullptr, Fp.inner[i + 1], first + 1 + i))) return rc;
+        for (int i = 0; i < nl; i++) m->dbg["inner" + std::to_string(first + i)] = {Fp.inner[i], first + i, 256, 0};
         for (int i = 0; i < nl; i++) sp[i] = {&m->fpn_layer[i], Fp.inner[i], Fp.Pf[i], first + i, false};
         if (prune)
             for (int i = 0; i < 2; i++) { sp[i].out16 = Fq.p16[i]; sp[i].energy4 = Fq.energy[i]; }
-        if ((rc = conv_group_on(m, sp, nl, V))) return rc;
+        if ((rc = kept && ru->mode == 2 && ru->gather_fpn ? gconv_group_on(m, sp, nl, V, *ru) : conv_group_on(m, sp, nl, V))) return rc;
         if (!retina) return 0;
         if ((rc = conv_on(m, m->p6, Fp.Pf[2], Fp.Pf[3], 5, 6, V, false))) return rc;
         if (feat && !feat->p7) return 0;
diff --git a/cald_amd/csrc/host.h b/cald_amd/csrc/host.h
--- a/cald_amd/csrc/host.h
+++ b/cald_amd/csrc/host.h
@@ -58,6 +58,8 @@
     char* train_scratch = nullptr; size_t train_scratch_cap = 0;
     double cut_rows[3] = {0.0, 0.0, 0.0}, cut_dense[3] = {0.0, 0.0, 0.0};
     long long cut_batches = 0, cut_fallbacks = 0;
+    double cut_st_rows[6] = {}, cut_st_dense[6] = {}, cut_st_tiles[6] = {}, cut_st_dense_tiles[6] = {};
+    long long cut_kept[3] = {0, 0, 0};
 };
 
 namespace cald_host {
@@ -137,6 +139,8 @@
     struct CutReuse {
         int mode = -1;
         char* slot[2] = {nullptr, nullptr}; size_t cap[2] = {0, 0};
+        bool ext_refused = false;
+        size_t ext_cap = 0;
         char* h_gp[2] = {nullptr, nullptr}; char* d_gp = nullptr;
     } cr;
 };
@@ -150,7 +154,12 @@
 struct ConvSpec { const ConvLayer* L; const float* in; float* out; int level; bool relu; const int* dyn = nullptr; const int* row_map = nullptr; const unsigned* in16 = nullptr;
                   unsigned* out16 = nullptr; float* energy4 = nullptr; };
 
-#define CUT_MAX_BLOCKS 32
+#define CUT_MAX_BLOCKS 36
+#define CUT_STAGE_LATERAL 4
+#define CUT_STAGE_OUTPUT 5
+#define CUT_KEPT_FPN 0
+#define CUT_KEPT_STAGES 1
+#define CUT_KEPT_NONE 2
 struct FwdReuse {
     int mode = 0;
     int nblk = 0;
@@ -159,6 +168,10 @@
     const char* d_gp = nullptr;
     int tiles[CUT_MAX_BLOCKS][2] = {};
     double rows[CUT_MAX_BLOCKS][2] = {};
+    bool fpn = false, gather_fpn = false;
+    float* pf[4] = {}; unsigned* p16[2] = {}; float* energy[2] = {};
+    int fpn_tiles[4] = {};
+    double fpn_rows[4] = {};
 };
 struct FwdFeatures {
     const int (*pad_to)[2] = nullptr;
diff --git a/cald_amd/csrc/host_logic.h b/cald_amd/csrc/host_logic.h
--- a/cald_amd/csrc/host_logic.h
+++ b/cald_amd/csrc/host_logic.h
@@ -293,6 +293,28 @@
         s = out[b]; l = lo;
     }
 }
+static inline CutRect cut_hull(const CutRect& a, const CutRect& b) {
+    return {a.x0 < b.x0 ? a.x0 : b.x0, a.y0 < b.y0 ? a.y0 : b.y0, a.x1 > b.x1 ? a.x1 : b.x1, a.y1 > b.y1 ? a.y1 : b.y1};
+}
+static inline void cut_fpn_geometry(int Hp, int Wp, const CutSet* c, CutSet* inner, CutSet* outp) {
+    inner[3] = c[3];
+    for (int i = 2; i >= 0; i--) {
+        const int Hl = Hp >> (2 + i), Wl = Wp >> (2 + i);
+        const CutSet& up = inner[i + 1];
+        CutSet s; s.n = 0;
+        if (up.n == c[i].n) {
+            for (int q = 0; q < up.n; q++) {
+                CutRect u = {2 * up.r[q].x0, 2 * up.r[q].y0, 2 * up.r[q].x1 + 1, 2 * up.r[q].y1 + 1};
+                if (u.x1 > Wl - 1) u.x1 = Wl - 1; if (u.y1 > Hl - 1) u.y1 = Hl - 1;
+                s.r[s.n++] = cut_hull(u, c[i].r[q]);
+            }
+        } else if (up.n || c[i].n) {
+            s.n = 1; s.r[0] = {0, 0, Wl - 1, Hl - 1};
+        }
+        inner[i] = s;
+    }
+    for (int i = 0; i < 4; i++) outp[i] = cut_map(inner[i], 3, 1, 1, Hp >> (2 + i), Wp >> (2 + i));
+}
 static inline int cut_disjoint(const CutSet& s, CutRect* o, int cap) {
     int ys[2 * CUT_SET_MAX], ny = 0;
     for (int i = 0; i < s.n; i++) { ys[ny++] = s.r[i].y0; ys[ny++] = s.r[i].y1 + 1; }
diff --git a/cald_amd/csrc/model.hip b/cald_amd/csrc/model.hip
--- a/cald_amd/csrc/model.hip
+++ b/cald_amd/csrc/model.hip
@@ -320,6 +320,12 @@
     m->cr.mode = mode;
     return 0;
 }
+extern "C" int cald_model_set_cutout_retention_cap(cald_model* m, int64_t bytes, int64_t* was) {
+    if (!m || bytes < 0) return fail(CALD_ERR_INVALID, "bad argument");
+    if (was) *was = (int64_t)m->cr.ext_cap;
+    m->cr.ext_cap = (size_t)bytes;
+    return 0;
+}
 extern "C" int cald_model_set_row_packing(cald_model* m, int mode, int* was) {
     if (!m || mode < -1 || mode > 1) return fail(CALD_ERR_INVALID, "bad argument");
     if (was) *was = m->row_packing;
diff --git a/cald_amd/csrc/ops.hip b/cald_amd/csrc/ops.hip
--- a/cald_amd/csrc/ops.hip
+++ b/cald_amd/csrc/ops.hip
@@ -28,6 +28,28 @@
             q[0] = sset.n;
             for (int i = 0; i < sset.n; i++) { q[1 + 4 * i] = sset.r[i].x0; q[2 + 4 * i] = sset.r[i].y0; q[3 + 4 * i] = sset.r[i].x1; q[4 + 4 * i] = sset.r[i].y1; }
         }
+    return 0;
+}
+extern "C" int cald_op_cutout_fpn_geometry(int H, int W, int min_size, int max_size, int nrect, const int* rects, int nblk, const int* strides, int* out) {
+    if (H < 1 || W < 1 || nrect < 0 || nrect > CALD_MAX_CUT || (nrect && !rects) || nblk < 4 || nblk > 64 || !strides || !out)
+        return fail(CALD_ERR_INVALID, "bad argument");
+    int ends[4], ne = 0;
+    for (int b = 0; b < nblk; b++)
+        if (b == nblk - 1 || strides[b + 1] == 2) { if (ne == 4) return fail(CALD_ERR_INVALID, "more than four stages"); ends[ne++] = b; }
+    if (ne != 4) return fail(CALD_ERR_INVALID, "the strides describe %d stages, not four", ne);
+    int Hr, Wr, Hp, Wp;
+    transform_size(H, W, min_size, max_size, &Hr, &Wr, &Hp, &Wp);
+    std::vector<CutSet> o(nblk), t(nblk);
+    CutSet pool1, cs[4], sets[8];
+    cut_geometry(H, W, Hr, Wr, Hp, Wp, nrect, rects, nblk, strides, &pool1, o.data(), t.data());
+    for (int i = 0; i < 4; i++) cs[i] = o[ends[i]];
+    cut_fpn_geometry(Hp, Wp, cs, sets, sets + 4);
+    for (int e = 0; e < 8; e++) {
+        int* q = out + (size_t)e * (1 + 4 * CUT_SET_MAX);
+        memset(q, 0, sizeof(int) * (1 + 4 * CUT_SET_MAX));
+        q[0] = sets[e].n;
+        for (int i = 0; i < sets[e].n; i++) { q[1 + 4 * i] = sets[e].r[i].x0; q[2 + 4 * i] = sets[e].r[i].y0; q[3 + 4 * i] = sets[e].r[i].x1; q[4 + 4 * i] = sets[e].r[i].y1; }
+    }
     return 0;
 }
 static int get_pil(cald_ctx* c, int inSize, int outSize, int fid, PilCoef* out) {
diff --git a/cald_amd/csrc/sweep.hip b/cald_amd/csrc/sweep.hip
--- a/cald_amd/csrc/sweep.hip
+++ b/cald_amd/csrc/sweep.hip
@@ -64,6 +64,7 @@
     return on;
 }
 #define CUT_GATHER_MAX_COST 0.7
+#define CUT_FPN_MAX_COST CUT_GATHER_MAX_COST
 
 namespace {
 struct PairLayout {
@@ -92,6 +93,7 @@
     std::vector<char> view_inert;
     std::vector<float> cut_margin;
     bool kept = false;
+    bool kept_fpn = false;
     std::vector<int> ref_sel, pair_kind, view_isref;
     std::vector<float> pair_par;
     std::vector<ViewDesc> aviews;
@@ -109,6 +111,8 @@
     float *d_vm[2] = {nullptr, nullptr}, *d_pm = nullptr;
     SweepBatch bt[2];
     int nblk = 0, blk_lin[CUT_MAX_BLOCKS], blk_lout[CUT_MAX_BLOCKS], blk_stage[CUT_MAX_BLOCKS], blk_stride[CUT_MAX_BLOCKS];
+    int ngeo = 0, geo_stride[CUT_MAX_BLOCKS], c_blk[4] = {0, 0, 0, 0};
+    bool fpn_ok = false;
     std::vector<BatchPlan> rplan;
 
     static size_t al(size_t b) { return (b + 255) & ~(size_t)255; }
@@ -175,17 +179,31 @@
             bt[q].h_vm = b.get<float>((size_t)VT * CALD_VM); bt[q].h_pm = b.get<float>((size_t)P_MAX * 2);
         }
         if (m->prune && prune_ok) HIPCHK(hipMemsetAsync(c->d_prune_check, 0, 8, c->stream));
+        for (int a = 0; a < A && cut_a < 0; a++) if (cfg->augs[a].kind == CALD_AUG_CUTOUT) cut_a = a;
+        init_blocks();
+        reuse = (m->cr.mode < 0 ? cut_reuse_env() : m->cr.mode != 0) && cut_a >= 0 && !audit && m->cfg.precision == CALD_PRECISION_FP32 && nblk < CUT_MAX_BLOCKS;
+        rplan.resize(reuse ? 1 : 0);
+        return 0;
+    }
+    void init_blocks() {
         retina = m->cfg.arch == CALD_ARCH_RETINANET;
-        for (int a = 0; a < A && cut_a < 0; a++) if (cfg->augs[a].kind == CALD_AUG_CUTOUT) cut_a = a;
         for (int b = 0, layer = 0, l = 2; b < (int)m->blocks.size() && layer < 3 && nblk < CUT_MAX_BLOCKS; b++) {
             const Bottleneck& Bk = m->blocks[b];
             blk_stride[nblk] = Bk.c2.stride; blk_lin[nblk] = l; l += Bk.c2.stride == 2 ? 1 : 0; blk_lout[nblk] = l; blk_stage[nblk] = layer;
             nblk++;
             if (Bk.layer_end) layer++;
         }
-        reuse = (m->cr.mode < 0 ? cut_reuse_env() : m->cr.mode != 0) && cut_a >= 0 && !audit && m->cfg.precision == CALD_PRECISION_FP32 && nblk < CUT_MAX_BLOCKS;
-        rplan.resize(reuse ? 1 : 0);
-        return 0;
+        {
+            int layer = 0; bool fits = true;
+            for (size_t b = 0; b < m->blocks.size(); b++) {
+                if (ngeo == CUT_MAX_BLOCKS || layer > 3) { fits = false; break; }
+                geo_stride[ngeo] = m->blocks[b].c2.stride;
+                if (m->blocks[b].layer_end) c_blk[layer++] = ngeo;
+                ngeo++;
+            }
+            fpn_ok = fits && layer == 4 && !retina && ngeo >= nblk;
+            if (!fpn_ok) { ngeo = nblk; for (int b = 0; b < nblk; b++) geo_stride[b] = blk_stride[b]; }
+        }
     }
 
     void plan_of(int nv, const ViewDesc* vs, BatchPlan& P) const {
@@ -201,33 +219,59 @@
         }
         return off;
     }
+    size_t retain_layout_fpn(const BatchPlan& P, int nv, char* base, FwdReuse* ru) const {
+        size_t off = retain_layout(P, nv, base, ru ? ru->out : nullptr);
+        auto take = [&](size_t bytes) { char* p = base + off; off += al(bytes); return p; };
+        for (int i = 0; i < 4; i++) { char* p = take((size_t)level_pix(P, 2 + i, nv) * 256 * 4); if (ru) ru->pf[i] = reinterpret_cast<float*>(p); }
+        if (m->prune && prune_ok)
+            for (int i = 0; i < 2; i++) {
+                char* p = take((size_t)level_pix(P, 2 + i, nv) * 256 * 4); char* e = take((size_t)level_pix(P, 2 + i, nv) * 4 * 4);
+                if (ru) { ru->p16[i] = reinterpret_cast<unsigned*>(p); ru->energy[i] = reinterpret_cast<float*>(e); }
+            }
+        if (ru) ru->fpn = true;
+        return off;
+    }
 
     int enqueue_ref(int k) {
         SweepBatch& b = bt[k & 1];
         b.i0 = k * B; b.nb = (n_images - b.i0 < B) ? n_images - b.i0 : B; b.live = true; b.P = 0; b.VV = b.nb;
         std::vector<ViewDesc> views = ref_views(images_dev, H, W, b.i0, b.nb);
         const DetBuffers& D = *DS[k & 1];
-        FwdReuse ru; b.kept = false;
-        if (reuse) {
-            plan_of(b.nb, views.data(), rplan[0]);
-            const size_t need = retain_layout(rplan[0], b.nb, nullptr, nullptr);
-            cald_model::CutReuse& R = m->cr;
-            const int q = k & 1;
-            if (need > R.cap[q]) {
-                HIPCHK(hipStreamSynchronize(c->stream));
-                if (R.slot[q]) hipFree(R.slot[q]);
-                R.slot[q] = nullptr; R.cap[q] = 0;
-                if (hipMalloc((void**)&R.slot[q], need + (need >> 3)) != hipSuccess) { (void)hipGetLastError(); R.slot[q] = nullptr; }
-                else R.cap[q] = need + (need >> 3);
-            }
-            if (R.slot[q]) { ru.mode = 1; ru.nblk = nblk; retain_layout(rplan[0], b.nb, R.slot[q], ru.out); b.kept = true; }
-            else c->cut_fallbacks++;
-        }
+        FwdReuse ru;
+        if (int r = retain(k, views.data(), ru)) return r;
         int r = forward_model(m, b.nb, views.data(), D, audit ? d_vm[k & 1] : nullptr, prune_ok, b.kept ? &ru : nullptr);
         if (r) return r;
         if (hipMemcpyAsync(b.h_count, D.count, (size_t)b.nb * 4, hipMemcpyDeviceToHost, c->stream) != hipSuccess ||
             hipMemcpyAsync(b.h_boxes, D.boxes, (size_t)b.nb * cap * 16, hipMemcpyDeviceToHost, c->stream) != hipSuccess ||
             hipEventRecord(m->ss.ev_ref[k & 1], c->stream) != hipSuccess) return fail(CALD_ERR_HIP, "D2H of reference detections failed");
+        return 0;
+    }
+    int retain(int k, const ViewDesc* views, FwdReuse& ru) {
+        SweepBatch& b = bt[k & 1];
+        b.kept = b.kept_fpn = false;
+        if (reuse) {
+            plan_of(b.nb, views, rplan[0]);
+            cald_model::CutReuse& R = m->cr;
+            const int q = k & 1;
+            const size_t need3 = retain_layout(rplan[0], b.nb, nullptr, nullptr), needx = fpn_ok ? retain_layout_fpn(rplan[0], b.nb, nullptr, nullptr) : 0;
+            bool ext = fpn_ok && !R.ext_refused && !(R.ext_cap && needx > R.ext_cap);
+            for (int attempt = 0; attempt < 2; attempt++) {
+                const size_t need = ext ? needx : need3;
+                if (need <= R.cap[q]) break;
+                HIPCHK(hipStreamSynchronize(c->stream));
+                if (R.slot[q]) hipFree(R.slot[q]);
+                R.slot[q] = nullptr; R.cap[q] = 0;
+                if (hipMalloc((void**)&R.slot[q], need + (need >> 3)) == hipSuccess) { R.cap[q] = need + (need >> 3); break; }
+                (void)hipGetLastError(); R.slot[q] = nullptr;
+                if (!ext) break;
+                ext = false; R.ext_refused = true;
+            }
+            if (R.slot[q]) {
+                ru.mode = 1; ru.nblk = nblk; b.kept = true; b.kept_fpn = ext;
+                if (ext) retain_layout_fpn(rplan[0], b.nb, R.slot[q], &ru); else retain_layout(rplan[0], b.nb, R.slot[q], ru.out);
+            } else c->cut_fallbacks++;
+            c->cut_kept[!b.kept ? CUT_KEPT_NONE : b.kept_fpn ? CUT_KEPT_FPN : CUT_KEPT_STAGES]++;
+        }
         return 0;
     }
 
@@ -342,43 +386,54 @@
 
     int cut_plan(int k, int V, const ViewDesc* vs, FwdReuse& ru) {
         cald_model::CutReuse& R = m->cr;
-        const size_t per = cut_plan_set_bytes(V), total = per * 2 * (size_t)nblk;
+        const bool fpn = bt[k & 1].kept_fpn;
+        const size_t per = cut_plan_set_bytes(V), total = per * (2 * (size_t)nblk + (fpn ? 4 : 0));
         if (!R.d_gp) {
-            const size_t cap = cut_plan_set_bytes(CALD_MAX_VIEWS) * 2 * CUT_MAX_BLOCKS;
+            const size_t cap = cut_plan_set_bytes(CALD_MAX_VIEWS) * (2 * CUT_MAX_BLOCKS + 4);
             HIPCHK(hipMalloc((void**)&R.d_gp, cap));
             HIPCHK(hipHostMalloc((void**)&R.h_gp[0], cap)); HIPCHK(hipHostMalloc((void**)&R.h_gp[1], cap));
         }
         plan_of(V, vs, rplan[0]);
         const BatchPlan& P = rplan[0];
         char* const h = R.h_gp[k & 1];
-        std::vector<CutSet> g_out((size_t)V * nblk), g_t1((size_t)V * nblk);
+        std::vector<CutSet> g_out((size_t)V * ngeo), g_t1((size_t)V * ngeo), g_fpn((size_t)V * 4);
         for (int v = 0; v < V; v++) {
             int Hr, Wr, Hp, Wp; CutSet pool1;
             transform_size(vs[v].H, vs[v].W, m->cfg.min_size, m->cfg.max_size, &Hr, &Wr, &Hp, &Wp);
-            cut_geometry(vs[v].H, vs[v].W, Hr, Wr, Hp, Wp, vs[v].nrect, vs[v].rects, nblk, blk_stride, &pool1, &g_out[(size_t)v * nblk], &g_t1[(size_t)v * nblk]);
-        }
+            cut_geometry(vs[v].H, vs[v].W, Hr, Wr, Hp, Wp, vs[v].nrect, vs[v].rects, ngeo, geo_stride, &pool1, &g_out[(size_t)v * ngeo], &g_t1[(size_t)v * ngeo]);
+            if (fpn) {
+                CutSet cs[4], inner[4];
+                for (int i = 0; i < 4; i++) cs[i] = g_out[(size_t)v * ngeo + c_blk[i]];
+                cut_fpn_geometry(Hp, Wp, cs, inner, &g_fpn[(size_t)v * 4]);
+            }
+        }
+        auto put_set = [&](size_t index, int lvl, const CutSet* sets, size_t stride_v, int* tiles_out, double* rows_out) {
+            LevelSeg* sg = reinterpret_cast<LevelSeg*>(h + index * per);
+            GatherSet* gs = reinterpret_cast<GatherSet*>(reinterpret_cast<char*>(sg) + (size_t)(V + 1) * sizeof(LevelSeg));
+            int tiles = 0; double rows = 0.0;
+            for (int v = 0; v < V; v++) {
+                LevelSeg L = P.seg[lvl][v]; L.tile_start = tiles; sg[v] = L;
+                CutRect rr[CALD_GATHER_RECTS];
+                int n = cut_disjoint(sets[(size_t)v * stride_v], rr, CALD_GATHER_RECTS);
+                if (n < 0) { n = 1; rr[0] = {0, 0, L.W - 1, L.H - 1}; }
+                GatherSet& G = gs[v]; memset(&G, 0, sizeof(G));
+                G.nr = n;
+                for (int q = 0; q < n; q++) {
+                    G.x0[q] = rr[q].x0; G.y0[q] = rr[q].y0; G.w[q] = rr[q].x1 - rr[q].x0 + 1;
+                    G.cum[q + 1] = G.cum[q] + G.w[q] * (rr[q].y1 - rr[q].y0 + 1);
+                }
+                tiles += (G.cum[n] + 127) / 128; rows += (double)G.cum[n];
+            }
+            sg[V] = P.seg[lvl][V]; sg[V].tile_start = tiles;
+            *tiles_out = tiles; *rows_out = rows;
+        };
         auto kf = [](const ConvLayer& L) { return (double)L.Cout * (double)(L.KH * L.KW * L.CinTrue); };
-        double cost_g[3] = {0, 0, 0}, cost_d[3] = {0, 0, 0}, rows_g[3] = {0, 0, 0}, rows_d[3] = {0, 0, 0};
+        double cost_g[3] = {0, 0, 0}, cost_d[3] = {0, 0, 0}, rows_g[3] = {0, 0, 0}, rows_d[3] = {0, 0, 0}, tiles_g[3] = {0, 0, 0}, tiles_d[3] = {0, 0, 0};
         for (int b = 0; b < nblk; b++)
             for (int kind = 0; kind < 2; kind++) {
                 const int lvl = kind ? blk_lin[b] : blk_lout[b];
-                LevelSeg* sg = reinterpret_cast<LevelSeg*>(h + (size_t)(2 * b + kind) * per);
-                GatherSet* gs = reinterpret_cast<GatherSet*>(reinterpret_cast<char*>(sg) + (size_t)(V + 1) * sizeof(LevelSeg));
-                int tiles = 0; double rows = 0.0;
-                for (int v = 0; v < V; v++) {
-                    LevelSeg L = P.seg[lvl][v]; L.tile_start = tiles; sg[v] = L;
-                    CutRect rr[CALD_GATHER_RECTS];
-                    int n = cut_disjoint(kind ? g_t1[(size_t)v * nblk + b] : g_out[(size_t)v * nblk + b], rr, CALD_GATHER_RECTS);
-                    if (n < 0) { n = 1; rr[0] = {0, 0, L.W - 1, L.H - 1}; }
-                    GatherSet& G = gs[v]; memset(&G, 0, sizeof(G));
-                    G.nr = n;
-                    for (int q = 0; q < n; q++) {
-                        G.x0[q] = rr[q].x0; G.y0[q] = rr[q].y0; G.w[q] = rr[q].x1 - rr[q].x0 + 1;
-                        G.cum[q + 1] = G.cum[q] + G.w[q] * (rr[q].y1 - rr[q].y0 + 1);
-                    }
-                    tiles += (G.cum[n] + 127) / 128; rows += (double)G.cum[n];
-                }
-                sg[V] = P.seg[lvl][V]; sg[V].tile_start = tiles;
+                int tiles; double rows;
+                put_set((size_t)(2 * b + kind), lvl, (kind ? g_t1.data() : g_out.data()) + b, (size_t)ngeo, &tiles, &rows);
                 ru.tiles[b][kind] = tiles; ru.rows[b][kind] = rows;
                 const Bottleneck& Bk = m->blocks[b];
                 const double w = kind ? kf(Bk.c1) : kf(Bk.c2) + kf(Bk.c3) + (Bk.has_down ? kf(Bk.down) : 0.0);
@@ -386,14 +441,45 @@
                 const int st = blk_stage[b];
                 cost_g[st] += 128.0 * tiles * w; cost_d[st] += dense * w;
                 rows_g[st] += rows * nconv; rows_d[st] += dense * nconv;
+                tiles_g[st] += tiles * nconv; tiles_d[st] += (double)P.seg[lvl][V].tile_start * nconv;
             }
         for (int st = 0; st < 3; st++) {
             ru.gather[st] = m->cr.mode != 2 && cost_g[st] <= CUT_GATHER_MAX_COST * cost_d[st];
             c->cut_rows[st] += ru.gather[st] ? rows_g[st] : rows_d[st]; c->cut_dense[st] += rows_d[st];
+            c->cut_st_rows[st] += ru.gather[st] ? rows_g[st] : rows_d[st]; c->cut_st_dense[st] += rows_d[st];
+            c->cut_st_tiles[st] += ru.gather[st] ? tiles_g[st] : tiles_d[st]; c->cut_st_dense_tiles[st] += tiles_d[st];
+        }
+        {
+            double r4 = 0.0, t4 = 0.0, rl = 0.0, tl = 0.0;
+            int lvl = 2;
+            for (size_t b = 0; b < m->blocks.size(); b++) {
+                const Bottleneck& Bk = m->blocks[b];
+                const int lo = lvl + (Bk.c2.stride == 2 ? 1 : 0);
+                if ((int)b >= nblk) {
+                    const double n_in = 1.0, n_out = Bk.has_down ? 3.0 : 2.0;
+                    r4 += n_in * (double)level_pix(P, lvl, V) + n_out * (double)level_pix(P, lo, V);
+                    t4 += n_in * (double)P.seg[lvl][V].tile_start + n_out * (double)P.seg[lo][V].tile_start;
+                }
+                lvl = lo;
+            }
+            if (!retina) for (int i = 0; i < 4; i++) { rl += (double)level_pix(P, 2 + i, V); tl += (double)P.seg[2 + i][V].tile_start; }
+            c->cut_st_rows[3] += r4; c->cut_st_dense[3] += r4; c->cut_st_tiles[3] += t4; c->cut_st_dense_tiles[3] += t4;
+            c->cut_st_rows[CUT_STAGE_LATERAL] += rl; c->cut_st_dense[CUT_STAGE_LATERAL] += rl;
+            c->cut_st_tiles[CUT_STAGE_LATERAL] += tl; c->cut_st_dense_tiles[CUT_STAGE_LATERAL] += tl;
+            double fg = 0.0, fd = 0.0, frg = 0.0, frd = 0.0;
+            if (fpn)
+                for (int i = 0; i < 4; i++) {
+                    put_set(2 * (size_t)nblk + i, 2 + i, g_fpn.data() + i, 4, &ru.fpn_tiles[i], &ru.fpn_rows[i]);
+                    fg += ru.fpn_tiles[i]; frg += ru.fpn_rows[i];
+                }
+            if (!retina) for (int i = 0; i < 4; i++) { fd += (double)P.seg[2 + i][V].tile_start; frd += (double)level_pix(P, 2 + i, V); }
+            ru.gather_fpn = fpn && m->cr.mode != 2 && 128.0 * fg <= CUT_FPN_MAX_COST * frd;
+            c->cut_st_rows[CUT_STAGE_OUTPUT] += ru.gather_fpn ? frg : frd; c->cut_st_dense[CUT_STAGE_OUTPUT] += frd;
+            c->cut_st_tiles[CUT_STAGE_OUTPUT] += ru.gather_fpn ? fg : fd; c->cut_st_dense_tiles[CUT_STAGE_OUTPUT] += fd;
         }
         if (hipMemcpyAsync(R.d_gp, h, total, hipMemcpyHostToDevice, c->stream) != hipSuccess) return fail(CALD_ERR_HIP, "H2D of the cut_out gather plan failed");
         ru.mode = 2; ru.nblk = nblk; ru.d_gp = R.d_gp;
-        retain_layout(P, V, m->cr.slot[k & 1], ru.out);
+        if (fpn) retain_layout_fpn(P, V, m->cr.slot[k & 1], &ru); else retain_layout(P, V, m->cr.slot[k & 1], ru.out);
         c->cut_batches++;
         return 0;
     }
@@ -530,6 +616,41 @@
         return rc;
     }
 };
+}
+
+extern "C" int cald_debug_cutout_forward(cald_model* m, int n_views, const cald_view* views, const cald_dets* out, int prune) {
+    if (!m || !views || !out || n_views < 1 || n_views > CALD_MAX_VIEWS) return fail(CALD_ERR_INVALID, "bad argument");
+    if (!m->finalized) return fail(CALD_ERR_STATE, "model not finalized");
+    std::vector<ViewDesc> cut(n_views), ref(n_views);
+    for (int i = 0; i < n_views; i++) {
+        const cald_view& v = views[i];
+        if (v.nrect < 0 || v.nrect > CALD_MAX_CUT || v.flip || v.noise_dev) return fail(CALD_ERR_INVALID, "view %d is no cut_out view", i);
+        cut[i] = plain_view(v.image_dev, v.H, v.W); ref[i] = cut[i];
+        cut[i].nrect = v.nrect;
+        for (int q = 0; q < 4 * v.nrect; q++) cut[i].rects[q] = v.rects[q];
+    }
+    DetBuffers det;
+    det.boxes = out->boxes_dev; det.scores = out->scores_dev; det.labels = (long long*)out->labels_dev; det.props = out->props_dev;
+    det.prob_max = out->prob_max_dev; det.scores_cls = out->scores_cls_dev; det.count = out->count_dev;
+    det.cap = out->cap; det.C = m->cfg.num_classes;
+    if (!det.boxes || !det.scores || !det.labels || !det.props || !det.prob_max || !det.scores_cls || !det.count)
+        return fail(CALD_ERR_INVALID, "output buffers must all be provided");
+    SweepRun R{m, n_views, nullptr, nullptr, nullptr, nullptr, nullptr, nullptr, nullptr, nullptr, false};
+    R.c = m->ctx;
+    HIPCHK(hipSetDevice(R.c->device));
+    R.prune_ok = prune != 0;
+    R.init_blocks();
+    R.reuse = (m->cr.mode < 0 ? cut_reuse_env() : m->cr.mode != 0) && m->cfg.precision == CALD_PRECISION_FP32 && R.nblk < CUT_MAX_BLOCKS;
+    R.rplan.resize(1);
+    R.bt[0].nb = n_views;
+    if (m->prune && R.prune_ok) HIPCHK(hipMemsetAsync(R.c->d_prune_check, 0, 8, R.c->stream));
+    FwdReuse ru, ru2;
+    int rc = R.retain(0, ref.data(), ru);
+    if (!rc) rc = forward_model(m, n_views, ref.data(), det, nullptr, R.prune_ok, R.bt[0].kept ? &ru : nullptr);
+    if (!rc && R.bt[0].kept) rc = R.cut_plan(0, n_views, cut.data(), ru2);
+    if (!rc) rc = forward_model(m, n_views, cut.data(), det, nullptr, R.prune_ok, R.bt[0].kept ? &ru2 : nullptr);
+    if (!rc) HIPCHK(hipStreamSynchronize(R.c->stream));
+    return rc;
 }
 
 static int sweep_checked(cald_model* m, int n_images, const uint8_t* const* images_dev, const int* H, const int* W,
diff --git a/cald_amd/detector.py b/cald_amd/detector.py
--- a/cald_amd/detector.py
+++ b/cald_amd/detector.py
@@ -158,7 +158,7 @@
             self._handle = h
         return self._handle
 
-    def forward_views(self, views):
+    def forward_views(self, views, _entry=None):
         L = _ffi.lib()
         h = self.handle()
         n = len(views)
@@ -184,7 +184,7 @@
                     arr[i].rects[j] = int(r)
         d = _ffi.Dets(out["boxes"].data_ptr(), out["scores"].data_ptr(), out["labels"].data_ptr(), out["props"].data_ptr(),
                       out["prob_max"].data_ptr(), out["scores_cls"].data_ptr(), out["count"].data_ptr(), cap)
-        _ffi.check(L.cald_forward(h, n, arr, C.byref(d)))
+        _ffi.check(L.cald_forward(h, n, arr, C.byref(d)) if _entry is None else _entry(L, h, n, arr, C.byref(d)))
         counts = out["count"].cpu().tolist()
         res = []
         for i, k in enumerate(counts):
@@ -215,6 +215,9 @@
             noise = rem.contiguous() if bool((rem != 0).any()) else None
             views.append((g.permute(1, 2, 0).contiguous(), False, None, noise))
         return self.forward_views(views)
+
+    def debug_cutout_forward(self, views, prune=False):
+        return self.forward_views(views, _entry=lambda L, h, n, arr, d: L.cald_debug_cutout_forward(h, n, arr, d, int(bool(prune))))
 
     def set_rpn_prune(self, on):
         was = C.c_int(0)
diff --git a/include/cald_hip.h b/include/cald_hip.h
--- a/include/cald_hip.h
+++ b/include/cald_hip.h
@@ -185,6 +185,7 @@
 int cald_op_pil_resize(cald_ctx* ctx, const uint8_t* src_dev, int H, int W, uint8_t* dst_dev, int oh, int ow);
 int cald_op_cutout_rects(uint64_t seed, int H, int W, int N, const float* boxes, int cut_num, int* rects_out, int* n_out);
 int cald_op_cutout_geometry(int H, int W, int min_size, int max_size, int nrect, const int* rects, int nblk, const int* strides, int* out);
+int cald_op_cutout_fpn_geometry(int H, int W, int min_size, int max_size, int nrect, const int* rects, int nblk, const int* strides, int* out);
 int cald_op_augment(cald_ctx* ctx, int kind, double param, uint64_t seed, const uint8_t* src_dev, int H, int W,
                     int n_boxes, const float* boxes, void* dst_dev, float* boxes_out, int* aux_out);
 int cald_op_noise_stream(cald_ctx* ctx, uint64_t seed, const uint8_t* src_dev, int H, int W, int nseg, const int* kinds,
@@ -295,6 +296,9 @@
 int cald_model_set_row_packing(cald_model* m, int mode, int* was);
 int cald_model_set_box_min_size(cald_model* m, float min_size, float* was);
 int cald_profile_cutout(cald_ctx* ctx, double* rows3, double* dense_rows3, int64_t* batches, int64_t* fallbacks);
+int cald_profile_cutout_stages(cald_ctx* ctx, double* rows6, double* dense_rows6, double* tiles6, double* dense_tiles6, int64_t* kept3);
+int cald_model_set_cutout_retention_cap(cald_model* m, int64_t bytes, int64_t* was);
+int cald_debug_cutout_forward(cald_model* m, int n_views, const cald_view* views, const cald_dets* out, int prune);
 int cald_profile_roi_rows(cald_ctx* ctx, double* mean_rows_per_view, int64_t* views);
 int cald_profile_dump(cald_ctx* ctx, const char* path);
 
```

New measurement: 178.4, median of 6. 1.02x the previous value.
